# nv-tlabs/3dgrut

Measured on AMD Instinct MI355X. Metric: train rays/sec (3DGUT forward+backward, primary rays), higher is better.
Workload: dtype f32; 1 GPU; 3DGUT fwd+bwd, 1000000 Gaussians (cloud B trained-like, seed 42), 1920x1080, one view per GPU, SH degree 3, k_buffer 0; parallelism=view-dp1

## Files before the change

3dgrut_amd/csrc/common.hpp:

```cpp
#pragma once

#include <hip/hip_runtime.h>

#include <cstdarg>
#include <cstdint>
#include <cstdio>
#include <cstring>

#include "../../include/grut_amd.h"

#define GRUT_ABI_VERSION 5
#define GRUT_WAVE 64

namespace grut {

void set_last_error(const char* fmt, ...);

#define GRUT_HIP(expr)                                                                          \
    do {                                                                                        \
        hipError_t _e = (expr);                                                                 \
        if (_e != hipSuccess) {                                                                 \
            grut::set_last_error("%s:%d %s -> %s", __FILE__, __LINE__, #expr, hipGetErrorString(_e)); \
            return GRUT_ERR_RUNTIME;                                                            \
        }                                                                                       \
    } while (0)

#define GRUT_CHECK(expr)                       \
    do {                                       \
        int _s = (expr);                       \
        if (_s != GRUT_OK) return _s;          \
    } while (0)

#define GRUT_REQUIRE(cond, ...)                \
    do {                                       \
        if (!(cond)) {                         \
            grut::set_last_error(__VA_ARGS__); \
            return GRUT_ERR_BAD_INPUT;         \
        }                                      \
    } while (0)

#ifdef __HIPCC__
__device__ __forceinline__ uint32_t xcd_contiguous(uint32_t b, uint32_t n) {
    const uint32_t xcd = b & 7u, idx = b >> 3, q = n >> 3, rem = n & 7u;
    return xcd * q + (xcd < rem ? xcd : rem) + idx;
}
#endif

struct ScratchAllocator {
    void* (*alloc)(void* user, uint64_t bytes) = nullptr;
    void (*release)(void* user, void* ptr) = nullptr;
    void* user = nullptr;
};
ScratchAllocator& scratch_allocator();
inline hipStream_t& scratch_stream() {
    static thread_local hipStream_t s = nullptr;
    return s;
}
struct ScratchStreamScope {
    hipStream_t prev;
    explicit ScratchStreamScope(hipStream_t s) : prev(scratch_stream()) { scratch_stream() = s; }
    ~ScratchStreamScope() { scratch_stream() = prev; }
    ScratchStreamScope(const ScratchStreamScope&) = delete;
    ScratchStreamScope& operator=(const ScratchStreamScope&) = delete;
};
struct DeviceBuffer {
    void* ptr = nullptr;
    size_t bytes = 0;
    bool external = false;
    int ensure(size_t need, float growth = 1.0f) {
        if (need <= bytes) return GRUT_OK;
        size_t n = (size_t)((double)need * growth);
        n = (n + 255) & ~(size_t)255;
        release();
        const ScratchAllocator& a = scratch_allocator();
        if (a.alloc) {
            ptr = a.alloc(a.user, n);
            if (!ptr) {
                set_last_error("scratch allocation of %zu bytes failed in the caller's allocator", n);
                return GRUT_ERR_RUNTIME;
            }
            external = true;
            {
                static int count = 0;
                const char* pz = getenv("GRUT_POISON_SCRATCH");
                const char* pi = getenv("GRUT_POISON_INDEX");
                const bool poison = pz && (!pi || atoi(pi) == count);
                if (pz && pi && atoi(pi) == count) fprintf(stderr, "[grut] poisoned allocation %d: %zu bytes\n", count, n);
                ++count;
                GRUT_HIP(hipMemsetAsync(ptr, poison ? atoi(pz) : 0, n, scratch_stream()));
            }
        } else {
            GRUT_HIP(hipMalloc(&ptr, n));
            external = false;
        }
        bytes = n;
        return GRUT_OK;
    }
    void release() {
        if (ptr) {
            const ScratchAllocator& a = scratch_allocator();
            if (external && a.release) a.release(a.user, ptr);
            else if (!external) (void)hipFree(ptr);
        }
        ptr = nullptr;
        bytes = 0;
    }
    template <typename T> T* as() const { return reinterpret_cast<T*>(ptr); }
};

inline uint32_t div_up(uint32_t a, uint32_t b) { return (a + b - 1) / b; }

struct EventTimer {
    static constexpr int kRing = 256;
    hipEvent_t start[kRing], stop[kRing];
    int count = 0, created = 0;
    int begin(hipStream_t s) {
        int i = count % kRing;
        if (i >= created) {
            GRUT_HIP(hipEventCreate(&start[i]));
            GRUT_HIP(hipEventCreate(&stop[i]));
            created = i + 1;
        }
        GRUT_HIP(hipEventRecord(start[i], s));
        return GRUT_OK;
    }
    int end(hipStream_t s) {
        int i = count % kRing;
        GRUT_HIP(hipEventRecord(stop[i], s));
        count++;
        return GRUT_OK;
    }
    float collect() {
        int n = count < kRing ? count : kRing;
        if (n == 0) return -1.f;
        double sum = 0;
        for (int i = 0; i < n; ++i) {
            float ms = 0;
            (void)hipEventSynchronize(stop[i]);
            (void)hipEventElapsedTime(&ms, start[i], stop[i]);
            sum += ms;
        }
        count = 0;
        return (float)(sum / n);
    }
    void destroy() {
        for (int i = 0; i < created; ++i) {
            (void)hipEventDestroy(start[i]);
            (void)hipEventDestroy(stop[i]);
        }
        created = 0;
    }
};

size_t scan_scratch_bytes(uint32_t n);
int inclusive_scan_u32(hipStream_t s, uint32_t n, const uint32_t* in, const uint32_t* gather, uint32_t* out,
                       void* scratch, size_t scratch_bytes);
size_t sort_scratch_bytes(uint32_t n);
int sort_pairs_u32(hipStream_t s, uint32_t n, const uint32_t* n_dev, int begin_bit, int end_bit,
                   uint32_t* keys, uint32_t* vals, uint32_t* keys_tmp, uint32_t* vals_tmp,
                   void* scratch, size_t scratch_bytes, uint32_t** out_keys, uint32_t** out_vals, bool vals_iota = false);

}

#ifdef __HIPCC__
namespace grut {

struct f3 {
    float x, y, z;
};
__device__ __forceinline__ f3 mk3(float x, float y, float z) { return f3{x, y, z}; }
__device__ __forceinline__ f3 operator+(f3 a, f3 b) { return f3{a.x + b.x, a.y + b.y, a.z + b.z}; }
__device__ __forceinline__ f3 operator-(f3 a, f3 b) { return f3{a.x - b.x, a.y - b.y, a.z - b.z}; }
__device__ __forceinline__ f3 operator*(f3 a, f3 b) { return f3{a.x * b.x, a.y * b.y, a.z * b.z}; }
__device__ __forceinline__ f3 operator*(f3 a, float s) { return f3{a.x * s, a.y * s, a.z * s}; }
__device__ __forceinline__ f3 operator*(float s, f3 a) { return f3{a.x * s, a.y * s, a.z * s}; }
__device__ __forceinline__ float dot(f3 a, f3 b) { return fmaf(a.x, b.x, fmaf(a.y, b.y, a.z * b.z)); }
__device__ __forceinline__ float mul_rn(float a, float b) { float r; asm("v_mul_f32 %0, %1, %2" : "=v"(r) : "v"(a), "v"(b)); return r; }
__device__ __forceinline__ float add_rn(float a, float b) { float r; asm("v_add_f32 %0, %1, %2" : "=v"(r) : "v"(a), "v"(b)); return r; }
__device__ __forceinline__ float mul_rn_u(float uniform, float b) { float r; asm("v_mul_f32 %0, %1, %2" : "=v"(r) : "s"(uniform), "v"(b)); return r; }
__device__ __forceinline__ float add_rn_u(float uniform, float b) { float r; asm("v_add_f32 %0, %1, %2" : "=v"(r) : "s"(uniform), "v"(b)); return r; }
__device__ __forceinline__ f3 cross(f3 a, f3 b) {
    return f3{a.y * b.z - a.z * b.y, a.z * b.x - a.x * b.z, a.x * b.y - a.y * b.x};
}
struct m3 {
    f3 r0, r1, r2;
};
__device__ __forceinline__ f3 mul_rows(const m3& m, f3 p) { return f3{dot(m.r0, p), dot(m.r1, p), dot(m.r2, p)}; }
__device__ __forceinline__ f3 mul_cols(const m3& m, f3 g) {
    return f3{g.x * m.r0.x + g.y * m.r1.x + g.z * m.r2.x, g.x * m.r0.y + g.y * m.r1.y + g.z * m.r2.y,
              g.x * m.r0.z + g.y * m.r1.z + g.z * m.r2.z};
}
__device__ __forceinline__ m3 quat_wxyz_to_rotT(float r, float x, float y, float z) {
    const float xx = x * x, yy = y * y, zz = z * z, xy = x * y, xz = x * z, yz = y * z;
    const float rx = r * x, ry = r * y, rz = r * z;
    m3 m;
    m.r0 = f3{1.f - 2.f * (yy + zz), 2.f * (xy + rz), 2.f * (xz - ry)};
    m.r1 = f3{2.f * (xy - rz), 1.f - 2.f * (xx + zz), 2.f * (yz + rx)};
    m.r2 = f3{2.f * (xz + ry), 2.f * (yz - rx), 1.f - 2.f * (xx + yy)};
    return m;
}

template <int DEG>
__device__ __forceinline__ float particle_response(float g) {
    if constexpr (DEG == 8) { const float g2 = g * g; return __expf(-0.000685871056241f * g2 * g2); }
    else if constexpr (DEG == 5) return __expf(-0.0185185185185f * g * g * sqrtf(g));
    else if constexpr (DEG == 4) return __expf(-0.0555555555556f * g * g);
    else if constexpr (DEG == 3) return __expf(-0.166666666667f * g * sqrtf(g));
    else if constexpr (DEG == 1) return __expf(-1.5f * sqrtf(g));
    else if constexpr (DEG == 0) return fmaxf(1.f - 0.329630334487f * sqrtf(g), 0.f);
    else return __expf(-0.5f * g);
}
template <int DEG>
__device__ __forceinline__ float particle_response_grd(float g, float gres, float gresGrd) {
    if constexpr (DEG == 8) return (-0.000685871056241f * 4.f) * g * g * g * gres * gresGrd;
    else if constexpr (DEG == 5) return (-0.0185185185185f * 2.5f) * g * sqrtf(g) * gres * gresGrd;
    else if constexpr (DEG == 4) return (-0.0555555555556f * 2.f) * g * gres * gresGrd;
    else if constexpr (DEG == 3) return (-0.166666666667f * 1.5f) * sqrtf(g) * gres * gresGrd;
    else if constexpr (DEG == 1) return (-1.5f * 0.5f) * sqrtf(g) * gres * gresGrd;
    else if constexpr (DEG == 0) return gres > 0.f ? (0.5f * -0.329630334487f * rsqrtf(g)) * gresGrd : 0.f;
    else return -0.5f * gres * gresGrd;
}

__device__ __forceinline__ int lane_id() { return (int)__builtin_amdgcn_mbcnt_hi(~0u, __builtin_amdgcn_mbcnt_lo(~0u, 0u)); }

template <int CTRL, int ROW_MASK = 0xf>
__device__ __forceinline__ float dpp_add(float v) {
    const int moved = __builtin_amdgcn_update_dpp(0, __float_as_int(v), CTRL, ROW_MASK, 0xf, true);
    return v + __int_as_float(moved);
}
__device__ __forceinline__ float wave_sum_to_lane63(float v) {
    v = dpp_add<0x111>(v);
    v = dpp_add<0x112>(v);
    v = dpp_add<0x114>(v);
    v = dpp_add<0x118>(v);
    v = dpp_add<0x142, 0xa>(v);
    v = dpp_add<0x143, 0xc>(v);
    return v;
}
template <int CTRL>
__device__ __forceinline__ float dpp_perm(float v) {
    return __int_as_float(__builtin_amdgcn_update_dpp(0, __float_as_int(v), CTRL, 0xf, 0xf, true));
}
__device__ __forceinline__ float wave_reduce_scatter16_rows(const float (&v)[16], int lane) {
    const bool b3 = lane & 8, b2 = lane & 4, b1 = lane & 2, b0 = lane & 1;
    float w[8], x[4], y[2];
#pragma unroll
    for (int i = 0; i < 8; ++i) {
        const float keep = b3 ? v[8 + i] : v[i], send = b3 ? v[i] : v[8 + i];
        w[i] = keep + dpp_perm<0x140>(send);
    }
#pragma unroll
    for (int i = 0; i < 4; ++i) {
        const float keep = b2 ? w[4 + i] : w[i], send = b2 ? w[i] : w[4 + i];
        x[i] = keep + dpp_perm<0x141>(send);
    }
#pragma unroll
    for (int i = 0; i < 2; ++i) {
        const float keep = b1 ? x[2 + i] : x[i], send = b1 ? x[i] : x[2 + i];
        y[i] = keep + dpp_perm<0x4E>(send);
    }
    float z = (b0 ? y[1] : y[0]) + dpp_perm<0xB1>(b0 ? y[0] : y[1]);
    return z;
}
__device__ __forceinline__ float wave_reduce_scatter16(const float (&v)[16], int lane) {
    float z = wave_reduce_scatter16_rows(v, lane);
    z += __shfl_xor(z, 16, 64);
    z += __shfl_xor(z, 32, 64);
    return z;
}

__device__ __forceinline__ float wave_reduce_scatter16_all(const float (&v)[16], int lane) {
    typedef unsigned v2u __attribute__((ext_vector_type(2)));
    const float z = wave_reduce_scatter16_rows(v, lane);
    const v2u a = __builtin_amdgcn_permlane32_swap(__float_as_uint(z), __float_as_uint(z), false, false);
    const float s = __uint_as_float(a.x) + __uint_as_float(a.y);
    const v2u b = __builtin_amdgcn_permlane16_swap(__float_as_uint(s), __float_as_uint(s), false, false);
    return __uint_as_float(b.x) + __uint_as_float(b.y);
}

typedef float v2f __attribute__((ext_vector_type(2)));
struct p3 {
    v2f x, y, z;
};
__device__ __forceinline__ v2f splat(float s) { v2f r = {s, s}; return r; }
__device__ __forceinline__ v2f pfma(v2f a, v2f b, v2f c) { return __builtin_elementwise_fma(a, b, c); }
__device__ __forceinline__ v2f pfma(float a, v2f b, v2f c) { return __builtin_elementwise_fma(splat(a), b, c); }
__device__ __forceinline__ v2f pdot(p3 a, p3 b) { return pfma(a.x, b.x, pfma(a.y, b.y, a.z * b.z)); }
__device__ __forceinline__ v2f pdot(f3 a, p3 b) { return pfma(a.x, b.x, pfma(a.y, b.y, a.z * b.z)); }
__device__ __forceinline__ p3 pcross(p3 a, p3 b) {
    return p3{pfma(a.y, b.z, -(a.z * b.y)), pfma(a.z, b.x, -(a.x * b.z)), pfma(a.x, b.y, -(a.y * b.x))};
}
__device__ __forceinline__ v2f psel(bool c0, bool c1, v2f t, v2f f) { v2f r = {c0 ? t.x : f.x, c1 ? t.y : f.y}; return r; }
__device__ __forceinline__ v2f pmax0(v2f a) { v2f r = {fmaxf(a.x, 0.f), fmaxf(a.y, 0.f)}; return r; }
__device__ __forceinline__ v2f prcp(v2f a) { v2f r = {__builtin_amdgcn_rcpf(a.x), __builtin_amdgcn_rcpf(a.y)}; return r; }

template <int DEG>
__device__ __forceinline__ float response_gray_limit(float x) {
    if (!(x < 1.f) || !(x > 0.f)) return x > 0.f ? 0.f : 3.0e38f;
    const float L = -logf(x);
    if constexpr (DEG == 8) return sqrtf(sqrtf(L / 0.000685871056241f));
    else if constexpr (DEG == 5) return powf(L / 0.0185185185185f, 0.4f);
    else if constexpr (DEG == 4) return sqrtf(L / 0.0555555555556f);
    else if constexpr (DEG == 3) return powf(L / 0.166666666667f, 2.f / 3.f);
    else if constexpr (DEG == 1) { const float t = L / 1.5f; return t * t; }
    else if constexpr (DEG == 0) { const float t = (1.f - x) / 0.329630334487f; return t * t; }
    else return 2.f * L;
}

__device__ __forceinline__ float wave_sum(float v) {
    v = wave_sum_to_lane63(v);
    return __int_as_float(__builtin_amdgcn_readlane(__float_as_int(v), 63));
}

// ... 3 lines not shown
```

3dgrut_amd/csrc/grt_api.hip:

```cpp
#include <cstdlib>
#include <vector>

#include "grt_internal.hpp"

using namespace grut;

struct GrtHandle {
    GrtConfig cfg;
    int device = -1;
    uint32_t N = 0;
    bool built = false;
    hipStream_t build_stream = nullptr;
    DeviceBuffer refit_todo;
    DeviceBuffer box8;
    uint32_t NP = 0;
    DeviceBuffer inst, aabb, slack, scene_enc, scene, codes, ids, codes_tmp, ids_tmp, sort_scratch, nodes,
        counters, dbg_ids, dbg_count;
    uint32_t* sorted_ids = nullptr;
    uint32_t* sorted_codes = nullptr;
    float scene_host[6] = {0, 0, 0, 0, 0, 0};
    bool scene_host_valid = false;
    EventTimer fwd_timer, bwd_timer, build_timer;
    DeviceBuffer log_pool, log_table, log_nbwd, log_state;
    GrtHitLog log = {nullptr, nullptr, nullptr, nullptr, 0, 0};
// ... 73 lines not shown
}

static GrtTraceParams trace_params(const GrtHandle* h, const GrtFrame& f) {
    GrtTraceParams P;
    memset(&P, 0, sizeof(P));
    P.degree = h->cfg.particle_kernel_degree;
    P.prim = h->cfg.primitive_type;
    P.bary = h->cfg.pipeline_type == GRUT_PIPELINE_BARYCENTRIC_SURFELS;
    P.clamping = h->cfg.particle_kernel_density_clamping;
    P.box8 = h->cfg.primitive_type == GRUT_PRIM_CUSTOM ? h->box8.as<float>() : nullptr;
    P.ncoef = (h->cfg.particle_radiance_sph_degree + 1) * (h->cfg.particle_radiance_sph_degree + 1);
    P.sph_degree = f.sph_degree < h->cfg.particle_radiance_sph_degree ? f.sph_degree : h->cfg.particle_radiance_sph_degree;
    if (P.sph_degree < 0) P.sph_degree = 0;
    P.normals = h->cfg.enable_normals;
    P.hitcounts = h->cfg.enable_hitcounts;
    P.min_response = h->cfg.particle_kernel_min_response;
    P.min_alpha = h->cfg.particle_kernel_min_alpha;
    P.max_alpha = h->cfg.particle_kernel_max_alpha;
    P.min_transmittance = f.min_transmittance;
    P.W = f.width;
    P.H = f.height;
    for (int k = 0; k < 12; ++k) P.ray_to_world[k] = f.ray_to_world[k];
    P.ray_to_world_dev = f.device_ray_to_world;
    P.sph_half = h->cfg.particle_feature_half;
    P.nht = h->cfg.feature_transform_type;
    if (P.nht) {
        const GrtConfig& c = h->cfg;
        P.nht_k = c.particle_feature_dim; P.nht_ipd = c.interp_point_feature_dim; P.nht_support = c.feature_interpolation_support;
        P.nht_act = c.feature_activation_type; P.nht_nf = c.feature_activation_num_frequencies;
        P.nht_ray_dim = P.nht_ipd * (P.nht_act == 2 ? 2 * P.nht_nf : (P.nht_act == 1 ? P.nht_nf : 1));
    }
    static const int sphere_lists = getenv("GRUT_GRT_SPHERE_LISTS") ? 1 : 0;
    P.sphere_lists = sphere_lists;
    static const float list_mark = getenv("GRUT_GRT_LIST_MARK") ? (float)atof(getenv("GRUT_GRT_LIST_MARK")) : 1.0f;
    P.list_mark = list_mark;
    static const uint32_t lane_area = getenv("GRUT_GRT_LANE_AREA") ? (uint32_t)atoi(getenv("GRUT_GRT_LANE_AREA")) : 32u;
    P.bin_lane_area = lane_area < 1u ? 1u : (lane_area > 64u ? 64u : lane_area);
    P.out_half = h->cfg.feature_output_half;
    return P;
}

static GrtBvh bvh_view(const GrtHandle* h) {
    GrtBvh b;
    b.nodes = h->nodes.as<GrtNode>();
    b.inst = h->inst.as<float>();
    b.scene = h->scene.as<float>();
    b.N = h->NP;
    return b;
}

extern "C" {

int grt_create(const GrtConfig* config, GrtHandle** handle) {
    GRUT_REQUIRE(config && handle, "grt_create: null argument");
    GRUT_CHECK(grt_validate(*config));
    GrtHandle* h = new GrtHandle();
    h->cfg = *config;
    if (hipGetDevice(&h->device) != hipSuccess) {
        set_last_error("grt_create: no HIP device");
        delete h;
        return GRUT_ERR_RUNTIME;
    }
    if (hipHostMalloc(reinterpret_cast<void**>(&h->log_state_host), 64, hipHostMallocDefault) != hipSuccess ||
        hipEventCreateWithFlags(&h->log_event, hipEventDisableTiming) != hipSuccess) {
        set_last_error("grt_create: pinned buffer / event allocation failed");
        delete h;
        return GRUT_ERR_RUNTIME;
    }
    *handle = h;
    return GRUT_OK;
}

static void release_scratch(GrtHandle* h) {
    DeviceBuffer* bufs[] = {&h->refit_todo, &h->box8, &h->inst, &h->aabb, &h->slack, &h->scene_enc, &h->scene, &h->codes, &h->ids, &h->codes_tmp, &h->ids_tmp,
                            &h->sort_scratch, &h->nodes, &h->counters, &h->dbg_ids, &h->dbg_count,
                            &h->work_counters, &h->l_flags, &h->l_starts, &h->l_bounds, &h->l_pair_cache, &h->l_block_cones, &h->l_super_cones, &h->l_inst_rel, &h->l_key_bits,
                            &h->l_counts, &h->l_pidx, &h->l_key_tmp, &h->l_pidx_tmp, &h->l_offsets, &h->l_scan_scratch, &h->l_sort_scratch,
                            &h->l_block_keys, &h->l_vals, &h->l_block_keys_tmp, &h->l_vals_tmp, &h->l_ranges,
                            &h->log_pool, &h->log_table, &h->log_nbwd, &h->log_state, &h->m_aabb, &h->m_slack, &h->m_scene_enc,
                            &h->m_scene, &h->m_codes, &h->m_ids, &h->m_codes_tmp, &h->m_ids_tmp, &h->m_sort_scratch, &h->m_nodes, &h->m_done, &h->m_materials};
    for (DeviceBuffer* b : bufs) b->release();
}

int grt_trim(GrtHandle* h) {
    GRUT_REQUIRE(h, "grt_trim: null handle");
    GRUT_HIP(hipDeviceSynchronize());
    release_scratch(h);
    h->built = false;
    h->tree_async = false;
    h->mesh_built = false;
    h->N = 0;
    h->NP = 0;
    h->log_valid = false;
    h->log_event_pending = false;
    h->scene_host_valid = false;
    h->list_entries = 0;
    h->log = GrtHitLog{nullptr, nullptr, nullptr, nullptr, 0, 0};
    h->log_lists = GrtLists{nullptr, nullptr, nullptr, nullptr, nullptr};
    h->sorted_codes = nullptr;
    h->sorted_ids = nullptr;
    return GRUT_OK;
}

void grt_destroy(GrtHandle* h) {
    if (!h) return;
    if (h->tree_stream) (void)hipStreamSynchronize(h->tree_stream);
    release_scratch(h);
    if (h->log_state_host) (void)hipHostFree(h->log_state_host);
    if (h->l_host) (void)hipHostFree(h->l_host);
    if (h->log_event) (void)hipEventDestroy(h->log_event);
    if (h->list_event) (void)hipEventDestroy(h->list_event);
    if (h->side_fork) (void)hipEventDestroy(h->side_fork);
    if (h->side_join) (void)hipEventDestroy(h->side_join);
    if (h->side_stream) (void)hipStreamDestroy(h->side_stream);
    if (h->tree_fork) (void)hipEventDestroy(h->tree_fork);
    if (h->tree_done) (void)hipEventDestroy(h->tree_done);
    if (h->tree_stream) (void)hipStreamDestroy(h->tree_stream);
    h->fwd_timer.destroy();
    h->bwd_timer.destroy();
    h->build_timer.destroy();
    delete h;
}

int grt_build_bvh(GrtHandle* h, void* stream_, uint32_t N, const float* positions, const float* rotations, const float* scales,
                  const float* densities, int rebuild, int allow_update) {
    (void)allow_update;
    GRUT_REQUIRE(h, "grt_build_bvh: null handle");
    hipStream_t s = reinterpret_cast<hipStream_t>(stream_);
    ScratchStreamScope scratch_scope(s);
    if (N == 0) {
        h->N = 0;
        h->NP = 0;
        h->built = true;
        return GRUT_OK;
    }
    GRUT_REQUIRE(positions && rotations && scales && densities, "grt_build_bvh: null buffer");
    const uint32_t per = h->cfg.primitive_type == GRUT_PRIM_TRIHEXA ? 3u : (h->cfg.primitive_type == GRUT_PRIM_SPHERE ? 2u : 1u);
    GRUT_REQUIRE((uint64_t)N * per <= 0x1FFFFFFEu, "grt_build_bvh: %u particles (the hit buffers keep 29 bits of proxy index)", N);
    if (!rebuild && (!h->built || h->N != N)) rebuild = 1;
    GRUT_CHECK(h->wait_tree(s));
    if (h->cfg.enable_kernel_timings) GRUT_CHECK(h->build_timer.begin(s));
    const uint32_t NP = N * per;
    const size_t n = NP;
    GRUT_CHECK(h->inst.ensure(n * 48, 1.25f));
    GRUT_CHECK(h->aabb.ensure(n * 24, 1.25f));
    GRUT_CHECK(h->slack.ensure(n * 4, 1.25f));
    if (h->cfg.primitive_type == GRUT_PRIM_CUSTOM) GRUT_CHECK(h->box8.ensure(n * 32, 1.25f));
    GRUT_CHECK(h->scene_enc.ensure(grt_scene_enc_bytes()));
    GRUT_CHECK(h->scene.ensure(64));
    GRUT_CHECK(h->codes.ensure(n * 4, 1.25f));
    GRUT_CHECK(h->ids.ensure(n * 4, 1.25f));
    GRUT_CHECK(h->codes_tmp.ensure(n * 4, 1.25f));
    GRUT_CHECK(h->ids_tmp.ensure(n * 4, 1.25f));
    GRUT_CHECK(h->sort_scratch.ensure(sort_scratch_bytes((uint32_t)(n * 1.25f) + 4096)));
    GRUT_CHECK(h->nodes.ensure(n * sizeof(GrtNode), 1.25f));
    GRUT_CHECK(h->counters.ensure(n * 4, 1.25f));

    GrtBuildParams P;
    P.N = NP;
    P.degree = h->cfg.particle_kernel_degree;
    P.prim = h->cfg.primitive_type;
    P.clamping = h->cfg.particle_kernel_density_clamping;
    P.min_response = h->cfg.particle_kernel_min_response;
    uint32_t* scene_enc = h->scene_enc.as<uint32_t>();
    grt_launch_proxies(s, P, positions, rotations, scales, densities, h->inst.as<float>(), h->aabb.as<float>(), h->slack.as<float>(), scene_enc,
                       h->cfg.primitive_type == GRUT_PRIM_CUSTOM ? h->box8.as<float>() : nullptr);
    grt_launch_morton(s, NP, h->aabb.as<float>(), scene_enc, h->scene.as<float>(), rebuild ? h->codes.as<uint32_t>() : nullptr,
                      rebuild ? h->ids.as<uint32_t>() : nullptr);
    GRUT_CHECK(h->refit_todo.ensure((n + 1) * 4, 1.25f));
    static const bool sync_build = getenv("GRUT_GRT_SYNC_BUILD") != nullptr;
    hipStream_t ts = s;
    h->tree_async = false;
    if (!sync_build) {
        if (!h->tree_stream) {
            GRUT_HIP(hipStreamCreateWithFlags(&h->tree_stream, hipStreamNonBlocking));
            GRUT_HIP(hipEventCreateWithFlags(&h->tree_fork, hipEventDisableTiming));
            GRUT_HIP(hipEventCreateWithFlags(&h->tree_done, hipEventDisableTiming));
        }
        GRUT_HIP(hipEventRecord(h->tree_fork, s));
        GRUT_HIP(hipStreamWaitEvent(h->tree_stream, h->tree_fork, 0));
        ts = h->tree_stream;
    }
    if (rebuild) {
        uint32_t *sc = nullptr, *si = nullptr;
        GRUT_CHECK(sort_pairs_u32(ts, NP, nullptr, 0, 30, h->codes.as<uint32_t>(), h->ids.as<uint32_t>(), h->codes_tmp.as<uint32_t>(),
                                  h->ids_tmp.as<uint32_t>(), h->sort_scratch.ptr, h->sort_scratch.bytes, &sc, &si));
        h->sorted_codes = sc;
        h->sorted_ids = si;
        grt_launch_hierarchy(ts, NP, sc, si, h->nodes.as<GrtNode>());
    }
    GRUT_HIP(hipMemsetAsync(h->counters.ptr, 0, n, ts));
    grt_launch_refit(ts, NP, h->aabb.as<float>(), h->slack.as<float>(), h->nodes.as<GrtNode>(), h->counters.as<uint8_t>(), h->refit_todo.as<uint32_t>());
    GRUT_HIP(hipGetLastError());
    if (h->cfg.enable_kernel_timings) GRUT_CHECK(h->build_timer.end(ts));
    if (ts != s) {
        GRUT_HIP(hipEventRecord(h->tree_done, ts));
        h->tree_async = true;
    }
    h->N = N;
    h->NP = NP;
    h->built = true;
    h->build_stream = s;
    h->scene_host_valid = false;
    return GRUT_OK;
}

static int build_lists(GrtHandle* h, hipStream_t s, const GrtTraceParams& P, const GrtBvh& bvh, const float* ray_origin, const float* ray_direction,
                       GrtLists* out) {
    GrtLists lists = {nullptr, nullptr, nullptr, nullptr, nullptr, nullptr};
    h->list_entries = 0;
    h->log_lists = lists;
    if (!getenv("GRUT_GRT_NO_LISTS") && h->N > 0 && !(h->cfg.primitive_type == GRUT_PRIM_CUSTOM && getenv("GRUT_GRT_CUSTOM_WALK")) && !(h->cfg.primitive_type == GRUT_PRIM_TRIHEXA && getenv("GRUT_GRT_TRIHEXA_WALK")) && !(h->cfg.primitive_type == GRUT_PRIM_TRISURFEL && getenv("GRUT_GRT_TRISURFEL_WALK")) &&
        (h->cfg.primitive_type == GRUT_PRIM_INSTANCES || !getenv("GRUT_GRT_NO_MESH_LISTS"))) {
        const uint32_t N = h->NP, nb = grt_num_blocks(P.W, P.H), ns = grt_num_super(P.W, P.H);
        if (!h->l_host) GRUT_HIP(hipHostMalloc(reinterpret_cast<void**>(&h->l_host), 64));
        GRUT_CHECK(h->l_flags.ensure(64));
        GRUT_CHECK(h->l_block_cones.ensure(grt_cone_table_bytes(P.W, P.H), 1.25f));
        GRUT_CHECK(h->l_super_cones.ensure((size_t)ns * sizeof(GrtCone), 1.25f));
        GRUT_CHECK(h->l_inst_rel.ensure((size_t)N * 64, 1.25f));
        GRUT_CHECK(h->l_pair_cache.ensure(grt_pair_cache_bytes(N), 1.25f));
        for (DeviceBuffer* b4 : {&h->l_key_bits, &h->l_counts, &h->l_pidx, &h->l_key_tmp, &h->l_pidx_tmp, &h->l_offsets, &h->l_starts})
            GRUT_CHECK(b4->ensure((size_t)N * 4, 1.25f));
        GRUT_CHECK(h->l_scan_scratch.ensure(scan_scratch_bytes((uint32_t)(N * 1.25f) + 4096)));
        uint32_t* flag = h->l_flags.as<uint32_t>();
        uint32_t* dir_len = flag + 2;
        grt_launch_list_cones(s, P, ray_origin, ray_direction, flag, dir_len, h->l_block_cones.as<GrtCone>(), h->l_super_cones.as<GrtCone>());
        grt_launch_list_count(s, P, bvh, ray_origin, flag, dir_len, h->l_block_cones.as<GrtCone>(), h->l_super_cones.as<GrtCone>(),
                              h->l_inst_rel.as<float>(), h->l_key_bits.as<uint32_t>(), h->l_counts.as<uint32_t>(), h->l_pidx.as<uint32_t>(), h->l_pair_cache.ptr);
        GRUT_CHECK(h->l_sort_scratch.ensure(sort_scratch_bytes((uint32_t)(N * 1.25f) + 4096)));
        uint32_t *sorted_key = nullptr, *rank_to_particle = nullptr;
        GRUT_CHECK(sort_pairs_u32(s, N, nullptr, 16, 32, h->l_key_bits.as<uint32_t>(), h->l_pidx.as<uint32_t>(), h->l_key_tmp.as<uint32_t>(),
                                  h->l_pidx_tmp.as<uint32_t>(), h->l_sort_scratch.ptr, h->l_sort_scratch.bytes, &sorted_key, &rank_to_particle, true));
        GRUT_CHECK(inclusive_scan_u32(s, N, h->l_counts.as<uint32_t>(), rank_to_particle, h->l_offsets.as<uint32_t>(), h->l_scan_scratch.ptr,
                                      h->l_scan_scratch.bytes));
        grt_launch_list_check(s, N, h->l_offsets.as<uint32_t>(), flag);
        GRUT_HIP(hipMemcpyAsync(&h->l_host[0], h->l_offsets.as<uint32_t>() + (N - 1), 4, hipMemcpyDeviceToHost, s));
        GRUT_HIP(hipMemcpyAsync(&h->l_host[1], flag, 8, hipMemcpyDeviceToHost, s));
        if (!h->list_event) GRUT_HIP(hipEventCreateWithFlags(&h->list_event, hipEventDisableTiming));
        GRUT_HIP(hipEventRecord(h->list_event, s));
        int bits = 1;
        while ((1ull << bits) <= nb) ++bits;
        uint32_t *sorted_blocks = nullptr, *sorted_ids = nullptr;
        auto enqueue_tail = [&](uint32_t n, const uint32_t* n_dev) -> int {
            grt_launch_list_expand(s, P, bvh, ray_origin, flag, dir_len, h->l_block_cones.as<GrtCone>(), h->l_super_cones.as<GrtCone>(),
                                   rank_to_particle, h->l_offsets.as<uint32_t>(), h->l_counts.as<uint32_t>(), h->l_starts.as<uint32_t>(), n,
                                   h->l_block_keys.as<uint32_t>(), h->l_vals.as<uint32_t>(), h->l_pair_cache.ptr);
            GRUT_CHECK(sort_pairs_u32(s, n, n_dev, 0, bits, h->l_block_keys.as<uint32_t>(), h->l_vals.as<uint32_t>(), h->l_block_keys_tmp.as<uint32_t>(),
                                      h->l_vals_tmp.as<uint32_t>(), h->l_sort_scratch.ptr, h->l_sort_scratch.bytes, &sorted_blocks, &sorted_ids));
            GRUT_HIP(hipMemsetAsync(h->l_ranges.ptr, 0, (size_t)nb * 8, s));
            grt_launch_list_ranges(s, n, n_dev, nb, sorted_blocks, h->l_ranges.as<uint32_t>());
            return GRUT_OK;
        };
        auto ensure_entries = [&](uint32_t n) -> bool {
            bool ok = true;
            for (DeviceBuffer* b4 : {&h->l_block_keys, &h->l_vals, &h->l_block_keys_tmp, &h->l_vals_tmp}) ok = ok && b4->ensure((size_t)n * 4, 1.3f) == GRUT_OK;
            ok = ok && h->l_ranges.ensure((size_t)nb * 8, 1.25f) == GRUT_OK;
            ok = ok && h->l_bounds.ensure((size_t)n * 8, 1.3f) == GRUT_OK;
            ok = ok && h->l_sort_scratch.ensure(sort_scratch_bytes((uint32_t)(n * 1.3f) + 4096)) == GRUT_OK;
            if (!ok) (void)hipGetLastError();
            return ok;
        };
        auto entry_capacity = [&]() -> uint32_t {
            size_t cap = h->l_bounds.bytes / 8;
            for (const DeviceBuffer* b4 : {&h->l_block_keys, &h->l_vals, &h->l_block_keys_tmp, &h->l_vals_tmp}) cap = cap < b4->bytes / 4 ? cap : b4->bytes / 4;
            if (h->l_ranges.bytes < (size_t)nb * 8) return 0u;
            while (cap > 0 && h->l_sort_scratch.bytes < sort_scratch_bytes((uint32_t)cap)) cap = cap * 3 / 4;
            return (uint32_t)(cap < 0xFFFF0000ull ? cap : 0xFFFF0000ull);
        };
        const bool speculate = getenv("GRUT_GRT_SPECULATE") != nullptr;
        const uint32_t spec_cap = speculate ? entry_capacity() : 0u;
        if (spec_cap > 0) GRUT_CHECK(enqueue_tail(spec_cap, h->l_offsets.as<uint32_t>() + (N - 1)));
        GRUT_HIP(hipEventSynchronize(h->list_event));
        const uint64_t I = h->l_host[0];
        bool usable = h->l_host[1] != 0u && h->l_host[2] == 0u && I > 0 && I < 0xFFFF0000ull;
        if (usable && !(spec_cap > 0 && I <= spec_cap)) {
            usable = ensure_entries((uint32_t)I);
            if (usable) GRUT_CHECK(enqueue_tail((uint32_t)I, nullptr));
        }
        if (usable) {
            lists.ranges = h->l_ranges.as<uint32_t>();
            lists.entries = sorted_ids;
            lists.inst_rel = h->l_inst_rel.as<float>();
            lists.block_cones = h->l_block_cones.as<GrtCone>();
            lists.dir_len_enc = dir_len;
            lists.bounds = h->l_bounds.as<float2>();
            h->list_entries = I;
        }
    }
    *out = lists;
    return GRUT_OK;
}

static int grt_forward_impl(GrtHandle* h, hipStream_t s, const GrtFrame* frame, const float* particle_density, const float* particle_sph,
                            const float* ray_origin, const float* ray_direction, float* out_features, float* out_density,
                            float* out_hit_distance, float* out_normals, float* out_hits_count, int32_t* out_visibility,
                            uint32_t* dbg_ids, uint32_t* dbg_count, uint32_t dbg_cap) {
    ScratchStreamScope scratch_scope(s);
    GRUT_REQUIRE(h && frame, "grt_forward: null handle/frame");
    if (!h->built) {
        set_last_error("grt_forward: build_bvh has not been called");
        return GRUT_ERR_NOT_READY;
    }
    GRUT_REQUIRE(frame->width > 0 && frame->height > 0, "grt_forward: empty image");
    GRUT_REQUIRE(frame->num_particles == h->N, "grt_forward: %u particles but the BVH holds %u", frame->num_particles, h->N);
    GRUT_REQUIRE(ray_origin && ray_direction && out_features && out_density && out_hit_distance && out_hits_count, "grt_forward: null buffer");
    if (h->N == 0) return GRUT_OK;
    GRUT_REQUIRE(particle_density && particle_sph && out_visibility, "grt_forward: null particle buffer");
    GRUT_REQUIRE(!h->cfg.enable_normals || out_normals, "grt_forward: normals enabled but no buffer");
    GrtTraceParams P = trace_params(h, *frame);
    P.dbg_cap = dbg_cap;
    if (h->cfg.enable_kernel_timings) GRUT_CHECK(h->fwd_timer.begin(s));
    GrtHitLog log = {nullptr, nullptr, nullptr, nullptr, 0, 0};
    h->log_valid = false;
    GRUT_REQUIRE(!(P.nht && dbg_ids), "grt_debug_forward_hits: not provided with neural harmonic features");
    if ((frame->keep_hits_for_backward || P.nht) && !dbg_ids && !P.bary) {
        const uint32_t blocks = div_up((uint32_t)P.W, 8) * div_up((uint32_t)P.H, 8);
        uint32_t want = blocks * 10u;
        if (h->log_event_pending && hipEventQuery(h->log_event) == hipSuccess) {
            h->log_event_pending = false;
            const uint32_t used = h->log_state_host[0];
            if (used + used / 2 > want) want = used + used / 2;
            if (h->log_state_host[7] && h->log_rounds < 4096u) h->log_rounds *= 2u;
        }
        const uint32_t kMaxRounds = h->log_rounds;
        if (h->log.capacity_chunks > want) want = h->log.capacity_chunks;
        if (const char* e = getenv("GRUT_GRT_LOG_CHUNKS")) want = (uint32_t)atoi(e) > 0 ? (uint32_t)atoi(e) : 1u;
        GRUT_CHECK(h->log_pool.ensure((size_t)want * kGrtLogSlots * 64 * 4));
        GRUT_CHECK(h->log_table.ensure((size_t)blocks * kMaxRounds * 4, 1.25f));
        GRUT_CHECK(h->log_nbwd.ensure((size_t)P.W * P.H * 4, 1.25f));
        GRUT_CHECK(h->log_state.ensure(64));
        h->log.pool = h->log_pool.as<uint32_t>();
        h->log.table = h->log_table.as<uint32_t>();
        h->log.ray_flags = h->log_nbwd.as<uint32_t>();
        h->log.state = h->log_state.as<uint32_t>();
        h->log.capacity_chunks = want;
        h->log.max_rounds = kMaxRounds;
        GRUT_HIP(hipMemsetAsync(h->log.table, 0xFF, (size_t)blocks * kMaxRounds * 4, s));
        GRUT_HIP(hipMemsetAsync(h->log.state, 0, 64, s));
        log = h->log;
        h->log_valid = true;
        h->log_W = P.W;
        h->log_H = P.H;
        h->log_density = particle_density;
        h->log_ray_o = ray_origin;
        h->log_ray_d = ray_direction;
        h->log_frame = *frame;
    }
    unsigned long long* counters = nullptr;
    if (getenv("GRUT_GRT_COUNT")) {
        const size_t wbytes = 128 + 24 * ((size_t)div_up((uint32_t)P.W, 64) * div_up((uint32_t)P.H, 64) * 64 + 512);
        GRUT_CHECK(h->work_counters.ensure(wbytes));
        counters = h->work_counters.as<unsigned long long>();
        GRUT_HIP(hipMemsetAsync(counters, 0, wbytes, s));
    }
    GrtBvh bvh = bvh_view(h);
    GrtLists lists;
    GRUT_CHECK(build_lists(h, s, P, bvh, ray_origin, ray_direction, &lists));
    if (h->log_valid || (P.bary && frame->keep_hits_for_backward)) h->log_lists = lists;
    if (!lists.ranges) GRUT_CHECK(h->wait_tree(s));
    grt_launch_trace_fwd(s, P, bvh, particle_density, particle_sph, ray_origin, ray_direction, out_features, out_density,
                         out_hit_distance, out_normals, out_hits_count, out_visibility, dbg_ids, dbg_count, counters, log, lists);
    if (P.nht) {
        for (int attempt = 0; attempt < 8; ++attempt) {
            uint32_t st[8] = {0, 0, 0, 0, 0, 0, 0, 0};
            GRUT_HIP(hipMemcpyAsync(st, log.state, 32, hipMemcpyDeviceToHost, s));
            GRUT_HIP(hipStreamSynchronize(s));
            if (st[1] == 0u && st[7] == 0u) break;
            GRUT_REQUIRE(attempt < 7, "grt_forward: the hit log does not fit (neural harmonic features)");
            const uint32_t blocks = div_up((uint32_t)P.W, 8) * div_up((uint32_t)P.H, 8);
            if (st[7]) {
                h->log_rounds = h->log_rounds < 4096u ? h->log_rounds * 2u : h->log_rounds;
                GRUT_CHECK(h->log_table.ensure((size_t)blocks * h->log_rounds * 4, 1.25f));
                h->log.table = h->log_table.as<uint32_t>();
                h->log.max_rounds = h->log_rounds;
            }
            const uint32_t want = st[7] && st[0] < h->log.capacity_chunks ? h->log.capacity_chunks : h->log.capacity_chunks * 2u;
            GRUT_CHECK(h->log_pool.ensure((size_t)want * kGrtLogSlots * 64 * 4));
            h->log.pool = h->log_pool.as<uint32_t>();
            h->log.capacity_chunks = want;
            GRUT_HIP(hipMemsetAsync(h->log.table, 0xFF, (size_t)blocks * h->log.max_rounds * 4, s));
            GRUT_HIP(hipMemsetAsync(h->log.state, 0, 64, s));
            log = h->log;
            grt_launch_trace_fwd(s, P, bvh, particle_density, particle_sph, ray_origin, ray_direction, out_features, out_density,
                                 out_hit_distance, out_normals, out_hits_count, out_visibility, dbg_ids, dbg_count, counters, log, lists);
        }
        grt_launch_nht_fwd(s, P, particle_density, particle_sph, ray_origin, ray_direction, out_features, log);
    }
    if (log.pool && !h->log_event_pending) {
        GRUT_HIP(hipMemcpyAsync(h->log_state_host, log.state, 32, hipMemcpyDeviceToHost, s));
        GRUT_HIP(hipEventRecord(h->log_event, s));
        h->log_event_pending = true;
    }
    if (counters) {
        GRUT_HIP(hipMemcpyAsync(h->work_host, counters, 128, hipMemcpyDeviceToHost, s));
        GRUT_HIP(hipStreamSynchronize(s));
        fprintf(stderr, "[grut] grt fwd: nodes %llu, leaf tests %llu, processed %llu, rounds %llu, inserts %llu (rays %d)\n", h->work_host[0],
                h->work_host[1], h->work_host[2], h->work_host[3], h->work_host[4], frame->width * frame->height);
        fprintf(stderr, "[grut] grt fwd list batches fetched (64 entries each) %llu\n", h->work_host[12]);
        fprintf(stderr, "[grut] grt fwd leaf tests: passed %llu, distance out of range %llu, box missed %llu, beyond 3 sigma %llu; wave-level leaf visits %llu, of which ran the box test %llu, the insert chain %llu\n",
                h->work_host[5], h->work_host[6], h->work_host[7], h->work_host[8], h->work_host[9], h->work_host[10], h->work_host[11]);
        fprintf(stderr, "[grut] grt fwd phases, summed over the packets' waves (ms): scans %.1f (candidate work loops %.1f with packet lists), hit log %.1f, per-hit evaluation %.1f\n", h->work_host[13] * 1e-5,
                lists.ranges ? h->work_host[0] * 1e-5 : 0.0, h->work_host[14] * 1e-5, h->work_host[15] * 1e-5);
        if (lists.ranges) h->work_host[0] = 0;
    }
    GRUT_HIP(hipGetLastError());
    if (h->cfg.enable_kernel_timings) GRUT_CHECK(h->fwd_timer.end(s));
    return GRUT_OK;
}

int grt_forward(GrtHandle* h, void* stream_, const GrtFrame* frame, const float* particle_density, const void* particle_sph,
                const float* ray_origin, const float* ray_direction, void* out_features, float* out_density, float* out_hit_distance,
                float* out_normals, float* out_hits_count, int32_t* out_visibility) {
    return grt_forward_impl(h, reinterpret_cast<hipStream_t>(stream_), frame, particle_density, reinterpret_cast<const float*>(particle_sph), ray_origin, ray_direction,
                            reinterpret_cast<float*>(out_features), out_density, out_hit_distance, out_normals, out_hits_count, out_visibility, nullptr, nullptr, 0);
}

int grt_debug_forward_hits(GrtHandle* h, void* stream_, const GrtFrame* frame, const float* particle_density, const void* particle_sph,
                           const float* ray_origin, const float* ray_direction, void* out_features, float* out_density,
                           float* out_hit_distance, float* out_normals, float* out_hits_count, int32_t* out_visibility,
                           uint32_t* hit_ids, uint32_t* hit_counts, uint32_t capacity) {
    GRUT_REQUIRE(hit_ids && hit_counts && capacity > 0, "grt_debug_forward_hits: null hit buffers");
    return grt_forward_impl(h, reinterpret_cast<hipStream_t>(stream_), frame, particle_density, reinterpret_cast<const float*>(particle_sph), ray_origin, ray_direction,
                            reinterpret_cast<float*>(out_features), out_density, out_hit_distance, out_normals, out_hits_count, out_visibility, hit_ids, hit_counts,
                            capacity);
}

int grt_backward(GrtHandle* h, void* stream_, const GrtFrame* frame, const float* particle_density, const void* particle_sph_,
                 const float* ray_origin, const float* ray_direction, const void* features_, const float* density, const float* hit_distance,
                 const float* normals, const float* grad_features, const float* grad_density, const float* grad_hit_distance,
                 const float* grad_normals, float* grad_particle_density, float* grad_particle_sph) {
    const float* particle_sph = reinterpret_cast<const float*>(particle_sph_);
    const float* features = reinterpret_cast<const float*>(features_);
    (void)normals;
    (void)grad_normals;
    GRUT_REQUIRE(h && frame, "grt_backward: null handle/frame");
    if (h->cfg.pipeline_type == GRUT_PIPELINE_BARYCENTRIC_SURFELS) {
        set_last_error("grt_backward: pipeline_type barycentricSurfels is forward only (the reference ships no backward program for it)");
        return GRUT_ERR_UNSUPPORTED;
    }
    hipStream_t s = reinterpret_cast<hipStream_t>(stream_);
    ScratchStreamScope scratch_scope(s);
    if (!h->built) {
        set_last_error("grt_backward: build_bvh has not been called");
        return GRUT_ERR_NOT_READY;
    }
    GRUT_REQUIRE(frame->num_particles == h->N, "grt_backward: %u particles but the BVH holds %u", frame->num_particles, h->N);
    if (h->N == 0) return GRUT_OK;
    GRUT_REQUIRE(particle_density && particle_sph && ray_origin && ray_direction && features && density && hit_distance && grad_features &&
                     grad_density && grad_particle_density && grad_particle_sph, "grt_backward: null buffer");
    GrtTraceParams P = trace_params(h, *frame);
    P.bwd_sig = h->dbg_bwd_sig;
    P.bwd_cnt = h->dbg_bwd_cnt;
    if (h->cfg.enable_kernel_timings) GRUT_CHECK(h->bwd_timer.begin(s));
    GrtHitLog log = {nullptr, nullptr, nullptr, nullptr, 0, 0};
    GrtLists lists = {nullptr, nullptr, nullptr, nullptr, nullptr, nullptr};
    if (h->log_matches(*frame, particle_density, ray_origin, ray_direction)) {
        log = h->log;
        lists = h->log_lists;
    }
    if (log.pool && getenv("GRUT_GRT_COUNT")) {
        std::vector<uint32_t> nb((size_t)P.W * P.H);
        uint32_t st[2] = {0, 0};
        GRUT_HIP(hipMemcpyAsync(nb.data(), log.ray_flags, nb.size() * 4, hipMemcpyDeviceToHost, s));
        GRUT_HIP(hipMemcpyAsync(st, log.state, 8, hipMemcpyDeviceToHost, s));
        GRUT_HIP(hipStreamSynchronize(s));
        size_t flagged = 0;
        for (uint32_t v : nb) flagged += (v >> 31);
        fprintf(stderr, "[grut] grt bwd: %zu of %zu rays re-derive their rounds (log chunks %u, overflow %u, lists %s)\n", flagged, nb.size(), st[0], st[1],
                lists.ranges ? "yes" : "no");
    }
    if (!lists.ranges) GRUT_CHECK(h->wait_tree(s));
    hipStream_t rederive = s;
    struct SideJoin {
        GrtHandle* h;
        hipStream_t s;
        bool armed;
        int join() {
            armed = false;
            GRUT_HIP(hipEventRecord(h->side_join, h->side_stream));
            GRUT_HIP(hipStreamWaitEvent(s, h->side_join, 0));
            return GRUT_OK;
        }
        ~SideJoin() { if (armed) (void)join(); }
    } side{h, s, false};
    if (log.pool) {
        if (!h->side_stream) {
            GRUT_HIP(hipStreamCreateWithFlags(&h->side_stream, hipStreamNonBlocking));
            GRUT_HIP(hipEventCreateWithFlags(&h->side_fork, hipEventDisableTiming));
            GRUT_HIP(hipEventCreateWithFlags(&h->side_join, hipEventDisableTiming));
        }
        GRUT_HIP(hipEventRecord(h->side_fork, s));
        side.armed = true;
        GRUT_HIP(hipStreamWaitEvent(h->side_stream, h->side_fork, 0));
        rederive = h->side_stream;
    }
    grt_launch_trace_bwd(s, rederive, P, bvh_view(h), particle_density, particle_sph, ray_origin, ray_direction, features, density, hit_distance,
                         grad_features, grad_density, grad_hit_distance, grad_particle_density, grad_particle_sph, log, lists);
    if (log.pool) GRUT_CHECK(side.join());
    GRUT_HIP(hipGetLastError());
    if (h->cfg.enable_kernel_timings) GRUT_CHECK(h->bwd_timer.end(s));
    return GRUT_OK;
}

int grt_build_mesh_bvh(GrtHandle* h, void* stream_, uint32_t num_vertices, const float* vertices, uint32_t num_faces, const int32_t* triangles,
                       int rebuild, int allow_update) {
    GRUT_REQUIRE(h, "grt_build_mesh_bvh: null handle");
    hipStream_t s = reinterpret_cast<hipStream_t>(stream_);
    ScratchStreamScope scratch_scope(s);
    const bool refit_only = !rebuild && allow_update && h->mesh_built && h->mesh_faces == num_faces && num_faces > 0;
    h->mesh_built = false;
    if (num_faces == 0) {
        h->mesh_faces = 0;
        h->mesh_built = true;
        return GRUT_OK;
    }
    GRUT_REQUIRE(vertices && triangles && num_vertices > 0, "grt_build_mesh_bvh: null buffer");
    const size_t n = num_faces;
    GRUT_CHECK(h->m_aabb.ensure(n * 24, 1.25f));
    GRUT_CHECK(h->m_slack.ensure(n * 4, 1.25f));
    GRUT_CHECK(h->m_scene_enc.ensure(grt_scene_enc_bytes()));
    GRUT_CHECK(h->m_scene.ensure(64));
    GRUT_CHECK(h->m_codes.ensure(n * 4, 1.25f));
    GRUT_CHECK(h->m_ids.ensure(n * 4, 1.25f));
    GRUT_CHECK(h->m_codes_tmp.ensure(n * 4, 1.25f));
    GRUT_CHECK(h->m_ids_tmp.ensure(n * 4, 1.25f));
    GRUT_CHECK(h->m_sort_scratch.ensure(sort_scratch_bytes((uint32_t)(n * 1.25f) + 4096)));
    GRUT_CHECK(h->m_nodes.ensure(n * sizeof(GrtNode), 1.25f));
    GRUT_CHECK(h->m_done.ensure(n * 4, 1.25f));
    grt_launch_mesh_aabb(s, num_faces, vertices, triangles, h->m_aabb.as<float>(), h->m_slack.as<float>(), h->m_scene_enc.as<uint32_t>());
    grt_launch_morton(s, num_faces, h->m_aabb.as<float>(), h->m_scene_enc.as<uint32_t>(), h->m_scene.as<float>(),
                      refit_only ? nullptr : h->m_codes.as<uint32_t>(), refit_only ? nullptr : h->m_ids.as<uint32_t>());
    if (!refit_only) {
        uint32_t *sc = nullptr, *si = nullptr;
        GRUT_CHECK(sort_pairs_u32(s, num_faces, nullptr, 0, 30, h->m_codes.as<uint32_t>(), h->m_ids.as<uint32_t>(), h->m_codes_tmp.as<uint32_t>(),
                                  h->m_ids_tmp.as<uint32_t>(), h->m_sort_scratch.ptr, h->m_sort_scratch.bytes, &sc, &si));
        grt_launch_hierarchy(s, num_faces, sc, si, h->m_nodes.as<GrtNode>());
    }
    GRUT_HIP(hipMemsetAsync(h->m_done.ptr, 0, n, s));
    grt_launch_refit(s, num_faces, h->m_aabb.as<float>(), h->m_slack.as<float>(), h->m_nodes.as<GrtNode>(), h->m_done.as<uint8_t>());
    GRUT_HIP(hipGetLastError());
    h->mesh_faces = num_faces;
    h->mesh_built = true;
    return GRUT_OK;
}

int grt_trace_hybrid(GrtHandle* h, void* stream_, const GrtFrame* frame, const float* particle_density, const void* particle_sph_,
                     const float* ray_origin, const float* ray_direction, const float* ray_max_t, const GrtMesh* mesh, const GrtHybridOptions* options,
                     float* out_radiance, float* out_opacity, float* out_last_ray, uint32_t* out_bounces) {
    GRUT_REQUIRE(h && frame && mesh && options, "grt_trace_hybrid: null argument");
    const float* particle_sph = reinterpret_cast<const float*>(particle_sph_);
    hipStream_t s = reinterpret_cast<hipStream_t>(stream_);
    ScratchStreamScope scratch_scope(s);
    if (!h->built || !h->mesh_built) {
        set_last_error("grt_trace_hybrid: build_bvh / build_mesh_bvh have not been called");
        return GRUT_ERR_NOT_READY;
    }
    GRUT_REQUIRE(frame->width > 0 && frame->height > 0 && ray_origin && ray_direction && out_radiance && out_opacity, "grt_trace_hybrid: null buffer");
    GRUT_REQUIRE(frame->num_particles == h->N, "grt_trace_hybrid: %u particles but the BVH holds %u", frame->num_particles, h->N);
    GRUT_REQUIRE(mesh->num_faces == h->mesh_faces, "grt_trace_hybrid: %u faces but the mesh BVH holds %u", mesh->num_faces, h->mesh_faces);
    GRUT_REQUIRE(h->N == 0 || (particle_density && particle_sph), "grt_trace_hybrid: null particle buffer");
    GRUT_REQUIRE(mesh->num_faces == 0 || (mesh->vertices && mesh->triangles && mesh->prim_type && mesh->refractive_index), "grt_trace_hybrid: null mesh buffer");
    GRUT_REQUIRE(!(options->playground_opts & 1u) || mesh->num_faces == 0 || mesh->vertex_normals, "grt_trace_hybrid: smooth normals need vertex_normals");
    GRUT_REQUIRE((mesh->vertex_tangents != nullptr) == (mesh->vertex_has_tangents != nullptr), "grt_trace_hybrid: vertex_tangents and vertex_has_tangents go together");
    GRUT_REQUIRE(mesh->num_materials == 0 || mesh->materials, "grt_trace_hybrid: null material table");
    const GrtTraceParams P = trace_params(h, *frame);
    GRUT_CHECK(h->wait_tree(s));
    GrtBvh bvh = bvh_view(h);
    GrtMaterial fallback;
    memset(&fallback, 0, sizeof(fallback));
    fallback.diffuse_factor[0] = fallback.diffuse_factor[1] = fallback.diffuse_factor[2] = fallback.diffuse_factor[3] = 1.f;
    fallback.alpha_cutoff = 0.5f;
    const uint32_t nm = mesh->num_materials ? mesh->num_materials : 1u;
    GRUT_CHECK(h->m_materials.ensure((size_t)nm * sizeof(GrtMaterial), 2.f));
    GRUT_HIP(hipMemcpyAsync(h->m_materials.ptr, mesh->num_materials ? mesh->materials : &fallback, (size_t)nm * sizeof(GrtMaterial), hipMemcpyHostToDevice, s));
    GRUT_HIP(hipStreamSynchronize(s));
    GrtMeshView mv;
    mv.nodes = h->m_nodes.as<GrtNode>();
    mv.vertices = mesh->vertices; mv.triangles = mesh->triangles; mv.vnormals = mesh->vertex_normals; mv.vtangents = mesh->vertex_tangents;
    mv.vhas_tangents = mesh->vertex_has_tangents; mv.prim_type = mesh->prim_type; mv.mat_uv = mesh->mat_uv; mv.mat_id = mesh->mat_id;
    mv.refr = mesh->refractive_index; mv.materials = h->m_materials.as<GrtMaterial>(); mv.num_materials = nm; mv.envmap = mesh->envmap;
    mv.envmap_offset[0] = mesh->envmap_offset[0]; mv.envmap_offset[1] = mesh->envmap_offset[1];
    mv.F = mesh->num_faces;
    GrtHybridParams hp;
    hp.opts = options->playground_opts;
    hp.max_pbr_bounces = options->max_pbr_bounces;
    hp.frame_number = options->frame_number;
    if (h->cfg.enable_kernel_timings) GRUT_CHECK(h->fwd_timer.begin(s));
    GrtLists lists;
    GRUT_CHECK(build_lists(h, s, P, bvh, ray_origin, ray_direction, &lists));
    grt_launch_hybrid(s, P, bvh, mv, hp, particle_density, particle_sph, ray_origin, ray_direction, ray_max_t, out_radiance, out_opacity, out_last_ray,
                      out_bounces, lists);
    GRUT_HIP(hipGetLastError());
    if (h->cfg.enable_kernel_timings) GRUT_CHECK(h->fwd_timer.end(s));
    return GRUT_OK;
}

int grt_debug_backward_signature(GrtHandle* h, unsigned long long* ray_signature, uint32_t* ray_hit_count) {
    GRUT_REQUIRE(h && ((ray_signature != nullptr) == (ray_hit_count != nullptr)), "grt_debug_backward_signature: both buffers or none");
    h->dbg_bwd_sig = ray_signature;
    h->dbg_bwd_cnt = ray_hit_count;
    return GRUT_OK;
}

int grt_timings(GrtHandle* h, float* forward_ms, float* backward_ms, float* build_ms) {
    GRUT_REQUIRE(h, "grt_timings: null handle");
    if (forward_ms) *forward_ms = h->fwd_timer.collect();
    if (backward_ms) *backward_ms = h->bwd_timer.collect();
    if (build_ms) *build_ms = h->build_timer.collect();
    return GRUT_OK;
}

int grt_debug_fetch_work(GrtHandle* h, void* stream_, unsigned long long* out, uint64_t count) {
    GRUT_REQUIRE(h && out, "grt_debug_fetch_work: null argument");
    GRUT_REQUIRE(h->work_counters.ptr && count * 8 <= h->work_counters.bytes, "grt_debug_fetch_work: no instrumented frame / count too large");
    GRUT_HIP(hipMemcpyAsync(out, h->work_counters.ptr, count * 8, hipMemcpyDeviceToDevice, reinterpret_cast<hipStream_t>(stream_)));
    return GRUT_OK;
}

int grt_stats(GrtHandle* h, GrtStats* stats) {
    GRUT_REQUIRE(h && stats, "grt_stats: null argument");
    memset(stats, 0, sizeof(*stats));
    stats->num_particles = h->N;
    stats->num_nodes = h->NP > 1 ? h->NP - 1 : (h->NP ? 1 : 0);
    stats->nodes_visited = h->work_host[0];
    stats->candidates = h->work_host[1];
    stats->processed_hits = h->work_host[2];
    stats->list_entries = h->list_entries;
    stats->packet_tests = h->work_host[9];
    stats->list_batches = h->work_host[12];
    if (h->log_valid && h->log.pool) {
        uint32_t st[8] = {0, 0, 0, 0, 0, 0, 0, 0};
        GRUT_HIP(hipDeviceSynchronize());
        GRUT_HIP(hipMemcpy(st, h->log.state, 32, hipMemcpyDeviceToHost));
        stats->bwd_premise_rays = st[2];
        stats->bwd_rederived_rays = st[3];
        stats->bwd_atomic_instructions = st[4];
        stats->bwd_atomic_words = (uint64_t)st[5] * 16u;
    }
    if (h->built && h->N > 0) {
        if (!h->scene_host_valid) {
            GRUT_HIP(hipMemcpyAsync(h->scene_host, h->scene.ptr, 24, hipMemcpyDeviceToHost, h->build_stream));
            GRUT_HIP(hipStreamSynchronize(h->build_stream));
            h->scene_host_valid = true;
        }
        for (int k = 0; k < 6; ++k) stats->scene_aabb[k] = h->scene_host[k];
    }
    return GRUT_OK;
}

int grt_debug_fetch_instances(GrtHandle* h, void* stream_, float* instances) {
    GRUT_REQUIRE(h && h->built && instances, "grt_debug_fetch_instances: no BVH / null buffer");
    const size_t per = h->N ? h->NP / h->N : 1;
    if (h->N) GRUT_HIP(hipMemcpy2DAsync(instances, 48, h->inst.ptr, 48 * per, 48, h->N, hipMemcpyDeviceToDevice, reinterpret_cast<hipStream_t>(stream_)));
    return GRUT_OK;
}

int grt_debug_fetch_custom_boxes(GrtHandle* h, void* stream_, float* box8) {
    GRUT_REQUIRE(h && h->built && box8, "grt_debug_fetch_custom_boxes: no BVH / null buffer");
    if (h->cfg.primitive_type != GRUT_PRIM_CUSTOM) { set_last_error("grt_debug_fetch_custom_boxes: primitive_type is not custom"); return GRUT_ERR_NOT_READY; }
    if (h->N) GRUT_HIP(hipMemcpyAsync(box8, h->box8.ptr, (size_t)h->N * 32, hipMemcpyDeviceToDevice, reinterpret_cast<hipStream_t>(stream_)));
    return GRUT_OK;
}

int grt_debug_fetch_lists(GrtHandle* h, void* stream_, uint32_t* ranges, uint32_t* entries, uint64_t entry_capacity) {
    GRUT_REQUIRE(h && ranges && entries, "grt_debug_fetch_lists: null argument");
    if (!h->log_lists.ranges || h->list_entries == 0 || h->list_entries > entry_capacity) {
        set_last_error("grt_debug_fetch_lists: no packet lists kept (a training forward of a one-origin frame keeps them) or capacity %llu < %llu entries",
                       (unsigned long long)entry_capacity, (unsigned long long)h->list_entries);
        return GRUT_ERR_NOT_READY;
    }
    hipStream_t s = reinterpret_cast<hipStream_t>(stream_);
    const uint32_t blocks = div_up((uint32_t)h->log_W, 8) * div_up((uint32_t)h->log_H, 8);
    GRUT_HIP(hipMemcpyAsync(ranges, h->log_lists.ranges, (size_t)blocks * 8, hipMemcpyDeviceToDevice, s));
    GRUT_HIP(hipMemcpyAsync(entries, h->log_lists.entries, (size_t)h->list_entries * 4, hipMemcpyDeviceToDevice, s));
    return GRUT_OK;
}

}
```

3dgrut_amd/csrc/gut_api.hip:

```cpp
#include <vector>

#include "gut_internal.hpp"

namespace grut {

static thread_local char g_last_error[512] = "";
ScratchAllocator& scratch_allocator() {
    static ScratchAllocator a;
    return a;
}
void set_last_error(const char* fmt, ...) {
    va_list ap;
    va_start(ap, fmt);
    vsnprintf(g_last_error, sizeof(g_last_error), fmt, ap);
    va_end(ap);
}

static uint32_t bits_for(uint32_t n) {
    uint32_t b = 1;
    while ((1ull << b) <= n) ++b;
    return b;
}

}

using namespace grut;

struct GutHandle {
    GutConfig cfg;
    int device = -1;
    DeviceBuffer tiles_count, proj_pos, conic_opacity, extent, depth, rgb, depth_key, particle_idx;
    DeviceBuffer depth_key_tmp, particle_idx_tmp, offsets, sort_scratch, scan_scratch, counters;
    DeviceBuffer rec64;
    DeviceBuffer part_offset, pos_particle, grad_partial, grad_flag, g_rgb, poses_dev, walk8;
    DeviceBuffer tile_keys, tile_vals, tile_keys_tmp, tile_vals_tmp, tile_sort_scratch, ranges;
    DeviceBuffer ck_tc, ck_d, ck_reached, ck_boundary_tile, ck_nht;
    GutCheckpoints checkpoints;
    uint32_t* host_counters = nullptr;
    hipEvent_t count_event = nullptr;
    bool have_forward = false;
    hipStream_t fwd_stream = nullptr;
    const void* fwd_density = nullptr;
    const void* fwd_ray_o = nullptr;
    const void* fwd_ray_d = nullptr;
    uint32_t fwd_frame_id = 0;
    GutParams params;
    uint32_t num_intersections = 0;
    uint32_t tile_capacity = 0;
    uint32_t ck_boundaries_capacity = 0;
    uint32_t* sorted_pos = nullptr;
    uint32_t* sorted_tile_keys = nullptr;
    uint32_t* rank_to_particle = nullptr;
    GutStats stats;
    EventTimer fwd_timer, bwd_timer;
    bool profile = false;
    bool count_work = false;
    DeviceBuffer work_counters;
    unsigned long long work_host[4] = {0, 0, 0, 0};
    bool work_pending = false;
    static constexpr int kProfRing = 64;
    hipEvent_t prof_ev[kProfRing][GUT_NUM_STAGES][2];
    bool prof_used[kProfRing][GUT_NUM_STAGES];
    int prof_slot = 0, prof_created = 0;
    int prof_fwd_slot = 0;

    uint32_t profile_mask = 0xFFFFFFFFu;
    int stage_begin(int stage, hipStream_t s, int slot) {
        if (!profile || !((profile_mask >> stage) & 1u)) return GRUT_OK;
        GRUT_HIP(hipEventRecord(prof_ev[slot][stage][0], s));
        return GRUT_OK;
    }
    int stage_end(int stage, hipStream_t s, int slot) {
        if (!profile || !((profile_mask >> stage) & 1u)) return GRUT_OK;
        GRUT_HIP(hipEventRecord(prof_ev[slot][stage][1], s));
        prof_used[slot][stage] = true;
        return GRUT_OK;
    }
};

static int validate_config(const GutConfig& c) {
    GRUT_REQUIRE(c.ut_require_all_sigma_points_valid == 0, "ut_require_all_sigma_points_valid must be false (threedgut.cuh:78)");
    GRUT_REQUIRE(c.particle_radiance_sph_degree >= 0 && c.particle_radiance_sph_degree <= 3, "sph degree must be in [0,3]");
    if (c.k_buffer_size != 0 && c.k_buffer_size != 4 && c.k_buffer_size != 8 && c.k_buffer_size != 16) {
        set_last_error("k_buffer_size=%d: the hit buffer is instantiated for 0 (unsorted), 4, 8 and 16 entries", c.k_buffer_size);
        return GRUT_ERR_UNSUPPORTED;
    }
    if (c.feature_transform_type != 0) {
        GRUT_REQUIRE(c.feature_transform_type == 1, "feature_transform_type %d: 0 (SH) or 1 (neural harmonic features)", c.feature_transform_type);
        GRUT_REQUIRE(c.feature_interpolation_support == 0 || c.feature_interpolation_support == 1, "feature_interpolation_support must be 0 (centre) or 1 (tetrahedra)");
        GRUT_REQUIRE(c.feature_activation_type >= 0 && c.feature_activation_type <= 3, "feature_activation_type must be 0..3");
        const int points = c.feature_interpolation_support == 1 ? 4 : 1;
        GRUT_REQUIRE(c.interp_point_feature_dim >= 1 && c.interp_point_feature_dim <= 16 && c.particle_feature_dim == points * c.interp_point_feature_dim,
                     "particle_feature_dim %d must be %d x interp_point_feature_dim (1..16)", c.particle_feature_dim, points);
        const int nf = c.feature_activation_num_frequencies;
        const int nr = c.interp_point_feature_dim * (c.feature_activation_type == 2 ? 2 * nf : (c.feature_activation_type == 1 ? nf : 1));
        GRUT_REQUIRE(nf >= 1 && nr >= 1 && nr <= 32, "ray feature dim %d: 1..32 supported", nr);
    }
    const int d = c.particle_kernel_degree;
    GRUT_REQUIRE(d == 0 || d == 1 || d == 2 || d == 3 || d == 4 || d == 5 || d == 8, "unsupported particle_kernel_degree %d", d);
    return GRUT_OK;
}

static GutParams make_params(const GutConfig& c, const GutFrame& f) {
    GutParams P;
    memset(&P, 0, sizeof(P));
    P.degree = c.particle_kernel_degree;
    P.min_response = c.particle_kernel_min_response;
    P.min_alpha = c.particle_kernel_min_alpha;
    P.max_alpha = c.particle_kernel_max_alpha;
    P.min_transmittance = c.min_transmittance;
    P.n_active = f.n_active_features < c.particle_radiance_sph_degree ? f.n_active_features : c.particle_radiance_sph_degree;
    if (P.n_active < 0) P.n_active = 0;
    P.ncoef = (c.particle_radiance_sph_degree + 1) * (c.particle_radiance_sph_degree + 1);
    P.hitcounts = c.enable_hitcounts;
    const float D = 3.f;
    const float lambda = c.ut_alpha * c.ut_alpha * (D + c.ut_kappa) - D;
    P.ut_w0m = lambda / (D + lambda);
    P.ut_wi = 1.f / (2.f * (D + lambda));
    P.ut_w0c = lambda / (D + lambda) + (1.f - c.ut_alpha * c.ut_alpha + c.ut_beta);
    P.ut_delta = sqrtf(c.ut_alpha * c.ut_alpha * (D + c.ut_kappa));
    P.ut_margin = c.ut_in_image_margin_factor;
    P.ut_require_all = c.ut_require_all_sigma_points_valid;
    P.n_rs_iter = c.n_rolling_shutter_iterations;
    P.k_buffer = c.k_buffer_size;
    P.global_z = c.global_z_order;
    P.rect_bounding = c.rect_bounding;
    P.tight_opacity = c.tight_opacity_bounding;
    P.tile_culling = c.tile_based_culling;
    P.W = f.width;
    P.H = f.height;
    P.gx = (f.width + 15) / 16;
    P.gy = (f.height + 15) / 16;
    P.N = f.num_particles;
    P.cam = f.camera;
    P.poses = make_frame_poses(f.pose_start, f.pose_end);
    P.poses_dev = nullptr;
    P.work = nullptr;
    P.out_features = f.out_features;
    P.out_opacity = f.out_opacity;
    P.sph_half = c.particle_feature_half;
    P.out_half = c.feature_output_half;
    P.nht = c.feature_transform_type;
    if (P.nht) {
        P.nht_k = c.particle_feature_dim; P.nht_ipd = c.interp_point_feature_dim; P.nht_support = c.feature_interpolation_support;
        P.nht_act = c.feature_activation_type; P.nht_nf = c.feature_activation_num_frequencies;
        P.nht_ray_dim = P.nht_ipd * (P.nht_act == 2 ? 2 * P.nht_nf : (P.nht_act == 1 ? P.nht_nf : 1));
    }
    return P;
}

static int ensure_particle_scratch(GutHandle* h, uint32_t N) {
    const size_t n = N ? N : 1;
    GRUT_CHECK(h->tiles_count.ensure(n * 4, 1.25f));
    GRUT_CHECK(h->proj_pos.ensure(n * 8, 1.25f));
    GRUT_CHECK(h->conic_opacity.ensure(n * 16, 1.25f));
    GRUT_CHECK(h->extent.ensure(n * 8, 1.25f));
    GRUT_CHECK(h->depth.ensure(n * 4, 1.25f));
    GRUT_CHECK(h->rgb.ensure(n * 12, 1.25f));
    GRUT_CHECK(h->depth_key.ensure(n * 4, 1.25f));
    GRUT_CHECK(h->particle_idx.ensure(n * 4, 1.25f));
    GRUT_CHECK(h->depth_key_tmp.ensure(n * 4, 1.25f));
    GRUT_CHECK(h->particle_idx_tmp.ensure(n * 4, 1.25f));
    GRUT_CHECK(h->offsets.ensure(n * 4, 1.25f));
    GRUT_CHECK(h->part_offset.ensure(n * 4, 1.25f));
    GRUT_CHECK(h->rec64.ensure(n * 64, 1.25f));
    GRUT_CHECK(h->walk8.ensure(n * 8, 1.25f));
    GRUT_CHECK(h->sort_scratch.ensure(sort_scratch_bytes((uint32_t)(n * 1.25f) + 4096)));
    GRUT_CHECK(h->scan_scratch.ensure(scan_scratch_bytes((uint32_t)(n * 1.25f) + 4096)));
    if (!h->counters.ptr) {
        GRUT_CHECK(h->counters.ensure(kGutCounterWords * 4));
        GRUT_HIP(hipMemset(h->counters.ptr, 0, kGutCounterWords * 4));
    }
    return GRUT_OK;
}

static int ensure_intersection_scratch(GutHandle* h, uint32_t I, uint32_t tiles) {
    const size_t n = I ? I : 1;
    if (n > h->tile_capacity) h->tile_capacity = (uint32_t)n;
    GRUT_CHECK(h->tile_keys.ensure(n * 4, 1.3f));
    GRUT_CHECK(h->tile_vals.ensure(n * 4, 1.3f));
    GRUT_CHECK(h->tile_keys_tmp.ensure(n * 4, 1.3f));
    GRUT_CHECK(h->tile_vals_tmp.ensure(n * 4, 1.3f));
    GRUT_CHECK(h->pos_particle.ensure(n * 4, 1.3f));
    GRUT_CHECK(h->tile_sort_scratch.ensure(sort_scratch_bytes((uint32_t)n), 1.3f));
    GRUT_CHECK(h->ranges.ensure((size_t)tiles * 8 + 8));
    const size_t nb = (size_t)I / kGutSegment + 1;
    if (!h->params.nht && h->params.k_buffer == 0) {
        GRUT_CHECK(h->ck_tc.ensure(nb * 4 * 64 * 16, 1.3f));
        GRUT_CHECK(h->ck_d.ensure(nb * 4 * 64 * 4, 1.3f));
    }
    GRUT_CHECK(h->ck_reached.ensure(nb * 4, 1.3f));
    GRUT_CHECK(h->ck_boundary_tile.ensure(nb * 4, 1.3f));
    h->checkpoints.tc = h->ck_tc.as<float4>();
    h->checkpoints.d = h->ck_d.as<float>();
    h->checkpoints.reached = h->ck_reached.as<uint8_t>();
    h->checkpoints.boundary_tile = h->ck_boundary_tile.as<uint32_t>();
    h->checkpoints.num_boundaries = (uint32_t)nb;
    h->ck_boundaries_capacity = (uint32_t)nb;
    if (nht_fast_path(h->params)) GRUT_CHECK(h->ck_nht.ensure(nht_checkpoint_bytes((uint32_t)nb), 1.3f));
    return GRUT_OK;
}

static GutProjected projected_view(GutHandle* h) {
    GutProjected p;
    p.tiles_count = h->tiles_count.as<uint32_t>();
    p.proj_pos = h->proj_pos.as<float2>();
    p.conic_opacity = h->conic_opacity.as<float4>();
    p.extent = h->extent.as<float2>();
    p.depth = h->depth.as<float>();
    p.rgb = h->rgb.as<float>();
    p.depth_key = h->depth_key.as<uint32_t>();
    p.particle_idx = h->particle_idx.as<uint32_t>();
    p.part_offset = h->part_offset.as<uint32_t>();
    p.rec64 = h->rec64.as<float4>();
    static const bool no_walk_cache = getenv("GRUT_GUT_NO_WALK_CACHE") != nullptr;
    p.walk8 = (no_walk_cache || h->params.gx >= 4096 || h->params.gy >= 4096) ? nullptr : h->walk8.as<uint2>();
    return p;
}

extern "C" {

int grut_abi_version(void) { return GRUT_ABI_VERSION; }
int grut_set_allocator(GrutAllocFn alloc_fn, GrutFreeFn free_fn, void* user) {
    GRUT_REQUIRE((alloc_fn == nullptr) == (free_fn == nullptr), "grut_set_allocator: give both functions or neither");
    grut::ScratchAllocator& a = grut::scratch_allocator();
    a.alloc = alloc_fn;
    a.release = free_fn;
    a.user = user;
    return GRUT_OK;
}
const char* grut_last_error(void) { return grut::g_last_error; }

int gut_create(const GutConfig* config, GutHandle** handle) {
    GRUT_REQUIRE(config && handle, "gut_create: null argument");
    GRUT_CHECK(validate_config(*config));
    GutHandle* h = new GutHandle();
    h->cfg = *config;
    memset(&h->stats, 0, sizeof(h->stats));
    if (hipGetDevice(&h->device) != hipSuccess) {
        set_last_error("gut_create: no HIP device");
        delete h;
        return GRUT_ERR_RUNTIME;
    }
    if (hipHostMalloc(reinterpret_cast<void**>(&h->host_counters), 64, hipHostMallocDefault) != hipSuccess ||
        hipEventCreateWithFlags(&h->count_event, hipEventDisableTiming) != hipSuccess) {
        set_last_error("gut_create: pinned counter / event allocation failed");
        delete h;
        return GRUT_ERR_RUNTIME;
    }
    *handle = h;
    return GRUT_OK;
}

static void release_scratch(GutHandle* h) {
    DeviceBuffer* bufs[] = {&h->tiles_count, &h->proj_pos, &h->conic_opacity, &h->extent, &h->depth, &h->rgb, &h->depth_key,
                            &h->particle_idx, &h->depth_key_tmp, &h->particle_idx_tmp, &h->offsets, &h->sort_scratch,
                            &h->scan_scratch, &h->counters, &h->rec64, &h->walk8, &h->part_offset, &h->pos_particle, &h->grad_partial, &h->grad_flag,
                            &h->g_rgb, &h->poses_dev, &h->work_counters, &h->tile_keys, &h->tile_vals, &h->tile_keys_tmp,
                            &h->tile_vals_tmp, &h->tile_sort_scratch, &h->ranges, &h->ck_tc, &h->ck_d, &h->ck_nht, &h->ck_reached,
                            &h->ck_boundary_tile};
    for (DeviceBuffer* b : bufs) b->release();
}

int gut_trim(GutHandle* h) {
    GRUT_REQUIRE(h, "gut_trim: null handle");
    if (h->fwd_stream) GRUT_HIP(hipStreamSynchronize(h->fwd_stream));
    else GRUT_HIP(hipDeviceSynchronize());
    release_scratch(h);
    h->tile_capacity = 0;
    h->have_forward = false;
    h->num_intersections = 0;
    h->sorted_pos = nullptr;
    h->sorted_tile_keys = nullptr;
    h->work_pending = false;
    h->ck_boundaries_capacity = 0;
    memset(&h->checkpoints, 0, sizeof(h->checkpoints));
    return GRUT_OK;
}

void gut_destroy(GutHandle* h) {
    if (!h) return;
    release_scratch(h);
    if (h->host_counters) (void)hipHostFree(h->host_counters);
    if (h->count_event) (void)hipEventDestroy(h->count_event);
    h->fwd_timer.destroy();
    h->bwd_timer.destroy();
    if (h->prof_created)
        for (int r = 0; r < GutHandle::kProfRing; ++r)
            for (int st = 0; st < GUT_NUM_STAGES; ++st) {
                (void)hipEventDestroy(h->prof_ev[r][st][0]);
                (void)hipEventDestroy(h->prof_ev[r][st][1]);
            }
    delete h;
}

int gut_forward(GutHandle* h, void* stream_, const GutFrame* frame, const float* particle_density, const void* particle_sph_,
                const float* ray_origin, const float* ray_direction, void* out_feat_density_, float* out_hit_distance,
                float* out_hit_count, int32_t* out_visibility) {
    const float* particle_sph = reinterpret_cast<const float*>(particle_sph_);
    float* out_feat_density = reinterpret_cast<float*>(out_feat_density_);
    GRUT_REQUIRE(h && frame, "gut_forward: null handle/frame");
    GRUT_REQUIRE(frame->width > 0 && frame->height > 0, "gut_forward: empty image");
    GRUT_REQUIRE(ray_origin && ray_direction && out_feat_density && out_hit_distance && out_hit_count, "gut_forward: null ray/output buffer");
    hipStream_t s = reinterpret_cast<hipStream_t>(stream_);
    ScratchStreamScope scratch_scope(s);
    h->have_forward = false;
    const uint32_t N = frame->num_particles;
    h->params = make_params(h->cfg, *frame);
    const GutParams& P = h->params;
    const uint32_t tiles = (uint32_t)(P.gx * P.gy);
    h->stats.num_particles = N;
    h->stats.num_tiles = tiles;
    h->stats.num_visible = 0;
    h->stats.num_intersections = 0;
    h->stats.key_bits = bits_for(tiles);
    h->num_intersections = 0;
    h->fwd_stream = s;
    h->fwd_density = particle_density;
    h->fwd_ray_o = ray_origin;
    h->fwd_ray_d = ray_direction;
    h->fwd_frame_id = frame->frame_id;
    if (N == 0) {
        h->have_forward = true;
        return GRUT_OK;
    }
    GRUT_REQUIRE(particle_density && particle_sph && out_visibility, "gut_forward: null particle buffer");
    GRUT_REQUIRE(!h->cfg.feature_output_half || (!frame->out_features && !frame->out_opacity), "gut_forward: feature_output_half excludes out_features / out_opacity");
    GRUT_REQUIRE(!h->cfg.feature_transform_type || (!frame->out_features && !frame->out_opacity), "gut_forward: neural harmonic features exclude out_features / out_opacity");
    if (h->cfg.enable_kernel_timings) GRUT_CHECK(h->fwd_timer.begin(s));

    GRUT_CHECK(ensure_particle_scratch(h, N));
    static const bool legacy_lists = getenv("GRUT_GUT_LEGACY_LISTS") != nullptr;
    const bool direct = h->stats.key_bits <= 16 && !legacy_lists;
    h->params.rec64 = direct ? h->rec64.as<float4>() : nullptr;
    h->params.ord_shift = h->stats.key_bits;
    h->params.sorted_keys = nullptr;
    if (frame->device_T_to_world) {
// ... 8 lines not shown
        h->params.work = h->work_counters.as<unsigned long long>();
        h->params.work_task_capacity = (uint32_t)((h->work_counters.bytes / 8 - fwd_words) / 2);
        h->work_pending = true;
    }
    const GutProjected proj = projected_view(h);
    uint32_t* d_counters = h->counters.as<uint32_t>();

    const int slot = h->prof_slot % GutHandle::kProfRing;
    if (h->profile) {
        for (int st = 0; st < GUT_NUM_STAGES; ++st) h->prof_used[slot][st] = false;
        h->prof_fwd_slot = slot;
        h->prof_slot++;
    }
    GRUT_CHECK(h->stage_begin(GUT_STAGE_PROJECT, s, slot));
    launch_project(s, P, particle_density, particle_sph, proj, out_visibility, d_counters + 1);
    GRUT_CHECK(h->stage_end(GUT_STAGE_PROJECT, s, slot));
    GRUT_CHECK(h->stage_begin(GUT_STAGE_DEPTH_SORT, s, slot));
    uint32_t *sorted_depth = nullptr, *rank_to_particle = nullptr;
    GRUT_CHECK(sort_pairs_u32(s, N, nullptr, 0, 32, proj.depth_key, proj.particle_idx, h->depth_key_tmp.as<uint32_t>(),
                              h->particle_idx_tmp.as<uint32_t>(), h->sort_scratch.ptr, h->sort_scratch.bytes, &sorted_depth,
                              &rank_to_particle, true));
    h->rank_to_particle = rank_to_particle;
    GRUT_CHECK(h->stage_end(GUT_STAGE_DEPTH_SORT, s, slot));
    GRUT_CHECK(h->stage_begin(GUT_STAGE_SCAN, s, slot));
    GRUT_CHECK(inclusive_scan_u32(s, N, proj.tiles_count, rank_to_particle, h->offsets.as<uint32_t>(), h->scan_scratch.ptr,
                                  h->scan_scratch.bytes));
    GRUT_CHECK(h->stage_end(GUT_STAGE_SCAN, s, slot));
    GRUT_CHECK(h->ranges.ensure((size_t)tiles * 8 + 8));
    launch_prepare_tail(s, h->offsets.as<uint32_t>() + (N - 1), d_counters + 1, h->host_counters, h->ranges.as<uint32_t>(), tiles * 2u,
                        h->ck_reached.as<uint32_t>(), h->ck_reached.ptr ? h->ck_boundaries_capacity : 0u);
    GRUT_HIP(hipEventRecord(h->count_event, s));
    const uint32_t tile_mask = (h->stats.key_bits >= 32) ? 0xFFFFFFFFu : ((1u << h->stats.key_bits) - 1u);
    bool first_tail = true;
    auto enqueue_tail = [&](uint32_t n, const uint32_t* n_dev) -> int {
        GRUT_CHECK(h->stage_begin(GUT_STAGE_EXPAND, s, slot));
        launch_expand(s, P, proj, rank_to_particle, h->offsets.as<uint32_t>(), n, h->tile_keys.as<uint32_t>(),
                      direct ? h->tile_vals.as<uint32_t>() : nullptr , h->pos_particle.as<uint32_t>());
        GRUT_CHECK(h->stage_end(GUT_STAGE_EXPAND, s, slot));
        GRUT_CHECK(h->stage_begin(GUT_STAGE_TILE_SORT, s, slot));
        uint32_t *sorted_tiles = nullptr, *sorted_idx = nullptr;
        GRUT_CHECK(sort_pairs_u32(s, n, n_dev, 0, (int)h->stats.key_bits, h->tile_keys.as<uint32_t>(), h->tile_vals.as<uint32_t>(),
                                  h->tile_keys_tmp.as<uint32_t>(), h->tile_vals_tmp.as<uint32_t>(), h->tile_sort_scratch.ptr,
                                  h->tile_sort_scratch.bytes, &sorted_tiles, &sorted_idx, !direct));
        h->sorted_tile_keys = sorted_tiles;
        h->params.sorted_keys = sorted_tiles;
        h->sorted_pos = sorted_idx;
        GRUT_CHECK(h->stage_end(GUT_STAGE_TILE_SORT, s, slot));
        GRUT_CHECK(h->stage_begin(GUT_STAGE_TILE_RANGES, s, slot));
        if (!first_tail) {
            GRUT_HIP(hipMemsetAsync(h->ranges.ptr, 0, (size_t)tiles * 8, s));
            GRUT_HIP(hipMemsetAsync(h->ck_reached.ptr, 0, (size_t)h->ck_boundaries_capacity * 4, s));
        }
        first_tail = false;
        launch_tile_ranges(s, n, n_dev, tile_mask, tiles, sorted_tiles, h->ranges.as<uint32_t>(), h->checkpoints.boundary_tile);
        GRUT_CHECK(h->stage_end(GUT_STAGE_TILE_RANGES, s, slot));
        GRUT_CHECK(h->stage_begin(GUT_STAGE_RENDER_FWD, s, slot));
        if (nht_fast_path(P))
            launch_render_nhtp_fwd(s, P, h->ranges.as<uint32_t>(), sorted_idx, h->pos_particle.as<uint32_t>(), particle_density, particle_sph, ray_origin,
                                   ray_direction, out_feat_density, out_hit_distance, out_hit_count, h->ck_nht.ptr, h->checkpoints, true);
        else if (P.nht)
            launch_render_nht_fwd(s, P, h->ranges.as<uint32_t>(), sorted_idx, h->pos_particle.as<uint32_t>(), particle_density, particle_sph, ray_origin,
                                  ray_direction, out_feat_density, out_hit_distance, out_hit_count);
        else if (P.k_buffer > 0)
            launch_render_k_fwd(s, P, h->ranges.as<uint32_t>(), sorted_idx, h->pos_particle.as<uint32_t>(), particle_density, proj.rgb, ray_origin,
                                ray_direction, out_feat_density, out_hit_distance, out_hit_count);
        else
            launch_render_fwd(s, P, h->ranges.as<uint32_t>(), sorted_idx, h->pos_particle.as<uint32_t>(), particle_density, proj.rgb, ray_origin,
                              ray_direction, out_feat_density, out_hit_distance, out_hit_count, h->checkpoints, true);
        GRUT_CHECK(h->stage_end(GUT_STAGE_RENDER_FWD, s, slot));
        return GRUT_OK;
    };
    const bool speculative = h->tile_capacity > 0;
    if (speculative) GRUT_CHECK(enqueue_tail(h->tile_capacity, h->offsets.as<uint32_t>() + (N - 1)));
    GRUT_HIP(hipEventSynchronize(h->count_event));
    const uint32_t I = h->host_counters[0];
    h->stats.num_visible = h->host_counters[1];
    h->stats.num_intersections = I;
    h->num_intersections = I;
    if (I == 0) {
        const float far = 1e6f;
        uint32_t bits;
        memcpy(&bits, &far, 4);
        GRUT_HIP(hipMemsetAsync(out_feat_density, 0, (size_t)P.W * P.H * (P.nht ? P.nht_ray_dim + 1 : 4) * (P.out_half ? 2 : 4), s));
        GRUT_HIP(hipMemsetD32Async(reinterpret_cast<hipDeviceptr_t>(out_hit_distance), (int)bits, (size_t)P.W * P.H, s));
        GRUT_HIP(hipMemsetAsync(out_hit_count, 0, (size_t)P.W * P.H * 4, s));
        if (P.out_features) GRUT_HIP(hipMemsetAsync(P.out_features, 0, (size_t)P.W * P.H * 12, s));
        if (P.out_opacity) GRUT_HIP(hipMemsetAsync(P.out_opacity, 0, (size_t)P.W * P.H * 4, s));
        if (h->cfg.enable_kernel_timings) GRUT_CHECK(h->fwd_timer.end(s));
        h->have_forward = true;
        return GRUT_OK;
    }
    if (!speculative || I > h->tile_capacity) {
        GRUT_CHECK(ensure_intersection_scratch(h, I + I / 2, tiles));
        first_tail = false;
        GRUT_CHECK(enqueue_tail(I, nullptr));
    }
    h->checkpoints.num_boundaries = I / kGutSegment + 1;
    GRUT_HIP(hipGetLastError());
    if (h->cfg.enable_kernel_timings) GRUT_CHECK(h->fwd_timer.end(s));
    h->have_forward = true;
    return GRUT_OK;
}

static int backward_impl(GutHandle* h, void* stream_, const GutFrame* frame, const float* particle_density, const void* particle_sph_,
                         const float* ray_origin, const float* ray_direction, const void* feat_density_, const float* grad_feat_density,
                         const float* hit_distance, const float* grad_hit_distance, float* grad_particle_density, float* grad_particle_sph,
                         float* grad_radiance, const GutGradIO* io = nullptr, uint32_t num_chunks = 1, GrutChunkFn on_chunk = nullptr,
                         void* chunk_user = nullptr) {
    const float* particle_sph = reinterpret_cast<const float*>(particle_sph_);
    const float* feat_density = reinterpret_cast<const float*>(feat_density_);
    GRUT_REQUIRE(h && frame, "gut_backward: null handle/frame");
    hipStream_t s = reinterpret_cast<hipStream_t>(stream_);
    ScratchStreamScope scratch_scope(s);
    if (!h->have_forward || h->fwd_stream != s) {
        set_last_error("gut_backward: no forward context on this stream");
        return GRUT_ERR_NOT_READY;
    }
    const GutParams& P = h->params;
    GRUT_REQUIRE(frame->num_particles == P.N && frame->width == P.W && frame->height == P.H, "gut_backward: frame differs from the forward frame");
    if (frame->frame_id != h->fwd_frame_id || (P.N > 0 && (particle_density != h->fwd_density || ray_origin != h->fwd_ray_o || ray_direction != h->fwd_ray_d))) {
        set_last_error("gut_backward: the forward context belongs to another forward (a later gut_forward ran on this handle before this "
                       "backward); run each backward before the next forward, or use one handle per in-flight frame");
        return GRUT_ERR_NOT_READY;
    }
    if (P.N == 0) return GRUT_OK;
    if (P.nht) {
        if (grad_radiance) {
            set_last_error("gut_backward_factored: neural harmonic features have no per-view factorisation; reduce the dense gradients");
            return GRUT_ERR_UNSUPPORTED;
        }
        const bool fast = nht_fast_path(P);
        if (io && !fast) {
            set_last_error("gut_backward_unpacked: this feature shape runs on the generic kernels, which write packed gradients only");
            return GRUT_ERR_UNSUPPORTED;
        }
        GRUT_REQUIRE(particle_density && particle_sph && feat_density && (io || grad_feat_density) && hit_distance && (io || grad_particle_density) &&
                         grad_particle_sph, "gut_backward: null buffer");
        if (h->cfg.enable_kernel_timings) GRUT_CHECK(h->bwd_timer.begin(s));
        GRUT_HIP(hipMemsetAsync(grad_particle_sph, 0, (size_t)P.N * P.nht_k * 4, s));
        const size_t I = h->num_intersections;
        if (fast) {
            const int slot = h->prof_fwd_slot;
            const GutProjected proj = projected_view(h);
            const GutGradOut g_out = io ? GutGradOut{nullptr, io->grad_positions, io->grad_density, io->grad_rotation, io->grad_scale}
                                        : GutGradOut{grad_particle_density, nullptr, nullptr, nullptr, nullptr};
            if (io) {
                GRUT_REQUIRE(io->grad_positions && io->grad_density && io->grad_rotation && io->grad_scale, "gut_backward_unpacked: null gradient output");
                GRUT_REQUIRE((reinterpret_cast<uintptr_t>(io->grad_rotation) & 15u) == 0, "gut_backward_unpacked: grad_rotation must be 16-byte aligned");
            }
            GutGradSlots slots;
            slots.stride = 16;
            slots.partial = nullptr;
            slots.flag = nullptr;
            slots.pos_particle = h->pos_particle.as<uint32_t>();
            if (I > 0) {
                GRUT_CHECK(h->grad_partial.ensure(2 * I * (size_t)slots.stride * 4, 1.3f));
                GRUT_CHECK(h->grad_flag.ensure(2 * I + 96, 1.3f));
                slots.partial = h->grad_partial.as<float>();
                slots.flag = h->grad_flag.as<uint8_t>();
                GRUT_HIP(hipMemsetAsync(slots.flag, 0, 2 * I, s));
                GRUT_CHECK(h->stage_begin(GUT_STAGE_RENDER_BWD, s, slot));
                launch_render_nhtp_bwd(s, P, h->ranges.as<uint32_t>(), h->sorted_pos, particle_density, particle_sph, ray_origin, ray_direction, feat_density,
                                       io ? nullptr : grad_feat_density, io ? io->grad_features : nullptr, io ? io->grad_opacity : nullptr, hit_distance,
                                       grad_hit_distance, slots, grad_particle_sph, h->ck_nht.ptr, h->checkpoints);
                GRUT_CHECK(h->stage_end(GUT_STAGE_RENDER_BWD, s, slot));
            }
            GRUT_CHECK(h->stage_begin(GUT_STAGE_PROJECT_BWD, s, slot));
            launch_grad_finalize_nht(s, P, proj, particle_density, slots, I > 0, g_out);
            GRUT_CHECK(h->stage_end(GUT_STAGE_PROJECT_BWD, s, slot));
        } else {
            GRUT_HIP(hipMemsetAsync(grad_particle_density, 0, (size_t)P.N * 48, s));
            if (I > 0)
                launch_render_nht_bwd(s, P, h->ranges.as<uint32_t>(), h->sorted_pos, h->pos_particle.as<uint32_t>(), particle_density, particle_sph, ray_origin,
                                      ray_direction, feat_density, grad_feat_density, hit_distance, grad_hit_distance, grad_particle_density, grad_particle_sph);
        }
        GRUT_HIP(hipGetLastError());
        if (h->cfg.enable_kernel_timings) GRUT_CHECK(h->bwd_timer.end(s));
        return GRUT_OK;
    }
    const GutGradIn g_in = io ? GutGradIn{nullptr, io->grad_features, io->grad_opacity} : GutGradIn{grad_feat_density, nullptr, nullptr};
    const GutGradOut g_out = io ? GutGradOut{nullptr, io->grad_positions, io->grad_density, io->grad_rotation, io->grad_scale}
                                : GutGradOut{grad_particle_density, nullptr, nullptr, nullptr, nullptr};
    if (io) {
        GRUT_REQUIRE(io->grad_positions && io->grad_density && io->grad_rotation && io->grad_scale, "gut_backward_unpacked: null gradient output");
        GRUT_REQUIRE((reinterpret_cast<uintptr_t>(io->grad_rotation) & 15u) == 0, "gut_backward_unpacked: grad_rotation must be 16-byte aligned");
        if (P.k_buffer > 0) {
            set_last_error("gut_backward_unpacked: the sorted (k_buffer_size > 0) backward accumulates into packed rows; use gut_backward");
            return GRUT_ERR_UNSUPPORTED;
        }
    }
    GRUT_REQUIRE(particle_density && particle_sph && feat_density && (io || grad_feat_density) && hit_distance && (io || grad_particle_density) &&
                     (grad_particle_sph || grad_radiance), "gut_backward: null buffer");
    if (h->cfg.enable_kernel_timings) GRUT_CHECK(h->bwd_timer.begin(s));
    const GutProjected proj = projected_view(h);
    const int slot = h->prof_fwd_slot;
    const bool has_gdist = grad_hit_distance != nullptr;
    GutGradSlots slots;
    slots.stride = has_gdist ? 20 : 16;
    slots.partial = nullptr;
    slots.flag = nullptr;
    slots.pos_particle = h->pos_particle.as<uint32_t>();
    const size_t I = h->num_intersections;
    if (P.k_buffer > 0) {
        GRUT_CHECK(h->g_rgb.ensure((size_t)P.N * 12, 1.25f));
        GRUT_HIP(hipMemsetAsync(h->g_rgb.ptr, 0, (size_t)P.N * 12, s));
        GRUT_HIP(hipMemsetAsync(grad_particle_density, 0, (size_t)P.N * 48, s));
        if (I > 0) {
            GRUT_CHECK(h->stage_begin(GUT_STAGE_RENDER_BWD, s, slot));
            launch_render_k_bwd(s, P, h->ranges.as<uint32_t>(), h->sorted_pos, h->pos_particle.as<uint32_t>(), particle_density, proj.rgb, ray_origin,
                                ray_direction, feat_density, grad_feat_density, hit_distance, grad_hit_distance, grad_particle_density,
                                h->g_rgb.as<float>());
            GRUT_CHECK(h->stage_end(GUT_STAGE_RENDER_BWD, s, slot));
        }
        GRUT_CHECK(h->stage_begin(GUT_STAGE_PROJECT_BWD, s, slot));
        launch_project_bwd(s, P, proj, particle_density, particle_sph, h->g_rgb.as<float>(), g_out, grad_particle_sph, grad_radiance);
        GRUT_CHECK(h->stage_end(GUT_STAGE_PROJECT_BWD, s, slot));
        GRUT_HIP(hipGetLastError());
        if (h->cfg.enable_kernel_timings) GRUT_CHECK(h->bwd_timer.end(s));
        return GRUT_OK;
    }
    if (I > 0) {
        GRUT_CHECK(h->grad_partial.ensure(2 * I * (size_t)slots.stride * 4, 1.3f));
        GRUT_CHECK(h->grad_flag.ensure(2 * I + 96, 1.3f));
        slots.partial = h->grad_partial.as<float>();
        slots.flag = h->grad_flag.as<uint8_t>();
        GRUT_HIP(hipMemsetAsync(slots.flag, 0, 2 * I, s));
        GRUT_CHECK(h->stage_begin(GUT_STAGE_RENDER_BWD, s, slot));
        launch_render_bwd(s, P, h->ranges.as<uint32_t>(), h->sorted_pos, particle_density, proj.rgb, ray_origin, ray_direction, feat_density,
                          g_in, hit_distance, grad_hit_distance, slots, h->checkpoints);
        GRUT_CHECK(h->stage_end(GUT_STAGE_RENDER_BWD, s, slot));
    }
    GRUT_CHECK(h->stage_begin(GUT_STAGE_PROJECT_BWD, s, slot));
    GRUT_CHECK(h->g_rgb.ensure((size_t)P.N * 12, 1.25f));
    if (num_chunks <= 1 || !on_chunk) {
        launch_grad_finalize(s, P, proj, particle_density, particle_sph, slots, has_gdist, I > 0, h->g_rgb.as<float>(), g_out,
                             grad_particle_sph, grad_radiance);
    } else {
        const uint32_t per = ((P.N + num_chunks - 1) / num_chunks + 127u) & ~127u;
        uint32_t c = 0;
        for (uint32_t first = 0; first < P.N; first += per, ++c) {
            const uint32_t end = first + per < P.N ? first + per : P.N;
            launch_grad_finalize(s, P, proj, particle_density, particle_sph, slots, has_gdist, I > 0, h->g_rgb.as<float>(), g_out,
                                 grad_particle_sph, grad_radiance, first, end);
            on_chunk(chunk_user, c, first, end - first);
        }
    }
    GRUT_CHECK(h->stage_end(GUT_STAGE_PROJECT_BWD, s, slot));
    GRUT_HIP(hipGetLastError());
    if (h->cfg.enable_kernel_timings) GRUT_CHECK(h->bwd_timer.end(s));
    return GRUT_OK;
}

int gut_backward(GutHandle* h, void* stream, const GutFrame* frame, const float* particle_density, const void* particle_sph,
                 const float* ray_origin, const float* ray_direction, const void* feat_density, const float* grad_feat_density,
                 const float* hit_distance, const float* grad_hit_distance, float* grad_particle_density, float* grad_particle_sph) {
    return backward_impl(h, stream, frame, particle_density, particle_sph, ray_origin, ray_direction, feat_density, grad_feat_density, hit_distance,
                         grad_hit_distance, grad_particle_density, grad_particle_sph, nullptr);
}

int gut_backward_unpacked(GutHandle* h, void* stream, const GutFrame* frame, const float* particle_density, const void* particle_sph,
                          const float* ray_origin, const float* ray_direction, const void* feat_density, const float* hit_distance,
                          const float* grad_hit_distance, const GutGradIO* io, float* grad_particle_sph) {
    GRUT_REQUIRE(io, "gut_backward_unpacked: null GutGradIO");
    return backward_impl(h, stream, frame, particle_density, particle_sph, ray_origin, ray_direction, feat_density, nullptr, hit_distance,
                         grad_hit_distance, nullptr, grad_particle_sph, nullptr, io);
}

int gut_backward_factored(GutHandle* h, void* stream, const GutFrame* frame, const float* particle_density, const void* particle_sph,
                          const float* ray_origin, const float* ray_direction, const void* feat_density, const float* grad_feat_density,
                          const float* hit_distance, const float* grad_hit_distance, float* grad_particle_density, float* grad_radiance) {
    GRUT_REQUIRE(grad_radiance, "gut_backward_factored: null buffer");
    return backward_impl(h, stream, frame, particle_density, particle_sph, ray_origin, ray_direction, feat_density, grad_feat_density, hit_distance,
                         grad_hit_distance, grad_particle_density, nullptr, grad_radiance);
}

int gut_backward_factored_chunked(GutHandle* h, void* stream, const GutFrame* frame, const float* particle_density, const void* particle_sph,
                                  const float* ray_origin, const float* ray_direction, const void* feat_density, const float* grad_feat_density,
                                  const float* hit_distance, const float* grad_hit_distance, float* grad_particle_density, float* grad_radiance,
                                  uint32_t num_chunks, GrutChunkFn on_chunk, void* user) {
    GRUT_REQUIRE(grad_radiance && on_chunk && num_chunks >= 1, "gut_backward_factored_chunked: null buffer / callback");
    GRUT_REQUIRE(!h || h->cfg.k_buffer_size == 0, "gut_backward_factored_chunked: the sorted mode finalises in one piece");
    return backward_impl(h, stream, frame, particle_density, particle_sph, ray_origin, ray_direction, feat_density, grad_feat_density, hit_distance,
                         grad_hit_distance, grad_particle_density, nullptr, grad_radiance, nullptr, num_chunks < 2 ? 2 : num_chunks, on_chunk, user);
}

int grut_sph_grad_from_views(void* stream, uint32_t num_particles, uint32_t num_views, const float* view_factors, const float* positions,
                             uint32_t position_stride, int32_t n_active_features, int32_t sph_degree, float scale, float* grad_particle_sph) {
    GRUT_REQUIRE(num_views > 0 && sph_degree >= 0 && sph_degree <= 3 && position_stride >= 3, "grut_sph_grad_from_views: bad arguments");
    if (num_particles == 0) return GRUT_OK;
    GRUT_REQUIRE(view_factors && positions && grad_particle_sph, "grut_sph_grad_from_views: null buffer");
    launch_sph_grad_from_views(reinterpret_cast<hipStream_t>(stream), num_particles, num_views, view_factors, positions, position_stride,
                               n_active_features, (sph_degree + 1) * (sph_degree + 1), scale, grad_particle_sph);
    GRUT_HIP(hipGetLastError());
    return GRUT_OK;
}

int gut_timings(GutHandle* h, float* forward_ms, float* backward_ms) {
    GRUT_REQUIRE(h, "gut_timings: null handle");
    if (forward_ms) *forward_ms = h->fwd_timer.collect();
    if (backward_ms) *backward_ms = h->bwd_timer.collect();
    return GRUT_OK;
}

int gut_profile_enable(GutHandle* h, int enable) {
    GRUT_REQUIRE(h, "gut_profile_enable: null handle");
    if (enable && h->prof_created == 0) {
        for (int r = 0; r < GutHandle::kProfRing; ++r)
            for (int st = 0; st < GUT_NUM_STAGES; ++st) {
                GRUT_HIP(hipEventCreate(&h->prof_ev[r][st][0]));
                GRUT_HIP(hipEventCreate(&h->prof_ev[r][st][1]));
                h->prof_used[r][st] = false;
            }
        h->prof_created = 1;
    }
    h->profile = enable != 0;
    h->count_work = enable >= 2;
    return GRUT_OK;
}

int gut_profile_select(GutHandle* h, uint32_t stage_mask) {
    GRUT_REQUIRE(h, "gut_profile_select: null handle");
    h->profile_mask = stage_mask;
    return GRUT_OK;
}

int gut_profile_read(GutHandle* h, float* stage_ms) {
    GRUT_REQUIRE(h && stage_ms, "gut_profile_read: null argument");
    GRUT_REQUIRE(h->prof_created, "gut_profile_read: profiling was never enabled");
    for (int st = 0; st < GUT_NUM_STAGES; ++st) {
        double sum = 0;
        int n = 0;
        for (int r = 0; r < GutHandle::kProfRing; ++r) {
            if (!h->prof_used[r][st]) continue;
            float ms = 0.f;
            GRUT_HIP(hipEventSynchronize(h->prof_ev[r][st][1]));
            GRUT_HIP(hipEventElapsedTime(&ms, h->prof_ev[r][st][0], h->prof_ev[r][st][1]));
            sum += ms;
            n++;
            h->prof_used[r][st] = false;
        }
        stage_ms[st] = n ? (float)(sum / n) : -1.f;
    }
    h->prof_slot = 0;
    return GRUT_OK;
}

int gut_stats(GutHandle* h, GutStats* stats) {
    GRUT_REQUIRE(h && stats, "gut_stats: null argument");
    if (h->work_pending && h->work_counters.ptr) {
        std::vector<unsigned long long> all(h->work_counters.bytes / 8);
        GRUT_HIP(hipMemcpyAsync(all.data(), h->work_counters.ptr, all.size() * 8, hipMemcpyDeviceToHost, h->fwd_stream));
        GRUT_HIP(hipStreamSynchronize(h->fwd_stream));
        for (int k = 0; k < 4; ++k) h->work_host[k] = all[k];
        const size_t n_fwd = (((size_t)h->params.gx * h->params.gy + 7) & ~(size_t)7) * 2;
        for (size_t b = 0; b < n_fwd && 16 + 4 * b + 3 < all.size(); ++b) {
            h->work_host[0] += all[16 + 4 * b + 2] & 0xFFFFFFFFull;
            h->work_host[1] += all[16 + 4 * b + 2] >> 32;
        }
        h->work_pending = false;
    }
    *stats = h->stats;
    stats->fwd_entries_evaluated = h->count_work ? h->work_host[0] : 0;
    stats->fwd_entries_accepted = h->count_work ? h->work_host[1] : 0;
    stats->bwd_entries_evaluated = h->count_work ? h->work_host[2] : 0;
    stats->bwd_entries_accepted = h->count_work ? h->work_host[3] : 0;
    return GRUT_OK;
}

int gut_debug_fetch_work(GutHandle* h, void* stream_, unsigned long long* out, uint64_t count) {
    GRUT_REQUIRE(h && out, "gut_debug_fetch_work: null argument");
    GRUT_REQUIRE(h->work_counters.ptr && count * 8 <= h->work_counters.bytes, "gut_debug_fetch_work: no instrumented frame / count too large");
    GRUT_HIP(hipMemcpyAsync(out, h->work_counters.ptr, count * 8, hipMemcpyDeviceToDevice, reinterpret_cast<hipStream_t>(stream_)));
    return GRUT_OK;
}

int gut_debug_fetch(GutHandle* h, void* stream_, uint32_t* tiles_count, float* proj_pos, float* conic_opacity, float* extent,
                    float* depth, float* rgb, uint32_t* sorted_particle_idx, uint32_t* tile_ranges) {
    GRUT_REQUIRE(h && h->have_forward, "gut_debug_fetch: no forward context");
    hipStream_t s = reinterpret_cast<hipStream_t>(stream_);
// ... 22 lines not shown
```

3dgrut_amd/csrc/gut_internal.hpp:

```cpp
#pragma once

#include "camera.hpp"
#include "common.hpp"

namespace grut {

struct GutParams {
    int degree;
    float min_response, min_alpha, max_alpha, min_transmittance;
    int n_active, ncoef, hitcounts;
    float ut_w0m, ut_wi, ut_w0c, ut_delta, ut_margin;
    int ut_require_all, n_rs_iter, k_buffer, global_z, rect_bounding, tight_opacity, tile_culling;
    int W, H, gx, gy;
    uint32_t N;
    GrutCamera cam;
    FramePoses poses;
    unsigned long long* work;
    const float4* rec64;
    const uint32_t* sorted_keys;
    uint32_t ord_shift;
    int nht, nht_k, nht_ipd, nht_support, nht_act, nht_nf, nht_ray_dim;
    int sph_half, out_half;
    uint32_t work_task_capacity;
    float* out_features;
    float* out_opacity;
    const FramePoses* poses_dev;
};
#ifdef __HIPCC__
__device__ __forceinline__ const FramePoses& frame_poses(const GutParams& P) { return P.poses_dev ? *P.poses_dev : P.poses; }
#endif
void launch_frame_poses(hipStream_t s, const float* T_start, const float* T_end, FramePoses* out);
void launch_prepare_tail(hipStream_t s, const uint32_t* last_offset, uint32_t* num_visible, uint32_t* host_counters, uint32_t* ranges_words,
                         uint32_t n_ranges_words, uint32_t* reached_words, uint32_t n_reached_words);

struct GutProjected {
    uint32_t* tiles_count;
    float2* proj_pos;
    float4* conic_opacity;
    float2* extent;
    float* depth;
    float* rgb;
    uint32_t* depth_key;
    uint32_t* particle_idx;
    uint32_t* part_offset;
    float4* rec64;
    uint2* walk8;
};

struct GutGradSlots {
    float* partial;
    uint8_t* flag;
    const uint32_t* pos_particle;
    int stride;
};

struct GutGradOut {
    float* packed;
    float* pos;
    float* dns;
    float* rot;
    float* scl;
};
struct GutGradIn {
    const float* fd;
    const float* rgb;
    const float* opa;
};
#ifdef __HIPCC__
__device__ __forceinline__ float4 load_grad_in(const GutGradIn& g, size_t pix) {
    if (g.fd) return reinterpret_cast<const float4*>(g.fd)[pix];
    float4 r = make_float4(0.f, 0.f, 0.f, 0.f);
    if (g.rgb) { r.x = g.rgb[3 * pix]; r.y = g.rgb[3 * pix + 1]; r.z = g.rgb[3 * pix + 2]; }
    if (g.opa) r.w = g.opa[pix];
    return r;
}
#endif

#ifndef GRUT_GUT_SEGMENT
#define GRUT_GUT_SEGMENT 64
#endif
constexpr uint32_t kGutSegment = GRUT_GUT_SEGMENT;

struct GutCheckpoints {
    float4* tc;
    float* d;
    uint8_t* reached;
    uint32_t* boundary_tile;
    uint32_t num_boundaries;
};

constexpr uint32_t kGutCounterReplicas = 64, kGutCounterStride = 32, kGutCounterWords = kGutCounterReplicas * kGutCounterStride + 32;
void launch_project(hipStream_t s, const GutParams& P, const float* density12, const float* sph, const GutProjected& out,
                    int32_t* visibility, uint32_t* num_visible);
void launch_expand(hipStream_t s, const GutParams& P, const GutProjected& proj, const uint32_t* rank_to_particle,
                   const uint32_t* offsets, uint32_t capacity, uint32_t* tile_keys, uint32_t* tile_vals, uint32_t* pos_particle);
void launch_gather_particle_idx(hipStream_t s, uint32_t n, const uint32_t* sorted_pos, const uint32_t* pos_particle, uint32_t* out);
void launch_tile_ranges(hipStream_t s, uint32_t n, const uint32_t* n_dev, uint32_t tile_mask, uint32_t num_tiles,
                        const uint32_t* sorted_tile_keys, uint32_t* ranges, uint32_t* boundary_tile);
void launch_render_fwd(hipStream_t s, const GutParams& P, const uint32_t* ranges, const uint32_t* sorted_pos, const uint32_t* pos_particle,
                       const float* density12,
                       const float* rgb, const float* ray_o, const float* ray_d, float* out_fd, float* out_dist, float* out_cnt,
                       const GutCheckpoints& ck, bool write_checkpoints);
void launch_render_bwd(hipStream_t s, const GutParams& P, const uint32_t* ranges, const uint32_t* sorted_pos, const float* density12,
                       const float* rgb, const float* ray_o, const float* ray_d, const float* fd, const GutGradIn& g_fd, const float* dist,
                       const float* g_dist, const GutGradSlots& slots, const GutCheckpoints& ck);
void launch_render_nht_fwd(hipStream_t s, const GutParams& P, const uint32_t* ranges, const uint32_t* sorted_pos, const uint32_t* pos_particle,
                           const float* density12, const float* features, const float* ray_o, const float* ray_d, float* out_fd, float* out_dist,
                           float* out_cnt);
void launch_render_nht_bwd(hipStream_t s, const GutParams& P, const uint32_t* ranges, const uint32_t* sorted_pos, const uint32_t* pos_particle,
                           const float* density12, const float* features, const float* ray_o, const float* ray_d, const float* fd, const float* g_fd,
                           const float* dist, const float* g_dist, float* g_density12, float* g_features);
bool nht_fast_path(const GutParams& P);
uint64_t nht_checkpoint_bytes(uint32_t num_boundaries);
void launch_render_nhtp_fwd(hipStream_t s, const GutParams& P, const uint32_t* ranges, const uint32_t* sorted_pos, const uint32_t* pos_particle,
                            const float* density12, const float* features, const float* ray_o, const float* ray_d, float* out_fd, float* out_dist,
                            float* out_cnt, void* ck_nht, const GutCheckpoints& ck, bool write_checkpoints);
void launch_render_nhtp_bwd(hipStream_t s, const GutParams& P, const uint32_t* ranges, const uint32_t* sorted_pos, const float* density12,
                            const float* features, const float* ray_o, const float* ray_d, const float* fd, const float* g_fd, const float* g_feat,
                            const float* g_opa, const float* dist, const float* g_dist, const GutGradSlots& slots, float* g_features,
                            const void* ck_nht, const GutCheckpoints& ck);
void launch_grad_finalize_nht(hipStream_t s, const GutParams& P, const GutProjected& proj, const float* density12, const GutGradSlots& slots,
                              bool have_partials, const GutGradOut& g_out);
void launch_render_k_fwd(hipStream_t s, const GutParams& P, const uint32_t* ranges, const uint32_t* sorted_pos, const uint32_t* pos_particle,
                         const float* density12, const float* rgb, const float* ray_o, const float* ray_d, float* out_fd, float* out_dist,
                         float* out_cnt);
void launch_render_k_bwd(hipStream_t s, const GutParams& P, const uint32_t* ranges, const uint32_t* sorted_pos, const uint32_t* pos_particle,
                         const float* density12, const float* rgb, const float* ray_o, const float* ray_d, const float* fd, const float* g_fd,
                         const float* dist, const float* g_dist, float* g_density12, float* g_rgb);
void launch_project_bwd(hipStream_t s, const GutParams& P, const GutProjected& proj, const float* density12, const float* sph,
                        const float* g_rgb, const GutGradOut& g_out, float* g_sph, float* g_radiance, uint32_t first = 0u, uint32_t end = 0xFFFFFFFFu);
void launch_grad_finalize(hipStream_t s, const GutParams& P, const GutProjected& proj, const float* density12, const float* sph,
                          const GutGradSlots& slots, bool has_gdist, bool have_partials, float* g_rgb, const GutGradOut& g_out, float* g_sph,
                          float* g_radiance, uint32_t first = 0u, uint32_t end = 0xFFFFFFFFu);
void launch_sph_grad_from_views(hipStream_t s, uint32_t N, uint32_t n_views, const float* factors, const float* positions, uint32_t pos_stride,
                                int n_active, int ncoef, float scale, float* g_sph);

}
```

3dgrut_amd/csrc/gut_kernels.hip:

```cpp
#include <cstdlib>

#include <hip/hip_fp16.h>

#include "gut_internal.hpp"

namespace grut {

namespace {

#define GRUT_SH_CONSTANTS                                                                                                   \
    constexpr float kC0 = 0.28209479177387814f, kC1 = 0.4886025119029199f;                                                  \
    constexpr float kC2[5] = {1.0925484305920792f, -1.0925484305920792f, 0.31539156525252005f, -1.0925484305920792f,        \
                              0.5462742152960396f};                                                                         \
    constexpr float kC3[7] = {-0.5900435899266435f, 2.890611442640554f, -0.4570457994644658f, 0.3731763325901154f,          \
                              -0.4570457994644658f, 1.445305721320277f, -0.5900435899266435f};                               \
    (void)kC0; (void)kC1; (void)kC2; (void)kC3

__device__ __forceinline__ void sh_basis(int deg, f3 d, float b[16]) {
    GRUT_SH_CONSTANTS;
    const float x = d.x, y = d.y, z = d.z;
#pragma unroll
    for (int i = 0; i < 16; ++i) b[i] = 0.f;
    b[0] = kC0;
    if (deg > 0) {
// ... 560 lines not shown
        const TileConic sco = {bcast_f(tc.cx, src), bcast_f(tc.cy, src), bcast_f(tc.cz, src), bcast_f(tc.rcpx, src), bcast_f(tc.rcpy, src)};
        const uint32_t sp = (uint32_t)bcast_i((int)p, src), send = (uint32_t)bcast_i((int)max_off, src);
        uint32_t o = (uint32_t)bcast_i((int)off, src);
        const uint32_t o0 = o;
        coop_tile_walk(lane, P.gx, culling, sb, sco, bcast_f(cx, src), bcast_f(cy, src), bcast_f(pmax, src),
                       [&](bool keep, uint32_t tile) {
                           const unsigned long long m = __ballot(keep);
                           const uint32_t slot = o + (uint32_t)__popcll(m & lt_mask);
                           if (keep && slot < send) emit_entry(direct, osh, tile_keys, tile_vals, pos_particle, slot, slot - o0, tile, sp);
                           o += (uint32_t)__popcll(m);
                       });
        for (uint32_t q = o + lane; q < send; q += 64) emit_padding(direct, tile_keys, tile_vals, pos_particle, q);
    }
}

__global__ __launch_bounds__(256) void gut_gather_particle_idx_kernel(uint32_t n, const uint32_t* __restrict__ sorted_pos,
                                                                      const uint32_t* __restrict__ pos_particle, uint32_t* __restrict__ out) {
    const uint32_t k = blockIdx.x * blockDim.x + threadIdx.x;
    if (k < n) out[k] = pos_particle ? pos_particle[sorted_pos[k]] : sorted_pos[k];
}

__global__ __launch_bounds__(256) void gut_tile_ranges_kernel(uint32_t n_cap, const uint32_t* __restrict__ n_dev, uint32_t tile_mask,
                                                              uint32_t num_tiles, const uint32_t* __restrict__ sorted_tile_keys,
                                                              uint2* __restrict__ ranges, uint32_t* __restrict__ boundary_tile) {
    const uint32_t k0 = (blockIdx.x * blockDim.x + threadIdx.x) * 4u;
    const uint32_t n = n_dev ? min(n_cap, *n_dev) : n_cap;
    if (k0 >= n) return;
    uint32_t key[4];
    if (k0 + 4u <= n) {
        const uint4 v = *reinterpret_cast<const uint4*>(sorted_tile_keys + k0);
        key[0] = v.x; key[1] = v.y; key[2] = v.z; key[3] = v.w;
    } else {
#pragma unroll
        for (int j = 0; j < 4; ++j) key[j] = (k0 + j < n) ? sorted_tile_keys[k0 + j] : 0u;
    }
    uint32_t pt = k0 ? (sorted_tile_keys[k0 - 1] & tile_mask) : 0xFFFFFFFFu;
#pragma unroll
    for (int j = 0; j < 4; ++j) {
        const uint32_t k = k0 + j;
        if (k >= n) break;
        const uint32_t t = key[j] & tile_mask;
        const bool valid = t < num_tiles;
        if ((k % kGutSegment) == 0) boundary_tile[k / kGutSegment] = valid ? t : 0xFFFFFFFFu;
        if (k == 0) {
            if (valid) ranges[t].x = 0;
        } else if (pt != t) {
            if (pt < num_tiles) ranges[pt].y = k;
            if (valid) ranges[t].x = k;
        }
        if (valid && k == n - 1) ranges[t].y = n;
        pt = t;
    }
}

constexpr uint32_t kGatherSmall = 32;
struct __attribute__((packed, aligned(2))) FlagChunk {
    unsigned long long lo, hi;
};

__device__ __forceinline__ float4 quat_contract(const float m[9], float4 q2) {
    const float r = q2.x, x = q2.y, y = q2.z, z = q2.w;
    const float m00 = m[0], m01 = m[1], m02 = m[2], m10 = m[3], m11 = m[4], m12 = m[5], m20 = m[6], m21 = m[7], m22 = m[8];
    const float s01 = m01 + m10, s02 = m02 + m20, s12 = m12 + m21;
    const float a01 = m01 - m10, a02 = m20 - m02, a12 = m12 - m21;
    float4 d;
    d.x = z * a01 + y * a02 + x * a12;
    d.y = y * s01 + z * s02 + r * a12 - 2.f * x * (m11 + m22);
    d.z = x * s01 + z * s12 + r * a02 - 2.f * y * (m00 + m22);
    d.w = x * s02 + y * s12 + r * a01 - 2.f * z * (m00 + m11);
    return d;
}

template <int STRIDE>
struct QuadAcc {
    float4 a;
    float4 x;
    __device__ __forceinline__ void clear() { a = make_float4(0.f, 0.f, 0.f, 0.f); x = a; }
    __device__ __forceinline__ void add_rows4(const float* __restrict__ partial, size_t sb, int b0, int b1, int b2, int b3, int c) {
        const float4 z = make_float4(0.f, 0.f, 0.f, 0.f);
        const float4* r0 = reinterpret_cast<const float4*>(partial + (sb + (size_t)b0) * STRIDE);
        const float4* r1 = reinterpret_cast<const float4*>(partial + (sb + (size_t)(b1 < 0 ? b0 : b1)) * STRIDE);
        const float4* r2 = reinterpret_cast<const float4*>(partial + (sb + (size_t)(b2 < 0 ? b0 : b2)) * STRIDE);
        const float4* r3 = reinterpret_cast<const float4*>(partial + (sb + (size_t)(b3 < 0 ? b0 : b3)) * STRIDE);
        const float4 v0 = r0[c], v1 = r1[c], v2 = r2[c], v3 = r3[c];
        float4 w0 = z, w1 = z, w2 = z, w3 = z;
        if (STRIDE > 16 && c == 0) { w0 = r0[4]; w1 = r1[4]; w2 = r2[4]; w3 = r3[4]; }
        a.x += v0.x; a.y += v0.y; a.z += v0.z; a.w += v0.w;
        if (b1 >= 0) { a.x += v1.x; a.y += v1.y; a.z += v1.z; a.w += v1.w; }
        if (b2 >= 0) { a.x += v2.x; a.y += v2.y; a.z += v2.z; a.w += v2.w; }
        if (b3 >= 0) { a.x += v3.x; a.y += v3.y; a.z += v3.z; a.w += v3.w; }
        if (STRIDE > 16 && c == 0) {
            x.x += w0.x; x.y += w0.y; x.z += w0.z; x.w += w0.w;
            if (b1 >= 0) { x.x += w1.x; x.y += w1.y; x.z += w1.z; x.w += w1.w; }
            if (b2 >= 0) { x.x += w2.x; x.y += w2.y; x.z += w2.z; x.w += w2.w; }
            if (b3 >= 0) { x.x += w3.x; x.y += w3.y; x.z += w3.z; x.w += w3.w; }
        }
    }
    __device__ __forceinline__ void add_row(const float* __restrict__ partial, size_t slot, int c) {
        const float4* row = reinterpret_cast<const float4*>(partial + slot * STRIDE);
        const float4 v = row[c];
        a.x += v.x; a.y += v.y; a.z += v.z; a.w += v.w;
        if (STRIDE > 16 && c == 0) {
            const float4 w = row[4];
            x.x += w.x; x.y += w.y; x.z += w.z; x.w += w.w;
        }
    }
};
template <int J>
__device__ __forceinline__ float quad_bcast(float v) {
    return __int_as_float(__builtin_amdgcn_update_dpp(0, __float_as_int(v), J | (J << 2) | (J << 4) | (J << 6), 0xf, 0xf, false));
}
template <int X>
__device__ __forceinline__ float quad_bcast_xor(float v) {
    constexpr int perm = X == 1 ? (1 | (0 << 2) | (3 << 4) | (2 << 6)) : (2 | (3 << 2) | (0 << 4) | (1 << 6));
    return __int_as_float(__builtin_amdgcn_update_dpp(0, __float_as_int(v), perm, 0xf, 0xf, false));
}
__device__ __forceinline__ float xor_sum_quads(float v) {
    v += __shfl_xor(v, 4, 64);
    v += __shfl_xor(v, 8, 64);
    v += __shfl_xor(v, 16, 64);
    v += __shfl_xor(v, 32, 64);
    return v;
}

template <int STRIDE, bool NHT = false, bool FUSE_SH = false>
__global__ __launch_bounds__(256) void gut_grad_gather_kernel(GutParams P, GutProjected proj, const float4* __restrict__ density12,
                                                              GutGradSlots slots, int have_partials, GutGradOut g_out,
                                                              float* __restrict__ g_rgb, uint32_t first, uint32_t end,
                                                              const float* __restrict__ sph = nullptr, float* __restrict__ g_sph = nullptr) {
    const int lane = threadIdx.x & 63, c = threadIdx.x & 3;
    const uint32_t i = first + blockIdx.x * 64u + (threadIdx.x >> 2);
    const uint32_t count = (i < end) ? proj.tiles_count[i] : 0u;
    const bool has = count != 0;
    QuadAcc<STRIDE> acc;
    acc.clear();
    const uint32_t off = has ? proj.part_offset[i] : 0u;
    float4 q = make_float4(1.f, 0.f, 0.f, 0.f), sc = make_float4(1.f, 1.f, 1.f, 0.f);
    if (has) { q = density12[3 * (size_t)i + 1]; sc = density12[3 * (size_t)i + 2]; }
    float4 sh0 = make_float4(0.f, 0.f, 0.f, 0.f), sh1 = sh0, sh2 = sh0, pa = sh0;
    f3 rad = mk3(0.f, 0.f, 0.f);
    if (FUSE_SH && has) {
        const float4* row = reinterpret_cast<const float4*>(sph + 48 * (size_t)i) + 3 * c;
        sh0 = row[0]; sh1 = row[1]; sh2 = row[2];
        pa = density12[3 * (size_t)i];
        rad = mk3(proj.rgb[3 * (size_t)i], proj.rgb[3 * (size_t)i + 1], proj.rgb[3 * (size_t)i + 2]);
    }
    if (have_partials) {
        if (has && count <= kGatherSmall) {
            const size_t s0 = 2 * (size_t)off;
            const uint32_t nb = 2 * count;
            for (uint32_t base = 0; base < nb; base += 64) {
                const FlagChunk* fc = reinterpret_cast<const FlagChunk*>(slots.flag + s0 + base);
                const FlagChunk w0 = fc[0], w1 = fc[1], w2 = fc[2], w3 = fc[3];
                constexpr unsigned long long kPack = 0x0102040810204080ull, kLsb = 0x0101010101010101ull;
                auto pack8 = [](unsigned long long w) { return ((w & kLsb) * kPack) >> 56; };
                unsigned long long m = pack8(w0.lo) | (pack8(w0.hi) << 8) | (pack8(w1.lo) << 16) | (pack8(w1.hi) << 24) |
                                       (pack8(w2.lo) << 32) | (pack8(w2.hi) << 40) | (pack8(w3.lo) << 48) | (pack8(w3.hi) << 56);
                const uint32_t rem = nb - base;
                if (rem < 64) m &= (1ull << rem) - 1ull;
                const size_t sb = s0 + base;
                while (m) {
                    const int b0 = __ffsll((long long)m) - 1;
                    m &= m - 1;
                    const int b1 = m ? __ffsll((long long)m) - 1 : -1;
                    m &= m - 1;
                    const int b2 = m ? __ffsll((long long)m) - 1 : -1;
                    m &= m - 1;
                    const int b3 = m ? __ffsll((long long)m) - 1 : -1;
                    m &= m - 1;
                    acc.add_rows4(slots.partial, sb, b0, b1, b2, b3, c);
                }
            }
        }
        unsigned long long big = __ballot(has && count > kGatherSmall && c == 0);
        while (big) {
            const int src = __ffsll((long long)big) - 1;
            big &= big - 1;
            const size_t s0 = 2 * (size_t)(uint32_t)__builtin_amdgcn_readlane((int)off, src);
            const uint32_t n2 = 2u * (uint32_t)__builtin_amdgcn_readlane((int)count, src);
            QuadAcc<STRIDE> part;
            part.clear();
            const int g = lane >> 2;
            for (uint32_t base = 0; base < n2; base += 64) {
                const bool set = (base + (uint32_t)lane < n2) && slots.flag[s0 + base + lane] != 0;
                const unsigned long long m = __ballot(set);
                if (m == 0) continue;
                int b[4], nb = 0;
#pragma unroll
                for (int j = 0; j < 4; ++j)
                    if ((m >> (g + 16 * j)) & 1ull) b[nb++] = g + 16 * j;
                if (nb > 0)
                    part.add_rows4(slots.partial, s0 + base, b[0], nb > 1 ? b[1] : -1, nb > 2 ? b[2] : -1, nb > 3 ? b[3] : -1, c);
            }
            part.a.x = xor_sum_quads(part.a.x); part.a.y = xor_sum_quads(part.a.y);
            part.a.z = xor_sum_quads(part.a.z); part.a.w = xor_sum_quads(part.a.w);
            if (STRIDE > 16) {
                part.x.x = xor_sum_quads(part.x.x); part.x.y = xor_sum_quads(part.x.y);
                part.x.z = xor_sum_quads(part.x.z); part.x.w = xor_sum_quads(part.x.w);
            }
            if ((lane >> 2) == (src >> 2)) acc = part;
        }
    }
    float r[20];
    r[0] = quad_bcast<0>(acc.a.x); r[1] = quad_bcast<0>(acc.a.y); r[2] = quad_bcast<0>(acc.a.z); r[3] = quad_bcast<0>(acc.a.w);
    r[4] = quad_bcast<1>(acc.a.x); r[5] = quad_bcast<1>(acc.a.y); r[6] = quad_bcast<1>(acc.a.z); r[7] = quad_bcast<1>(acc.a.w);
    r[8] = quad_bcast<2>(acc.a.x); r[9] = quad_bcast<2>(acc.a.y); r[10] = quad_bcast<2>(acc.a.z); r[11] = quad_bcast<2>(acc.a.w);
    r[12] = quad_bcast<3>(acc.a.x); r[13] = quad_bcast<3>(acc.a.y); r[14] = quad_bcast<3>(acc.a.z); r[15] = quad_bcast<3>(acc.a.w);
    r[16] = quad_bcast<0>(acc.x.x); r[17] = quad_bcast<0>(acc.x.y); r[18] = quad_bcast<0>(acc.x.z); r[19] = 0.f;
    if (i >= end) return;
    float4* gd = reinterpret_cast<float4*>(g_out.packed + 12 * (size_t)i);
    if (FUSE_SH && !has) {
        float4* out = reinterpret_cast<float4*>(g_sph + 48 * (size_t)i) + 3 * c;
        out[0] = out[1] = out[2] = make_float4(0.f, 0.f, 0.f, 0.f);
    }
    if (!has) {
        if (g_out.packed) {
            if (c < 3) gd[c] = make_float4(0.f, 0.f, 0.f, 0.f);
        } else if (c == 0) {
            g_out.pos[3 * (size_t)i] = 0.f; g_out.pos[3 * (size_t)i + 1] = 0.f; g_out.pos[3 * (size_t)i + 2] = 0.f;
            g_out.dns[i] = 0.f;
        } else if (c == 1) {
            reinterpret_cast<float4*>(g_out.rot)[i] = make_float4(0.f, 0.f, 0.f, 0.f);
        } else if (c == 2) {
            g_out.scl[3 * (size_t)i] = 0.f; g_out.scl[3 * (size_t)i + 1] = 0.f; g_out.scl[3 * (size_t)i + 2] = 0.f;
        }
        return;
    }
    const m3 rt = quat_wxyz_to_rotT(q.x, q.y, q.z, q.w);
    const f3 B = mk3(r[0], r[1], r[2]);
    const float* m = &r[4];
    const f3 gpos = mk3(-(B.x * rt.r0.x + B.y * rt.r1.x + B.z * rt.r2.x), -(B.x * rt.r0.y + B.y * rt.r1.y + B.z * rt.r2.y),
                        -(B.x * rt.r0.z + B.y * rt.r1.z + B.z * rt.r2.z));
    float gsx = -(rt.r0.x * m[0] + rt.r0.y * m[1] + rt.r0.z * m[2]) / sc.x;
    float gsy = -(rt.r1.x * m[3] + rt.r1.y * m[4] + rt.r1.z * m[5]) / sc.y;
    float gsz = -(rt.r2.x * m[6] + rt.r2.y * m[7] + rt.r2.z * m[8]) / sc.z;
    if (STRIDE > 16) { gsx += r[16]; gsy += r[17]; gsz += r[18]; }
    if (NHT) { gsx += r[13]; gsy += r[14]; gsz += r[15]; }
    const float4 dq = quat_contract(m, make_float4(2.f * q.x, 2.f * q.y, 2.f * q.z, 2.f * q.w));
    f3 gpos_out = gpos;
    if (FUSE_SH) {
        const FramePoses& FP = frame_poses(P);
        const int nact = min((P.n_active + 1) * (P.n_active + 1), P.ncoef);
        float ilen;
        const f3 dir = sh_view_direction(mk3(pa.x, pa.y, pa.z), mk3(FP.s2w_t[0], FP.s2w_t[1], FP.s2w_t[2]), ilen);
        f3 g = mk3(r[13], r[14], r[15]);
        if (!(rad.x > 0.f)) g.x = 0.f;
        if (!(rad.y > 0.f)) g.y = 0.f;
        if (!(rad.z > 0.f)) g.z = 0.f;
        const float rowv[12] = {sh0.x, sh0.y, sh0.z, sh0.w, sh1.x, sh1.y, sh1.z, sh1.w, sh2.x, sh2.y, sh2.z, sh2.w};
        float o[12];
        f3 gdir = mk3(0.f, 0.f, 0.f);
        auto part = [&](auto group) {
            constexpr int G = decltype(group)::value;
            float basis[16];
            f3 dbasis[16];
            sh_basis_pinned(P.n_active, dir, basis);
            sh_basis_grad_pinned(P.n_active, dir, dbasis);
#pragma unroll
            for (int j = 0; j < 4; ++j) {
                const bool on = 4 * G + j < nact;
                o[3 * j] = o[3 * j + 1] = o[3 * j + 2] = 0.f;
                if (on) {
                    const float s = sh_row_dot(g, rowv[3 * j], rowv[3 * j + 1], rowv[3 * j + 2]);
                    gdir = sh_axpy(gdir, dbasis[4 * G + j], s);
                    o[3 * j] = mul_rn(basis[4 * G + j], g.x); o[3 * j + 1] = mul_rn(basis[4 * G + j], g.y); o[3 * j + 2] = mul_rn(basis[4 * G + j], g.z);
                }
            }
        };
        switch (c) {
        case 0: part(std::integral_constant<int, 0>{}); break;
        case 1: part(std::integral_constant<int, 1>{}); break;
        case 2: part(std::integral_constant<int, 2>{}); break;
        default: part(std::integral_constant<int, 3>{}); break;
        }
        gdir = sh_sum(gdir, mk3(quad_bcast_xor<1>(gdir.x), quad_bcast_xor<1>(gdir.y), quad_bcast_xor<1>(gdir.z)));
        gdir = sh_sum(gdir, mk3(quad_bcast_xor<2>(gdir.x), quad_bcast_xor<2>(gdir.y), quad_bcast_xor<2>(gdir.z)));
        const f3 gsh = sh_position_gradient(dir, ilen, gdir);
        gpos_out = mk3(add_rn(gpos.x, gsh.x), add_rn(gpos.y, gsh.y), add_rn(gpos.z, gsh.z));
        float4* out = reinterpret_cast<float4*>(g_sph + 48 * (size_t)i) + 3 * c;
        out[0] = make_float4(o[0], o[1], o[2], o[3]);
        out[1] = make_float4(o[4], o[5], o[6], o[7]);
        out[2] = make_float4(o[8], o[9], o[10], o[11]);
    }
    if (FUSE_SH) {
        if (c == 0) {
            if (g_out.packed) gd[0] = make_float4(gpos_out.x, gpos_out.y, gpos_out.z, r[3]);
            else {
                g_out.pos[3 * (size_t)i] = gpos_out.x; g_out.pos[3 * (size_t)i + 1] = gpos_out.y; g_out.pos[3 * (size_t)i + 2] = gpos_out.z;
                g_out.dns[i] = r[3];
            }
        } else if (c == 1) {
            if (g_out.packed) gd[1] = dq;
            else reinterpret_cast<float4*>(g_out.rot)[i] = dq;
        } else if (c == 2) {
            if (g_out.packed) gd[2] = make_float4(gsx, gsy, gsz, 0.f);
            else { g_out.scl[3 * (size_t)i] = gsx; g_out.scl[3 * (size_t)i + 1] = gsy; g_out.scl[3 * (size_t)i + 2] = gsz; }
        }
        return;
    }
    if (c == 0) {
        if (g_out.packed) gd[0] = make_float4(gpos.x, gpos.y, gpos.z, r[3]);
        else {
            g_out.pos[3 * (size_t)i] = gpos.x; g_out.pos[3 * (size_t)i + 1] = gpos.y; g_out.pos[3 * (size_t)i + 2] = gpos.z;
            g_out.dns[i] = r[3];
        }
    } else if (c == 1) {
        if (g_out.packed) gd[1] = dq;
        else reinterpret_cast<float4*>(g_out.rot)[i] = dq;
    } else if (c == 2) {
        if (g_out.packed) gd[2] = make_float4(gsx, gsy, gsz, 0.f);
        else { g_out.scl[3 * (size_t)i] = gsx; g_out.scl[3 * (size_t)i + 1] = gsy; g_out.scl[3 * (size_t)i + 2] = gsz; }
    } else if (!NHT) {
        g_rgb[3 * (size_t)i] = r[13];
        g_rgb[3 * (size_t)i + 1] = r[14];
        g_rgb[3 * (size_t)i + 2] = r[15];
    }
}

constexpr int kShStride = 49;
template <bool FACTORED>
__global__ __launch_bounds__(128) void gut_project_bwd_kernel(GutParams P, const uint32_t* __restrict__ tiles_count,
                                                              const float4* __restrict__ density12, const float* __restrict__ sph,
                                                              const float* __restrict__ rgb, const float* __restrict__ g_rgb,
                                                              GutGradOut g_out, float* __restrict__ g_sph,
                                                              float* __restrict__ g_radiance, uint32_t first, uint32_t end) {
    __shared__ float s_rows[2][64 * kShStride];
    const int wave = threadIdx.x >> 6, lane = threadIdx.x & 63;
    const uint32_t wave_base = first + blockIdx.x * 128u + (uint32_t)wave * 64u;
    const uint32_t i = wave_base + lane;
    const int rowlen = 3 * P.ncoef;
    const int nact = min((P.n_active + 1) * (P.n_active + 1), P.ncoef);
    float* rows = s_rows[wave];
    const FramePoses& FP = frame_poses(P);
    const bool has = (i < end) && (tiles_count[i] != 0);
    const unsigned long long has_mask = __ballot(has);
    const int nrows = (int)min(64u, end > wave_base ? end - wave_base : 0u);
    if (P.sph_half) {
// ... 247 lines not shown
```

3dgrut_amd/csrc/gut_render.hip:

```cpp
#include <hip/hip_fp16.h>

#include "gut_internal.hpp"
#ifndef GRUT_RENDER_PART
#define GRUT_RENDER_PART 2
#endif

#ifndef GRUT_BWD_FULL_REDUCE
#define GRUT_BWD_FULL_REDUCE 2
#endif
#ifndef GRUT_BWD_WAVES
#define GRUT_BWD_WAVES 4
#endif

namespace grut {

namespace {

struct Ray {
    f3 o, d;
    float tmin, tmax;
    bool valid;
    bool inside;
};
__device__ __forceinline__ void swapf(float& a, float& b) { const float t = a; a = b; b = t; }
// ... 727 lines not shown
            const v2f ioma = prcp(oma);
            const v2f inextT_raw = iT * ioma;
            const v2f inextT = psel(nextT.x <= P.min_transmittance, nextT.y <= P.min_transmittance, splat(0.f), inextT_raw);
            const v2f resTrm = psel(alpha.x < 0.999999f, alpha.y < 0.999999f, T_fin * ioma, T);
            v2f dalpha = -(resTrm * gT);
            const p3 dc = p3{gC.x * weight, gC.y * weight, gC.z * weight};
            Cr = pfma(r4.x, weight, Cr); Cg = pfma(r4.y, weight, Cg); Cb = pfma(r4.z, weight, Cb);
            const v2f rr = pmax0((C_fin.x - Cr) * inextT), rg = pmax0((C_fin.y - Cg) * inextT), rb = pmax0((C_fin.z - Cb) * inextT);
            dalpha = pfma(T, pfma(r4.x - rr, gC.x, pfma(r4.y - rg, gC.y, (r4.z - rb) * gC.z)), dalpha);

            const v2f vu = pdot(g.v, g.u);
            const v2f t = vu * il2;
            const p3 a = p3{pfma(-t, g.v.x, g.u.x), pfma(-t, g.v.y, g.u.y), pfma(-t, g.v.z, g.u.z)};
            p3 dl;
            if (UNI) dl = p3{splat(rp.origin.x - r0.w), splat(rp.origin.y - r1.w), splat(rp.origin.z - r2.w)};
            else dl = p3{rp.o.x - r0.w, rp.o.y - r1.w, rp.o.z - r2.w};

            p3 uX = p3{splat(0.f), splat(0.f), splat(0.f)}, vX = uX, sX = uX;
            if (HAS_GDIST) {
                const v2f il = v2f{__builtin_amdgcn_rsqf(g.l2.x), __builtin_amdgcn_rsqf(g.l2.y)};
                const p3 nrm = p3{g.v.x * il, g.v.y * il, g.v.z * il};
                const v2f nu = vu * il;
                const v2f pdt = -nu;
                const p3 gscl = p3{prcp(splat(r3.x)), prcp(splat(r3.y)), prcp(splat(r3.z))};
                const p3 grdd = p3{nrm.x * pdt, nrm.y * pdt, nrm.z * pdt};
                const p3 grds = p3{gscl.x * grdd.x, gscl.y * grdd.y, gscl.z * grdd.z};
                const v2f gsq = pdot(grds, grds);
                const v2f gdist = v2f{__builtin_amdgcn_sqrtf(gsq.x), __builtin_amdgcn_sqrtf(gsq.y)};
                D = pfma(weight, gdist, D);
                const v2f resHitT = pmax0((D_fin - D) * inextT);
                dalpha = pfma((gdist - resHitT) * T, gD, dalpha);
                const v2f k = psel(gsq.x > 0.f, gsq.y > 0.f, weight * prcp(gdist) * gD, splat(0.f));
                const p3 grdsGrd = p3{grds.x * k, grds.y * k, grds.z * k};
                sX = p3{grdd.x * grdsGrd.x, grdd.y * grdsGrd.y, grdd.z * grdsGrd.z};
                const p3 sg = p3{gscl.x * grdsGrd.x, gscl.y * grdsGrd.y, gscl.z * grdsGrd.z};
                const v2f sd = pdot(sg, nrm);
                const p3 nGrd = p3{pfma(sg.x, pdt, -(g.u.x * sd)), pfma(sg.y, pdt, -(g.u.y * sd)), pfma(sg.z, pdt, -(g.u.z * sd))};
                uX = p3{-(nrm.x * sd), -(nrm.y * sd), -(nrm.z * sd)};
                const v2f ng = pdot(nrm, nGrd);
                vX = p3{(nGrd.x - nrm.x * ng) * il, (nGrd.y - nrm.y * ng) * il, (nGrd.z - nrm.z * ng) * il};
            }

            dalpha = psel(h0, h1, dalpha, splat(0.f));
            const v2f dn = resp * dalpha;
            const v2f dresp = r3.w * dalpha;
            const v2f wg2 = psel(h0, h1, 2.f * v2f{particle_response_grd<DEG>(gray.x, resp.x, dresp.x),
                                                    particle_response_grd<DEG>(gray.y, resp.y, dresp.y)}, splat(0.f));
            p3 uGrd = p3{a.x * wg2, a.y * wg2, a.z * wg2};
            float terms[16], extra[16];
            if (!HAS_GDIST) {
                const p3 B = p3{r3.x * uGrd.x, r3.y * uGrd.y, r3.z * uGrd.z};
                p3 e;
                v2f s;
                if (UNI) { e = rp.d; s = -t; }
                else { e = p3{pfma(-t, rp.d.x, dl.x), pfma(-t, rp.d.y, dl.y), pfma(-t, rp.d.z, dl.z)}; s = splat(1.f); }
                const p3 Bs = p3{B.x * s, B.y * s, B.z * s};
                const v2f m[9] = {Bs.x * e.x, Bs.x * e.y, Bs.x * e.z, Bs.y * e.x, Bs.y * e.y, Bs.y * e.z, Bs.z * e.x, Bs.z * e.y, Bs.z * e.z};
                terms[0] = B.x.x + B.x.y; terms[1] = B.y.x + B.y.y; terms[2] = B.z.x + B.z.y; terms[3] = dn.x + dn.y;
#pragma unroll
                for (int k = 0; k < 9; ++k) terms[4 + k] = m[k].x + m[k].y;
                terms[13] = dc.x.x + dc.x.y; terms[14] = dc.y.x + dc.y.y; terms[15] = dc.z.x + dc.z.y;
            } else {
                const v2f mt = psel(h0, h1, splat(1.f), splat(0.f));
                uGrd = p3{pfma(uX.x, mt, uGrd.x), pfma(uX.y, mt, uGrd.y), pfma(uX.z, mt, uGrd.z)};
                const p3 vGrd = p3{pfma(vX.x, mt, -(t * a.x * wg2)), pfma(vX.y, mt, -(t * a.y * wg2)), pfma(vX.z, mt, -(t * a.z * wg2))};
                const p3 B = p3{r3.x * uGrd.x, r3.y * uGrd.y, r3.z * uGrd.z};
                const p3 Bv = p3{r3.x * vGrd.x, r3.y * vGrd.y, r3.z * vGrd.z};
                const v2f m[9] = {pfma(B.x, dl.x, Bv.x * rp.d.x), pfma(B.x, dl.y, Bv.x * rp.d.y), pfma(B.x, dl.z, Bv.x * rp.d.z),
                                  pfma(B.y, dl.x, Bv.y * rp.d.x), pfma(B.y, dl.y, Bv.y * rp.d.y), pfma(B.y, dl.z, Bv.y * rp.d.z),
                                  pfma(B.z, dl.x, Bv.z * rp.d.x), pfma(B.z, dl.y, Bv.z * rp.d.y), pfma(B.z, dl.z, Bv.z * rp.d.z)};
                terms[0] = B.x.x + B.x.y; terms[1] = B.y.x + B.y.y; terms[2] = B.z.x + B.z.y; terms[3] = dn.x + dn.y;
#pragma unroll
                for (int k = 0; k < 9; ++k) terms[4 + k] = m[k].x + m[k].y;
                terms[13] = dc.x.x + dc.x.y; terms[14] = dc.y.x + dc.y.y; terms[15] = dc.z.x + dc.z.y;
                const p3 sXm = p3{sX.x * mt, sX.y * mt, sX.z * mt};
#pragma unroll
                for (int k = 0; k < 16; ++k) extra[k] = 0.f;
                extra[0] = sXm.x.x + sXm.x.y; extra[1] = sXm.y.x + sXm.y.y; extra[2] = sXm.z.x + sXm.z.y;
            }
#if GRUT_BWD_FULL_REDUCE == 2
            {
#pragma unroll
                for (int k = 0; k < 16; ++k) s_tr[k * 65 + lane] = terms[k];
                __builtin_amdgcn_fence(__ATOMIC_RELEASE, "workgroup");
                __builtin_amdgcn_wave_barrier();
                const float* col = &s_tr[(lane & 15) * 65 + (lane >> 4) * 16];
                float part = col[0];
#pragma unroll
                for (int k = 1; k < 16; ++k) part += col[k];
                typedef unsigned v2u __attribute__((ext_vector_type(2)));
                const v2u sa = __builtin_amdgcn_permlane32_swap(__float_as_uint(part), __float_as_uint(part), false, false);
                const float s2 = __uint_as_float(sa.x) + __uint_as_float(sa.y);
                const v2u sb = __builtin_amdgcn_permlane16_swap(__float_as_uint(s2), __float_as_uint(s2), false, false);
                const float tot = __uint_as_float(sb.x) + __uint_as_float(sb.y);
                if (lane < 16) s_acc[j * 16 + lane] = tot;
                __builtin_amdgcn_wave_barrier();
            }
            if (HAS_GDIST) {
                const float tot2 = wave_reduce_scatter16_all(extra, lane);
                if (lane < 16) s_acc2[j * 16 + lane] = tot2;
            }
#elif GRUT_BWD_FULL_REDUCE
            const float tot = wave_reduce_scatter16_all(terms, lane);
            if (lane < 16) s_acc[j * 16 + lane] = tot;
            if (HAS_GDIST) {
                const float tot2 = wave_reduce_scatter16_all(extra, lane);
                if (lane < 16) s_acc2[j * 16 + lane] = tot2;
            }
#else
            s_acc[j * 64 + lane] = wave_reduce_scatter16_rows(terms, lane);
            if (HAS_GDIST) s_acc2[j * 64 + lane] = wave_reduce_scatter16_rows(extra, lane);
#endif
            T = nextT;
            iT = inextT_raw;
            alive0 = alive0 && !(T.x < P.min_transmittance);
            alive1 = alive1 && !(T.y < P.min_transmittance);
        }
        __syncthreads();
        if (lane < (int)kBatch && ((hit_entries >> lane) & 1u)) {
            const float4* rec = &s_rec[lane * kRecQuads];
            const uint32_t pos = __float_as_uint(rec[5].w);
#if GRUT_BWD_FULL_REDUCE
            const float4* acc = reinterpret_cast<const float4*>(&s_acc[lane * 16]);
            float4 a0 = acc[0], a1 = acc[1], a2 = acc[2], a3 = acc[3];
#else
            const float4* acc = reinterpret_cast<const float4*>(&s_acc[lane * 64]);
            float4 a0 = acc[0], a1 = acc[1], a2 = acc[2], a3 = acc[3];
#pragma unroll
            for (int r = 1; r < 4; ++r) {
                const float4 b0 = acc[4 * r], b1 = acc[4 * r + 1], b2 = acc[4 * r + 2], b3 = acc[4 * r + 3];
                a0.x += b0.x; a0.y += b0.y; a0.z += b0.z; a0.w += b0.w; a1.x += b1.x; a1.y += b1.y; a1.z += b1.z; a1.w += b1.w;
                a2.x += b2.x; a2.y += b2.y; a2.z += b2.z; a2.w += b2.w; a3.x += b3.x; a3.y += b3.y; a3.z += b3.z; a3.w += b3.w;
            }
#endif
            if (!HAS_GDIST && UNI) {
                const float4 r0 = rec[0], r1 = rec[1], r2 = rec[2];
                const f3 dl = rp.origin - mk3(r0.w, r1.w, r2.w);
                a1.x += a0.x * dl.x; a1.y += a0.x * dl.y; a1.z += a0.x * dl.z;
                a1.w += a0.y * dl.x; a2.x += a0.y * dl.y; a2.y += a0.y * dl.z;
                a2.z += a0.z * dl.x; a2.w += a0.z * dl.y; a3.x += a0.z * dl.z;
            }
            const size_t slot = 2 * (size_t)pos + half;
            float4* out = reinterpret_cast<float4*>(slots.partial + slot * (HAS_GDIST ? 20 : 16));
            out[0] = a0; out[1] = a1; out[2] = a2; out[3] = a3;
            if (HAS_GDIST) {
                float ex = 0.f, ey = 0.f, ez = 0.f;
#if GRUT_BWD_FULL_REDUCE
                ex = s_acc2[lane * 16]; ey = s_acc2[lane * 16 + 1]; ez = s_acc2[lane * 16 + 2];
#else
                for (int r = 0; r < 4; ++r) { ex += s_acc2[lane * 64 + 16 * r]; ey += s_acc2[lane * 64 + 16 * r + 1]; ez += s_acc2[lane * 64 + 16 * r + 2]; }
#endif
                out[4] = make_float4(ex, ey, ez, 0.f);
            }
            slots.flag[slot] = 1;
        }
        __syncthreads();
        b = bend;
    }
    if (COUNT && P.work && lane == 0) { atomicAdd(&P.work[2], (unsigned long long)n_eval); atomicAdd(&P.work[3], (unsigned long long)n_acc); }
}

template <int DEG, bool HAS_GDIST, bool COUNT = false>
#if GRUT_BWD_WAVES
__global__ __launch_bounds__(64) __attribute__((amdgpu_waves_per_eu(HAS_GDIST ? 3 : GRUT_BWD_WAVES, HAS_GDIST ? 3 : GRUT_BWD_WAVES))) void gut_render_bwd_kernel(
#else
__global__ __launch_bounds__(64) void gut_render_bwd_kernel(
#endif
                                                            GutParams P, const uint2* __restrict__ ranges, EntryLists lists,
                                                            const float4* __restrict__ density12, const float* __restrict__ rgb,
                                                            const float* __restrict__ ray_o, const float* __restrict__ ray_d,
                                                            const float4* __restrict__ fd, GutGradIn g_in,
                                                            const float* __restrict__ dist, const float* __restrict__ g_dist,
                                                            GutGradSlots slots, GutCheckpoints ck) {
    constexpr uint32_t kBatch = kBwdBatch;
    __shared__ float4 s_rec[kBatch * kRecQuads];
#if GRUT_BWD_FULL_REDUCE == 2
    __shared__ float s_tr[16 * 65];
#else
    float* s_tr = nullptr;
#endif
#if GRUT_BWD_FULL_REDUCE
    __shared__ float s_acc[kBatch * 16];
    __shared__ float s_acc2[HAS_GDIST ? kBatch * 16 : 1];
#else
    __shared__ float s_acc[kBatch * 64];
    __shared__ float s_acc2[HAS_GDIST ? kBatch * 64 : 1];
#endif
    const uint32_t num_tiles = (uint32_t)(P.gx * P.gy), bnd_pad = (ck.num_boundaries + 7u) & ~7u;
    uint32_t vtile, half;
    half_mapping(blockIdx.x, vtile, half);
    uint32_t tile, seg_begin;
    bool from_checkpoint = false;
    uint32_t boundary = 0, reached_bits = 3u;
#ifndef GRUT_BWD_TASK_STRIDE
#define GRUT_BWD_TASK_STRIDE 0
#endif
    if (vtile >= bnd_pad) {
        tile = vtile - bnd_pad;
        if (tile >= num_tiles) return;
        seg_begin = ranges[tile].x;
    } else {
        boundary = GRUT_BWD_TASK_STRIDE > 1 ? stride_permute(vtile, bnd_pad, GRUT_BWD_TASK_STRIDE) : vtile;
        if (boundary == 0 || boundary >= ck.num_boundaries) return;
        reached_bits = ck.reached[(size_t)boundary * 2 + half];
        if (!reached_bits) return;
        tile = ck.boundary_tile[boundary];
        if (tile >= num_tiles) return;
        seg_begin = boundary * kGutSegment;
        if (seg_begin <= ranges[tile].x) return;
        from_checkpoint = true;
    }
    const int lane = threadIdx.x;
    const uint32_t seg_end = min(ranges[tile].y, (seg_begin / kGutSegment + 1u) * kGutSegment);
    const unsigned long long t_begin = COUNT ? wall_clock64() : 0ull;
    const RayPair rp = init_ray_pair(P, ray_o, ray_d, tile, half, lane);
    bool alive0 = rp.valid0, alive1 = rp.valid1;

    v2f T = splat(1.f), D = splat(0.f), Cr = splat(0.f), Cg = splat(0.f), Cb = splat(0.f);
    v2f T_fin = splat(0.f), D_fin = splat(0.f), gT = splat(0.f), gD = splat(0.f);
    p3 C_fin = p3{splat(0.f), splat(0.f), splat(0.f)}, gC = C_fin;
    if (alive0) {
        const size_t pix = (size_t)rp.py0 * P.W + rp.px;
        const float4 f = load_fd(P, fd, pix), g = load_grad_in(g_in, pix);
        C_fin.x.x = f.x; C_fin.y.x = f.y; C_fin.z.x = f.z; gC.x.x = g.x; gC.y.x = g.y; gC.z.x = g.z;
        T_fin.x = 1.f - f.w; gT.x = -g.w;
        if (HAS_GDIST) { D_fin.x = dist[pix]; gD.x = g_dist[pix]; }
    }
    if (alive1) {
        const size_t pix = (size_t)rp.py1 * P.W + rp.px;
        const float4 f = load_fd(P, fd, pix), g = load_grad_in(g_in, pix);
        C_fin.x.y = f.x; C_fin.y.y = f.y; C_fin.z.y = f.z; gC.x.y = g.x; gC.y.y = g.y; gC.z.y = g.z;
        T_fin.y = 1.f - f.w; gT.y = -g.w;
        if (HAS_GDIST) { D_fin.y = dist[pix]; gD.y = g_dist[pix]; }
    }
    if (from_checkpoint) {
        const size_t slot = (((size_t)boundary * 2 + half) * 64 + lane) * 2;
        const float4 zero4 = make_float4(0.f, 0.f, 0.f, 0.f);
        const float4 c0 = (reached_bits & 1u) ? ck.tc[slot] : zero4, c1 = (reached_bits & 2u) ? ck.tc[slot + 1] : zero4;
        T = v2f{c0.x, c1.x}; Cr = v2f{c0.y, c1.y}; Cg = v2f{c0.z, c1.z}; Cb = v2f{c0.w, c1.w};
        if (HAS_GDIST) D = v2f{(reached_bits & 1u) ? ck.d[slot] : 0.f, (reached_bits & 2u) ? ck.d[slot + 1] : 0.f};
        alive0 = alive0 && !(T.x < P.min_transmittance);
        alive1 = alive1 && !(T.y < P.min_transmittance);
    }

    BwdPixels px{T, D, Cr, Cg, Cb, T_fin, D_fin, gT, gD, C_fin, gC, alive0, alive1};
    if (rp.uniform_origin)
        render_bwd_sweep<DEG, HAS_GDIST, true, COUNT>(P, rp, seg_begin, seg_end, lane, half, lists, density12, rgb, slots, s_rec, s_acc, s_acc2, s_tr, px);
    else
        render_bwd_sweep<DEG, HAS_GDIST, false, COUNT>(P, rp, seg_begin, seg_end, lane, half, lists, density12, rgb, slots, s_rec, s_acc, s_acc2, s_tr, px);
    if (COUNT && P.work && lane == 0) {
        const size_t gid = (size_t)atomicAdd(&P.work[8], 1ull);
        const size_t base = 16 + 4 * (size_t)(((num_tiles + 7u) & ~7u) * 2u) + 2 * gid;
        if (gid < P.work_task_capacity) {
            P.work[base] = wall_clock64() - t_begin;
            P.work[base + 1] = t_begin;
        }
    }
}

__device__ __forceinline__ float gray_limit_rt(int deg, float x) {
    switch (deg) {
    case 8: return response_gray_limit<8>(x);
    case 5: return response_gray_limit<5>(x);
    case 4: return response_gray_limit<4>(x);
    case 3: return response_gray_limit<3>(x);
    case 1: return response_gray_limit<1>(x);
    case 0: return response_gray_limit<0>(x);
    default: return response_gray_limit<2>(x);
    }
}
__device__ __forceinline__ float response_rt(int deg, float g) {
    switch (deg) {
    case 8: return particle_response<8>(g);
    case 5: return particle_response<5>(g);
    case 4: return particle_response<4>(g);
    case 3: return particle_response<3>(g);
    case 1: return particle_response<1>(g);
    case 0: return particle_response<0>(g);
    default: return particle_response<2>(g);
    }
}
__device__ __forceinline__ float response_grd_rt(int deg, float g, float gres, float gresGrd) {
    switch (deg) {
    case 8: return particle_response_grd<8>(g, gres, gresGrd);
    case 5: return particle_response_grd<5>(g, gres, gresGrd);
    case 4: return particle_response_grd<4>(g, gres, gresGrd);
    case 3: return particle_response_grd<3>(g, gres, gresGrd);
    case 1: return particle_response_grd<1>(g, gres, gresGrd);
    case 0: return particle_response_grd<0>(g, gres, gresGrd);
    default: return particle_response_grd<2>(g, gres, gresGrd);
    }
}

__device__ __forceinline__ float sub_rn(float a, float b) { float r; asm("v_sub_f32 %0, %1, %2" : "=v"(r) : "v"(a), "v"(b)); return r; }
__device__ __forceinline__ void rn_rotT(float r, float x, float y, float z, f3& r0, f3& r1, f3& r2) {
    const float xx = mul_rn(x, x), yy = mul_rn(y, y), zz = mul_rn(z, z), xy = mul_rn(x, y), xz = mul_rn(x, z), yz = mul_rn(y, z);
    const float rx = mul_rn(r, x), ry = mul_rn(r, y), rz = mul_rn(r, z);
    r0 = mk3(sub_rn(1.f, mul_rn(2.f, add_rn(yy, zz))), mul_rn(2.f, add_rn(xy, rz)), mul_rn(2.f, sub_rn(xz, ry)));
    r1 = mk3(mul_rn(2.f, sub_rn(xy, rz)), sub_rn(1.f, mul_rn(2.f, add_rn(xx, zz))), mul_rn(2.f, add_rn(yz, rx)));
    r2 = mk3(mul_rn(2.f, add_rn(xz, ry)), mul_rn(2.f, sub_rn(yz, rx)), sub_rn(1.f, mul_rn(2.f, add_rn(xx, yy))));
}
__device__ __forceinline__ float oracle_order_hit_t(const Ray& ray, f3 pos, f3 scl, f3 rt0, f3 rt1, f3 rt2, f3 gis) {
    const f3 gposc = mk3(sub_rn(ray.o.x, pos.x), sub_rn(ray.o.y, pos.y), sub_rn(ray.o.z, pos.z));
    const f3 gro = mk3(mul_rn(gis.x, rn_dot3(rt0, gposc)), mul_rn(gis.y, rn_dot3(rt1, gposc)), mul_rn(gis.z, rn_dot3(rt2, gposc)));
    const f3 grdu = mk3(mul_rn(gis.x, rn_dot3(rt0, ray.d)), mul_rn(gis.y, rn_dot3(rt1, ray.d)), mul_rn(gis.z, rn_dot3(rt2, ray.d)));
    const float inv = 1.f / sqrtf(rn_dot3(grdu, grdu));
    const f3 grd = mk3(mul_rn(grdu.x, inv), mul_rn(grdu.y, inv), mul_rn(grdu.z, inv));
// ... 1341 lines not shown
```

3dgrut_amd/csrc/scan_sort.hip:

```cpp
#include "common.hpp"

namespace grut {

namespace {

constexpr int kScanThreads = 256;
constexpr int kScanItems   = 8;
constexpr int kScanTile    = kScanThreads * kScanItems;

__device__ __forceinline__ uint32_t wave_incl_scan_u32(uint32_t v, int lane) {
#pragma unroll
    for (int off = 1; off < 64; off <<= 1) {
        const uint32_t n = __shfl_up(v, off, 64);
        if (lane >= off) v += n;
    }
    return v;
}

__device__ __forceinline__ uint32_t block_excl_scan_256(uint32_t v, uint32_t* total, uint32_t* s_wave ) {
    const int lane = threadIdx.x & 63, wave = threadIdx.x >> 6;
    const uint32_t incl = wave_incl_scan_u32(v, lane);
    if (lane == 63) s_wave[wave] = incl;
    __syncthreads();
    uint32_t base = 0, tot = 0;
#pragma unroll
    for (int w = 0; w < 4; ++w) {
        const uint32_t s = s_wave[w];
        if (w < wave) base += s;
        tot += s;
    }
    *total = tot;
    __syncthreads();
    return base + incl - v;
}

__device__ __forceinline__ void load_items(const uint32_t* __restrict__ in, const uint32_t* __restrict__ gather,
                                           uint32_t base, uint32_t n, uint32_t (&x)[kScanItems]) {
    const uint32_t i0 = base + threadIdx.x * kScanItems;
    if (!gather && i0 + kScanItems <= n) {
        const uint4 a = *reinterpret_cast<const uint4*>(in + i0);
        const uint4 b = *reinterpret_cast<const uint4*>(in + i0 + 4);
        x[0] = a.x; x[1] = a.y; x[2] = a.z; x[3] = a.w; x[4] = b.x; x[5] = b.y; x[6] = b.z; x[7] = b.w;
    } else {
#pragma unroll
        for (int k = 0; k < kScanItems; ++k) {
            const uint32_t i = i0 + k;
            x[k] = i < n ? (gather ? in[gather[i]] : in[i]) : 0u;
        }
    }
}

__global__ __launch_bounds__(kScanThreads) void scan_reduce_kernel(const uint32_t* __restrict__ in,
                                                                   const uint32_t* __restrict__ gather, uint32_t n,
                                                                   uint32_t* __restrict__ block_sums) {
    __shared__ uint32_t s_wave[4];
    uint32_t x[kScanItems];
    load_items(in, gather, blockIdx.x * kScanTile, n, x);
    uint32_t s = 0;
#pragma unroll
    for (int k = 0; k < kScanItems; ++k) s += x[k];
    uint32_t total;
    (void)block_excl_scan_256(s, &total, s_wave);
    if (threadIdx.x == 0) block_sums[blockIdx.x] = total;
}

__global__ __launch_bounds__(kScanThreads) void scan_block_sums_kernel(uint32_t* __restrict__ block_sums, uint32_t nb) {
    __shared__ uint32_t s_wave[4];
    const uint32_t per = (nb + kScanThreads - 1) / kScanThreads;
    const uint32_t b0 = threadIdx.x * per;
    uint32_t s = 0;
    for (uint32_t k = 0; k < per; ++k) {
        const uint32_t i = b0 + k;
        if (i < nb) s += block_sums[i];
    }
    uint32_t total;
    uint32_t run = block_excl_scan_256(s, &total, s_wave);
    for (uint32_t k = 0; k < per; ++k) {
        const uint32_t i = b0 + k;
        if (i < nb) {
            const uint32_t v = block_sums[i];
            block_sums[i] = run;
            run += v;
        }
    }
}

template <bool EXCLUSIVE, bool FUSED>
__global__ __launch_bounds__(kScanThreads) void scan_apply_kernel(const uint32_t* __restrict__ in,
                                                                  const uint32_t* __restrict__ gather, uint32_t n,
                                                                  const uint32_t* __restrict__ block_sums,
                                                                  uint32_t* __restrict__ out) {
    __shared__ uint32_t s_wave[4];
    uint32_t x[kScanItems];
    const uint32_t base = blockIdx.x * kScanTile;
    load_items(in, gather, base, n, x);
    uint32_t s = 0;
#pragma unroll
    for (int k = 0; k < kScanItems; ++k) s += x[k];
    uint32_t total;
    uint32_t block_base;
    if (FUSED) {
        uint32_t pre = 0;
        for (uint32_t i = threadIdx.x; i < blockIdx.x; i += kScanThreads) pre += block_sums[i];
        (void)block_excl_scan_256(pre, &block_base, s_wave);
    } else {
        block_base = block_sums[blockIdx.x];
    }
    uint32_t run = block_excl_scan_256(s, &total, s_wave) + block_base;
    const uint32_t i0 = base + threadIdx.x * kScanItems;
    uint32_t y[kScanItems];
#pragma unroll
    for (int k = 0; k < kScanItems; ++k) {
        if (EXCLUSIVE) { y[k] = run; run += x[k]; }
        else { run += x[k]; y[k] = run; }
    }
    if (i0 + kScanItems <= n) {
        *reinterpret_cast<uint4*>(out + i0)     = make_uint4(y[0], y[1], y[2], y[3]);
        *reinterpret_cast<uint4*>(out + i0 + 4) = make_uint4(y[4], y[5], y[6], y[7]);
    } else {
#pragma unroll
        for (int k = 0; k < kScanItems; ++k)
            if (i0 + k < n) out[i0 + k] = y[k];
    }
}

int scan_impl(hipStream_t s, uint32_t n, const uint32_t* in, const uint32_t* gather, uint32_t* out, bool exclusive,
              void* scratch, size_t scratch_bytes) {
    if (n == 0) return GRUT_OK;
    const uint32_t nb = div_up(n, kScanTile);
    GRUT_REQUIRE(scratch_bytes >= (size_t)nb * sizeof(uint32_t), "scan scratch too small");
    uint32_t* sums = reinterpret_cast<uint32_t*>(scratch);
    hipLaunchKernelGGL(scan_reduce_kernel, dim3(nb), dim3(kScanThreads), 0, s, in, gather, n, sums);
    const bool fused = nb <= 8192u;
    if (!fused) hipLaunchKernelGGL(scan_block_sums_kernel, dim3(1), dim3(kScanThreads), 0, s, sums, nb);
    if (exclusive) {
        if (fused) hipLaunchKernelGGL((scan_apply_kernel<true, true>), dim3(nb), dim3(kScanThreads), 0, s, in, gather, n, sums, out);
        else hipLaunchKernelGGL((scan_apply_kernel<true, false>), dim3(nb), dim3(kScanThreads), 0, s, in, gather, n, sums, out);
    } else {
        if (fused) hipLaunchKernelGGL((scan_apply_kernel<false, true>), dim3(nb), dim3(kScanThreads), 0, s, in, gather, n, sums, out);
        else hipLaunchKernelGGL((scan_apply_kernel<false, false>), dim3(nb), dim3(kScanThreads), 0, s, in, gather, n, sums, out);
    }
    GRUT_HIP(hipGetLastError());
    return GRUT_OK;
}

constexpr int kSortThreads = 256;
#ifndef GRUT_SORT_SMALL
#define GRUT_SORT_SMALL 8
#endif
constexpr int kSortRoundsLarge = 16, kSortRoundsSmall = GRUT_SORT_SMALL;
constexpr uint32_t kSortSmallLimit = 2u << 20;
constexpr int kRadix       = 256;

__device__ __forceinline__ uint32_t eff_count(uint32_t n, const uint32_t* n_dev) {
    if (!n_dev) return n;
    const uint32_t m = *n_dev;
    return m < n ? m : n;
}

template <int kSortRounds>
__global__ __launch_bounds__(kSortThreads) void radix_hist_kernel(const uint32_t* __restrict__ keys, uint32_t n,
                                                                  const uint32_t* __restrict__ n_dev, int shift, uint32_t mask,
                                                                  uint32_t nb, uint32_t* __restrict__ hist) {
    __shared__ uint32_t s_hist[4][kRadix];
    const int wave = threadIdx.x >> 6;
    const uint32_t ne = eff_count(n, n_dev);
#pragma unroll
    for (int w = 0; w < 4; ++w) s_hist[w][threadIdx.x] = 0;
    __syncthreads();
    constexpr int kSortTile = kSortThreads * kSortRounds;
    const uint32_t base = blockIdx.x * kSortTile;
    if (base < ne) {
#pragma unroll
        for (int k = 0; k < kSortRounds / 4; ++k) {
            const uint32_t i = base + (k * kSortThreads + threadIdx.x) * 4;
            if (i + 4 <= ne) {
                const uint4 v = *reinterpret_cast<const uint4*>(keys + i);
                atomicAdd(&s_hist[wave][(v.x >> shift) & mask], 1u);
                atomicAdd(&s_hist[wave][(v.y >> shift) & mask], 1u);
                atomicAdd(&s_hist[wave][(v.z >> shift) & mask], 1u);
                atomicAdd(&s_hist[wave][(v.w >> shift) & mask], 1u);
            } else {
                for (uint32_t j = i; j < ne && j < i + 4; ++j) atomicAdd(&s_hist[wave][(keys[j] >> shift) & mask], 1u);
            }
        }
    }
    __syncthreads();
    const uint32_t d = threadIdx.x;
    hist[(size_t)d * nb + blockIdx.x] = s_hist[0][d] + s_hist[1][d] + s_hist[2][d] + s_hist[3][d];
}

__global__ __launch_bounds__(kSortThreads) void radix_rowscan_kernel(uint32_t* __restrict__ hist, uint32_t nb, uint32_t* __restrict__ totals) {
    __shared__ uint32_t s_wave[4];
    if (blockIdx.x == 0 && threadIdx.x >= gridDim.x) totals[threadIdx.x] = 0u;
    uint32_t* row = hist + (size_t)blockIdx.x * nb;
    uint32_t carry = 0;
    for (uint32_t base = 0; base < nb; base += kSortThreads) {
        const uint32_t i = base + threadIdx.x;
        const uint32_t v = i < nb ? row[i] : 0u;
        uint32_t total;
        const uint32_t excl = block_excl_scan_256(v, &total, s_wave);
        if (i < nb) row[i] = carry + excl;
        carry += total;
    }
    if (threadIdx.x == 0) totals[blockIdx.x] = carry;
}

template <int kSortRounds>
__global__ __launch_bounds__(kSortThreads) void radix_scatter_kernel(const uint32_t* __restrict__ keys_in,
                                                                     const uint32_t* __restrict__ vals_in, uint32_t n,
                                                                     const uint32_t* __restrict__ n_dev, int shift, uint32_t mask,
                                                                     uint32_t nb, const uint32_t* __restrict__ hist_scanned,
                                                                     const uint32_t* __restrict__ digit_totals,
                                                                     uint32_t* __restrict__ keys_out, uint32_t* __restrict__ vals_out) {
    constexpr int kSortTile = kSortThreads * kSortRounds, kSortWaveKeys = 64 * kSortRounds;
    __shared__ uint32_t s_cnt[4][kRadix];
    const int lane = threadIdx.x & 63, wave = threadIdx.x >> 6;
    const uint32_t ne = eff_count(n, n_dev);
    const uint32_t base = blockIdx.x * kSortTile;
    if (base >= ne) return;
#pragma unroll
    for (int w = 0; w < 4; ++w) s_cnt[w][threadIdx.x] = 0;
    __syncthreads();

    uint32_t key[kSortRounds], val[kSortRounds], rank[kSortRounds];
    const uint32_t wbase = base + wave * kSortWaveKeys;
    volatile uint32_t* cnt = s_cnt[wave];
#pragma unroll
    for (int r = 0; r < kSortRounds; ++r) {
        const uint32_t i = wbase + r * 64 + lane;
        const bool valid = i < ne;
        key[r] = valid ? keys_in[i] : 0xFFFFFFFFu;
        val[r] = valid ? (vals_in ? vals_in[i] : i) : 0u;
    }
#pragma unroll
    for (int r = 0; r < kSortRounds; ++r) {
        const uint32_t i = wbase + r * 64 + lane;
        const bool valid = i < ne;
        const uint32_t d = (key[r] >> shift) & mask;
        unsigned long long m = __ballot(valid);
#pragma unroll
        for (int b = 0; b < 8; ++b) {
            const unsigned long long bb = __ballot((d >> b) & 1u);
            m &= ((d >> b) & 1u) ? bb : ~bb;
        }
        const uint32_t before = __builtin_amdgcn_mbcnt_hi((uint32_t)(m >> 32), __builtin_amdgcn_mbcnt_lo((uint32_t)m, 0u));
        const uint32_t count  = (uint32_t)__popcll(m);
        uint32_t old = 0;
        if (valid) old = cnt[d];
        __builtin_amdgcn_wave_barrier();
        if (valid && before == 0) cnt[d] = old + count;
        __builtin_amdgcn_wave_barrier();
        rank[r] = old + before;
    }
    __syncthreads();
    __shared__ uint32_t s_keys[kSortTile], s_vals[kSortTile];
    __shared__ uint32_t s_dstart[kRadix];
    __shared__ uint32_t s_gdelta[kRadix];
    __shared__ uint32_t s_wave_tot[4];
    {
        const uint32_t d = threadIdx.x;
        uint32_t run = 0;
#pragma unroll
        for (int w = 0; w < 4; ++w) {
            const uint32_t c = s_cnt[w][d];
            s_cnt[w][d] = run;
            run += c;
        }
        uint32_t total;
        const uint32_t excl = block_excl_scan_256(run, &total, s_wave_tot);
        const uint32_t digit_base = block_excl_scan_256(digit_totals[d], &total, s_wave_tot);
        s_dstart[d] = excl;
        s_gdelta[d] = digit_base + hist_scanned[(size_t)d * nb + blockIdx.x] - excl;
    }
    __syncthreads();
#pragma unroll
    for (int r = 0; r < kSortRounds; ++r) {
        const uint32_t i = wbase + r * 64 + lane;
        if (i < ne) {
            const uint32_t d = (key[r] >> shift) & mask;
            const uint32_t pos = s_dstart[d] + s_cnt[wave][d] + rank[r];
            s_keys[pos] = key[r];
            s_vals[pos] = val[r];
        }
    }
    __syncthreads();
    const uint32_t nvalid = min((uint32_t)kSortTile, ne - base);
#pragma unroll
    for (int r = 0; r < kSortRounds; ++r) {
        const uint32_t idx = r * kSortThreads + threadIdx.x;
        if (idx < nvalid) {
            const uint32_t k = s_keys[idx];
            const uint32_t dst = s_gdelta[(k >> shift) & mask] + idx;
            keys_out[dst] = k;
            vals_out[dst] = s_vals[idx];
        }
    }
}


constexpr uint32_t kFlagAgg = 1u << 30, kFlagPrefix = 2u << 30, kCountMask = (1u << 30) - 1u;
constexpr int kMaxPasses = 4;
#ifndef GRUT_SORT_LOOKBACK
#define GRUT_SORT_LOOKBACK 8
#endif
constexpr int kLookback = GRUT_SORT_LOOKBACK;

__global__ __launch_bounds__(kSortThreads) void radix_global_hist_kernel(const uint32_t* __restrict__ keys, uint32_t n, const uint32_t* __restrict__ n_dev,
                                                                         int begin_bit, int width, int passes, int end_bit,
                                                                         uint32_t* __restrict__ hist ) {
    __shared__ uint32_t s_hist[kMaxPasses][kRadix];
    const uint32_t ne = eff_count(n, n_dev);
    for (int p = 0; p < kMaxPasses; ++p) s_hist[p][threadIdx.x] = 0;
    __syncthreads();
    const uint32_t stride = gridDim.x * kSortThreads * 4;
    for (uint32_t i = (blockIdx.x * kSortThreads + threadIdx.x) * 4; i < ne; i += stride) {
        uint32_t k[4];
        if (i + 4 <= ne) {
            const uint4 v = *reinterpret_cast<const uint4*>(keys + i);
            k[0] = v.x; k[1] = v.y; k[2] = v.z; k[3] = v.w;
        } else {
            for (int j = 0; j < 4; ++j) k[j] = i + j < ne ? keys[i + j] : 0xFFFFFFFFu;
        }
        const int cnt = (int)min(4u, ne - i);
        for (int j = 0; j < cnt; ++j)
            for (int p = 0; p < passes; ++p) {
                const int bit = begin_bit + p * width;
                const int nbits = (end_bit - bit) < width ? (end_bit - bit) : width;
                atomicAdd(&s_hist[p][(k[j] >> bit) & ((1u << nbits) - 1u)], 1u);
            }
    }
    __syncthreads();
    for (int p = 0; p < passes; ++p) {
        const uint32_t c = s_hist[p][threadIdx.x];
        if (c) atomicAdd(&hist[p * kRadix + threadIdx.x], c);
    }
}

template <int kSortRounds>
__global__ __launch_bounds__(kSortThreads) void radix_onesweep_kernel(const uint32_t* __restrict__ keys_in, const uint32_t* __restrict__ vals_in, uint32_t n,
                                                                      const uint32_t* __restrict__ n_dev, int shift, uint32_t mask,
                                                                      const uint32_t* __restrict__ digit_totals ,
                                                                      uint32_t* __restrict__ status , uint32_t* __restrict__ ticket,
                                                                      uint32_t* __restrict__ keys_out, uint32_t* __restrict__ vals_out) {
    constexpr int kSortTile = kSortThreads * kSortRounds, kSortWaveKeys = 64 * kSortRounds;
    __shared__ uint32_t s_cnt[4][kRadix];
    __shared__ uint32_t s_tile;
    const int lane = threadIdx.x & 63, wave = threadIdx.x >> 6;
    const uint32_t ne = eff_count(n, n_dev);
    if (threadIdx.x == 0) s_tile = atomicAdd(ticket, 1u);
#pragma unroll
    for (int w = 0; w < 4; ++w) s_cnt[w][threadIdx.x] = 0;
    __syncthreads();
    const uint32_t tile = s_tile;
    const uint32_t base = tile * kSortTile;
    if (base >= ne) return;

    uint32_t key[kSortRounds], val[kSortRounds], rank[kSortRounds];
    const uint32_t wbase = base + wave * kSortWaveKeys;
    volatile uint32_t* cnt = s_cnt[wave];
#pragma unroll
    for (int r = 0; r < kSortRounds; ++r) {
        const uint32_t i = wbase + r * 64 + lane;
        const bool valid = i < ne;
        key[r] = valid ? keys_in[i] : 0xFFFFFFFFu;
        val[r] = valid ? (vals_in ? vals_in[i] : i) : 0u;
    }
#pragma unroll
    for (int r = 0; r < kSortRounds; ++r) {
        const uint32_t i = wbase + r * 64 + lane;
        const bool valid = i < ne;
        const uint32_t d = (key[r] >> shift) & mask;
        unsigned long long m = __ballot(valid);
#pragma unroll
        for (int b = 0; b < 8; ++b) {
            const unsigned long long bb = __ballot((d >> b) & 1u);
            m &= ((d >> b) & 1u) ? bb : ~bb;
        }
        const uint32_t before = __builtin_amdgcn_mbcnt_hi((uint32_t)(m >> 32), __builtin_amdgcn_mbcnt_lo((uint32_t)m, 0u));
        const uint32_t count  = (uint32_t)__popcll(m);
        uint32_t old = 0;
        if (valid) old = cnt[d];
        __builtin_amdgcn_wave_barrier();
        if (valid && before == 0) cnt[d] = old + count;
        __builtin_amdgcn_wave_barrier();
        rank[r] = old + before;
    }
    __syncthreads();
    __shared__ uint32_t s_keys[kSortTile], s_vals[kSortTile];
    __shared__ uint32_t s_dstart[kRadix];
    __shared__ uint32_t s_gdelta[kRadix];
    __shared__ uint32_t s_wave_tot[4];
    {
        const uint32_t d = threadIdx.x;
        uint32_t run = 0;
#pragma unroll
        for (int w = 0; w < 4; ++w) {
            const uint32_t c = s_cnt[w][d];
            s_cnt[w][d] = run;
            run += c;
        }
        uint32_t before_tiles = 0;
        if (d <= mask) {
            uint32_t* mine = status + (size_t)tile * kRadix + d;
            __hip_atomic_store(mine, (tile == 0 ? kFlagPrefix : kFlagAgg) | run, __ATOMIC_RELAXED, __HIP_MEMORY_SCOPE_AGENT);
            if (tile > 0) {
                int t = (int)tile - 1;
                bool done = false;
                while (!done) {
                    uint32_t w[kLookback];
#pragma unroll
                    for (int k = 0; k < kLookback; ++k)
                        w[k] = t - k >= 0 ? __hip_atomic_load(status + (size_t)(t - k) * kRadix + d, __ATOMIC_RELAXED, __HIP_MEMORY_SCOPE_AGENT) : kFlagPrefix;
                    int used = 0;
#pragma unroll
                    for (int k = 0; k < kLookback; ++k) {
                        if (!done && used == k) {
                            if ((w[k] >> 30) != 0u) {
                                before_tiles += w[k] & kCountMask;
                                ++used;
                                done = (w[k] & kFlagPrefix) != 0u;
                            }
                        }
                    }
                    t -= used;
                    if (!done && used == 0) __builtin_amdgcn_s_sleep(1);
                }
                __hip_atomic_store(mine, kFlagPrefix | (before_tiles + run), __ATOMIC_RELAXED, __HIP_MEMORY_SCOPE_AGENT);
            }
        }
        uint32_t total;
        const uint32_t excl = block_excl_scan_256(run, &total, s_wave_tot);
        const uint32_t digit_base = block_excl_scan_256(digit_totals[d], &total, s_wave_tot);
        s_dstart[d] = excl;
        s_gdelta[d] = digit_base + before_tiles - excl;
    }
    __syncthreads();
#pragma unroll
    for (int r = 0; r < kSortRounds; ++r) {
        const uint32_t i = wbase + r * 64 + lane;
        if (i < ne) {
            const uint32_t d = (key[r] >> shift) & mask;
            const uint32_t pos = s_dstart[d] + s_cnt[wave][d] + rank[r];
            s_keys[pos] = key[r];
            s_vals[pos] = val[r];
        }
    }
    __syncthreads();
    const uint32_t nvalid = min((uint32_t)kSortTile, ne - base);
#pragma unroll
    for (int r = 0; r < kSortRounds; ++r) {
        const uint32_t idx = r * kSortThreads + threadIdx.x;
        if (idx < nvalid) {
            const uint32_t k = s_keys[idx];
            const uint32_t dst = s_gdelta[(k >> shift) & mask] + idx;
            keys_out[dst] = k;
            vals_out[dst] = s_vals[idx];
        }
    }
}

}

size_t scan_scratch_bytes(uint32_t n) { return (size_t)(div_up(n, kScanTile) + 1) * sizeof(uint32_t); }

int inclusive_scan_u32(hipStream_t s, uint32_t n, const uint32_t* in, const uint32_t* gather, uint32_t* out,
                       void* scratch, size_t scratch_bytes) {
    return scan_impl(s, n, in, gather, out, false, scratch, scratch_bytes);
}

constexpr size_t kOnesweepHead = (size_t)kMaxPasses * kRadix + 64;
static bool sort_legacy();
size_t sort_scratch_bytes(uint32_t n) {
    const uint32_t nb = div_up(n, (uint32_t)(kSortThreads * kSortRoundsSmall));
    const size_t hist = (size_t)kRadix * nb * sizeof(uint32_t);
    const size_t legacy = hist + kRadix * sizeof(uint32_t) + 256;
    const size_t onesweep = (kOnesweepHead + (size_t)kMaxPasses * nb * kRadix) * sizeof(uint32_t);
    return (sort_legacy() || legacy > onesweep) ? legacy : onesweep;
}

static bool sort_legacy() {
    static const bool v = [] { const char* e = getenv("GRUT_SORT_ONESWEEP"); return !(e && e[0] == '1'); }();
    return v;
}

int sort_pairs_u32(hipStream_t s, uint32_t n, const uint32_t* n_dev, int begin_bit, int end_bit,
                   uint32_t* keys, uint32_t* vals, uint32_t* keys_tmp, uint32_t* vals_tmp,
                   void* scratch, size_t scratch_bytes, uint32_t** out_keys, uint32_t** out_vals, bool vals_iota) {
    *out_keys = keys;
    *out_vals = vals;
    if (n == 0 || end_bit <= begin_bit) return GRUT_OK;
    GRUT_REQUIRE(scratch_bytes >= sort_scratch_bytes(n), "sort scratch too small");
    const bool small = n <= kSortSmallLimit;
    const uint32_t nb = div_up(n, (uint32_t)(kSortThreads * (small ? kSortRoundsSmall : kSortRoundsLarge)));
    uint32_t* hist = reinterpret_cast<uint32_t*>(scratch);
    uint32_t* totals = hist + (size_t)kRadix * nb;
    uint32_t *ki = keys, *vi = vals, *ko = keys_tmp, *vo = vals_tmp;
    {
        const int total_bits = end_bit - begin_bit, passes = (total_bits + 7) / 8, width = (total_bits + passes - 1) / passes;
        if (!sort_legacy() && passes <= kMaxPasses) {
            uint32_t* head = reinterpret_cast<uint32_t*>(scratch);
            uint32_t* tickets = head + (size_t)kMaxPasses * kRadix;
            uint32_t* status = head + kOnesweepHead;
            GRUT_HIP(hipMemsetAsync(head, 0, (kOnesweepHead + (size_t)passes * nb * kRadix) * sizeof(uint32_t), s));
            const uint32_t hist_blocks = nb < 1024u ? nb : 1024u;
            hipLaunchKernelGGL(radix_global_hist_kernel, dim3(hist_blocks), dim3(kSortThreads), 0, s, ki, n, n_dev, begin_bit, width, passes, end_bit, head);
            int p = 0;
            for (int bit = begin_bit; bit < end_bit; bit += width, ++p) {
                const int nbits = (end_bit - bit) < width ? (end_bit - bit) : width;
                const uint32_t mask = (1u << nbits) - 1u;
                const uint32_t* vin = (vals_iota && bit == begin_bit) ? nullptr : vi;
                uint32_t* st = status + (size_t)p * nb * kRadix;
                if (small) hipLaunchKernelGGL(radix_onesweep_kernel<kSortRoundsSmall>, dim3(nb), dim3(kSortThreads), 0, s, ki, vin, n, n_dev, bit, mask, head + p * kRadix, st, tickets + p, ko, vo);
                else hipLaunchKernelGGL(radix_onesweep_kernel<kSortRoundsLarge>, dim3(nb), dim3(kSortThreads), 0, s, ki, vin, n, n_dev, bit, mask, head + p * kRadix, st, tickets + p, ko, vo);
                uint32_t* t;
                t = ki; ki = ko; ko = t;
                t = vi; vi = vo; vo = t;
            }
            GRUT_HIP(hipGetLastError());
            *out_keys = ki;
            *out_vals = vi;
            return GRUT_OK;
        }
    }
    const int total_bits = end_bit - begin_bit, passes = (total_bits + 7) / 8, width = (total_bits + passes - 1) / passes;
    for (int bit = begin_bit; bit < end_bit; bit += width) {
        const int nbits = (end_bit - bit) < width ? (end_bit - bit) : width;
        const uint32_t mask = (1u << nbits) - 1u;
        if (small) hipLaunchKernelGGL(radix_hist_kernel<kSortRoundsSmall>, dim3(nb), dim3(kSortThreads), 0, s, ki, n, n_dev, bit, mask, nb, hist);
        else hipLaunchKernelGGL(radix_hist_kernel<kSortRoundsLarge>, dim3(nb), dim3(kSortThreads), 0, s, ki, n, n_dev, bit, mask, nb, hist);
        hipLaunchKernelGGL(radix_rowscan_kernel, dim3(1u << nbits), dim3(kSortThreads), 0, s, hist, nb, totals);
        const uint32_t* vin = (vals_iota && bit == begin_bit) ? nullptr : vi;
        if (small) hipLaunchKernelGGL(radix_scatter_kernel<kSortRoundsSmall>, dim3(nb), dim3(kSortThreads), 0, s, ki, vin, n, n_dev, bit, mask, nb, hist, totals, ko, vo);
        else hipLaunchKernelGGL(radix_scatter_kernel<kSortRoundsLarge>, dim3(nb), dim3(kSortThreads), 0, s, ki, vin, n, n_dev, bit, mask, nb, hist, totals, ko, vo);
        uint32_t* t;
        t = ki; ki = ko; ko = t;
        t = vi; vi = vo; vo = t;
    }
    GRUT_HIP(hipGetLastError());
    *out_keys = ki;
    *out_vals = vi;
    return GRUT_OK;
}

}

extern "C" {

uint64_t grut_sort_scratch_bytes(uint32_t n) { return grut::sort_scratch_bytes(n); }
uint64_t grut_scan_scratch_bytes(uint32_t n) { return grut::scan_scratch_bytes(n); }

int grut_sort_pairs_u32(void* stream, uint32_t n, int begin_bit, int end_bit, uint32_t* keys, uint32_t* values,
                        uint32_t* keys_tmp, uint32_t* values_tmp, void* scratch, uint64_t scratch_bytes,
                        uint32_t** sorted_keys, uint32_t** sorted_values) {
    return grut::sort_pairs_u32(reinterpret_cast<hipStream_t>(stream), n, nullptr, begin_bit, end_bit, keys, values,
                                keys_tmp, values_tmp, scratch, scratch_bytes, sorted_keys, sorted_values);
}

int grut_inclusive_scan_u32(void* stream, uint32_t n, const uint32_t* in, uint32_t* out, void* scratch, uint64_t scratch_bytes) {
    return grut::inclusive_scan_u32(reinterpret_cast<hipStream_t>(stream), n, in, nullptr, out, scratch, scratch_bytes);
}

}
```

Baseline: 1.067 billion rays/s.

## Fuse radix row-scan into histogram kernel and epoch-tag backward gradient flags

```diff
diff --git a/3dgrut_amd/csrc/common.hpp b/3dgrut_amd/csrc/common.hpp
--- a/3dgrut_amd/csrc/common.hpp
+++ b/3dgrut_amd/csrc/common.hpp
@@ -159,6 +159,16 @@
 int sort_pairs_u32(hipStream_t s, uint32_t n, const uint32_t* n_dev, int begin_bit, int end_bit,
                    uint32_t* keys, uint32_t* vals, uint32_t* keys_tmp, uint32_t* vals_tmp,
                    void* scratch, size_t scratch_bytes, uint32_t** out_keys, uint32_t** out_vals, bool vals_iota = false);
+constexpr size_t kSortTicketBytes = 256;
+inline int ensure_sort_scratch(DeviceBuffer& b, size_t need, float growth = 1.0f) {
+    const size_t before = b.bytes;
+    GRUT_CHECK(b.ensure(need, growth));
+    if (b.bytes != before) {
+        if (b.external) GRUT_HIP(hipMemsetAsync(b.ptr, 0, kSortTicketBytes, scratch_stream()));
+        else GRUT_HIP(hipMemset(b.ptr, 0, kSortTicketBytes));
+    }
+    return GRUT_OK;
+}
 
 }
 
diff --git a/3dgrut_amd/csrc/grt_api.hip b/3dgrut_amd/csrc/grt_api.hip
--- a/3dgrut_amd/csrc/grt_api.hip
+++ b/3dgrut_amd/csrc/grt_api.hip
@@ -249,7 +249,7 @@
     GRUT_CHECK(h->ids.ensure(n * 4, 1.25f));
     GRUT_CHECK(h->codes_tmp.ensure(n * 4, 1.25f));
     GRUT_CHECK(h->ids_tmp.ensure(n * 4, 1.25f));
-    GRUT_CHECK(h->sort_scratch.ensure(sort_scratch_bytes((uint32_t)(n * 1.25f) + 4096)));
+    GRUT_CHECK(ensure_sort_scratch(h->sort_scratch, sort_scratch_bytes((uint32_t)(n * 1.25f) + 4096)));
     GRUT_CHECK(h->nodes.ensure(n * sizeof(GrtNode), 1.25f));
     GRUT_CHECK(h->counters.ensure(n * 4, 1.25f));
 
@@ -324,7 +324,7 @@
         grt_launch_list_cones(s, P, ray_origin, ray_direction, flag, dir_len, h->l_block_cones.as<GrtCone>(), h->l_super_cones.as<GrtCone>());
         grt_launch_list_count(s, P, bvh, ray_origin, flag, dir_len, h->l_block_cones.as<GrtCone>(), h->l_super_cones.as<GrtCone>(),
                               h->l_inst_rel.as<float>(), h->l_key_bits.as<uint32_t>(), h->l_counts.as<uint32_t>(), h->l_pidx.as<uint32_t>(), h->l_pair_cache.ptr);
-        GRUT_CHECK(h->l_sort_scratch.ensure(sort_scratch_bytes((uint32_t)(N * 1.25f) + 4096)));
+        GRUT_CHECK(ensure_sort_scratch(h->l_sort_scratch, sort_scratch_bytes((uint32_t)(N * 1.25f) + 4096)));
         uint32_t *sorted_key = nullptr, *rank_to_particle = nullptr;
         GRUT_CHECK(sort_pairs_u32(s, N, nullptr, 16, 32, h->l_key_bits.as<uint32_t>(), h->l_pidx.as<uint32_t>(), h->l_key_tmp.as<uint32_t>(),
                                   h->l_pidx_tmp.as<uint32_t>(), h->l_sort_scratch.ptr, h->l_sort_scratch.bytes, &sorted_key, &rank_to_particle, true));
@@ -353,7 +353,7 @@
             for (DeviceBuffer* b4 : {&h->l_block_keys, &h->l_vals, &h->l_block_keys_tmp, &h->l_vals_tmp}) ok = ok && b4->ensure((size_t)n * 4, 1.3f) == GRUT_OK;
             ok = ok && h->l_ranges.ensure((size_t)nb * 8, 1.25f) == GRUT_OK;
             ok = ok && h->l_bounds.ensure((size_t)n * 8, 1.3f) == GRUT_OK;
-            ok = ok && h->l_sort_scratch.ensure(sort_scratch_bytes((uint32_t)(n * 1.3f) + 4096)) == GRUT_OK;
+            ok = ok && ensure_sort_scratch(h->l_sort_scratch, sort_scratch_bytes((uint32_t)(n * 1.3f) + 4096)) == GRUT_OK;
             if (!ok) (void)hipGetLastError();
             return ok;
         };
@@ -621,7 +621,7 @@
     GRUT_CHECK(h->m_ids.ensure(n * 4, 1.25f));
     GRUT_CHECK(h->m_codes_tmp.ensure(n * 4, 1.25f));
     GRUT_CHECK(h->m_ids_tmp.ensure(n * 4, 1.25f));
-    GRUT_CHECK(h->m_sort_scratch.ensure(sort_scratch_bytes((uint32_t)(n * 1.25f) + 4096)));
+    GRUT_CHECK(ensure_sort_scratch(h->m_sort_scratch, sort_scratch_bytes((uint32_t)(n * 1.25f) + 4096)));
     GRUT_CHECK(h->m_nodes.ensure(n * sizeof(GrtNode), 1.25f));
     GRUT_CHECK(h->m_done.ensure(n * 4, 1.25f));
     grt_launch_mesh_aabb(s, num_faces, vertices, triangles, h->m_aabb.as<float>(), h->m_slack.as<float>(), h->m_scene_enc.as<uint32_t>());
diff --git a/3dgrut_amd/csrc/gut_api.hip b/3dgrut_amd/csrc/gut_api.hip
--- a/3dgrut_amd/csrc/gut_api.hip
+++ b/3dgrut_amd/csrc/gut_api.hip
@@ -63,6 +63,19 @@
     bool prof_used[kProfRing][GUT_NUM_STAGES];
     int prof_slot = 0, prof_created = 0;
     int prof_fwd_slot = 0;
+
+    uint32_t flag_epoch = 0;
+    int next_flag_epoch(size_t I, hipStream_t s, GutGradSlots* slots) {
+        const size_t before = grad_flag.bytes;
+        GRUT_CHECK(grad_flag.ensure(2 * I + 96, 1.3f));
+        if (grad_flag.bytes != before || flag_epoch >= 255u) {
+            GRUT_HIP(hipMemsetAsync(grad_flag.ptr, 0, grad_flag.bytes, s));
+            flag_epoch = 0;
+        }
+        slots->flag = grad_flag.as<uint8_t>();
+        slots->epoch = ++flag_epoch;
+        return GRUT_OK;
+    }
 
     uint32_t profile_mask = 0xFFFFFFFFu;
     int stage_begin(int stage, hipStream_t s, int slot) {
@@ -165,7 +178,7 @@
     GRUT_CHECK(h->part_offset.ensure(n * 4, 1.25f));
     GRUT_CHECK(h->rec64.ensure(n * 64, 1.25f));
     GRUT_CHECK(h->walk8.ensure(n * 8, 1.25f));
-    GRUT_CHECK(h->sort_scratch.ensure(sort_scratch_bytes((uint32_t)(n * 1.25f) + 4096)));
+    GRUT_CHECK(ensure_sort_scratch(h->sort_scratch, sort_scratch_bytes((uint32_t)(n * 1.25f) + 4096)));
     GRUT_CHECK(h->scan_scratch.ensure(scan_scratch_bytes((uint32_t)(n * 1.25f) + 4096)));
     if (!h->counters.ptr) {
         GRUT_CHECK(h->counters.ensure(kGutCounterWords * 4));
@@ -182,7 +195,7 @@
     GRUT_CHECK(h->tile_keys_tmp.ensure(n * 4, 1.3f));
     GRUT_CHECK(h->tile_vals_tmp.ensure(n * 4, 1.3f));
     GRUT_CHECK(h->pos_particle.ensure(n * 4, 1.3f));
-    GRUT_CHECK(h->tile_sort_scratch.ensure(sort_scratch_bytes((uint32_t)n), 1.3f));
+    GRUT_CHECK(ensure_sort_scratch(h->tile_sort_scratch, sort_scratch_bytes((uint32_t)n), 1.3f));
     GRUT_CHECK(h->ranges.ensure((size_t)tiles * 8 + 8));
     const size_t nb = (size_t)I / kGutSegment + 1;
     if (!h->params.nht && h->params.k_buffer == 0) {
@@ -497,13 +510,12 @@
             slots.stride = 16;
             slots.partial = nullptr;
             slots.flag = nullptr;
+            slots.epoch = 0;
             slots.pos_particle = h->pos_particle.as<uint32_t>();
             if (I > 0) {
                 GRUT_CHECK(h->grad_partial.ensure(2 * I * (size_t)slots.stride * 4, 1.3f));
-                GRUT_CHECK(h->grad_flag.ensure(2 * I + 96, 1.3f));
                 slots.partial = h->grad_partial.as<float>();
-                slots.flag = h->grad_flag.as<uint8_t>();
-                GRUT_HIP(hipMemsetAsync(slots.flag, 0, 2 * I, s));
+                GRUT_CHECK(h->next_flag_epoch(I, s, &slots));
                 GRUT_CHECK(h->stage_begin(GUT_STAGE_RENDER_BWD, s, slot));
                 launch_render_nhtp_bwd(s, P, h->ranges.as<uint32_t>(), h->sorted_pos, particle_density, particle_sph, ray_origin, ray_direction, feat_density,
                                        io ? nullptr : grad_feat_density, io ? io->grad_features : nullptr, io ? io->grad_opacity : nullptr, hit_distance,
@@ -544,6 +556,7 @@
     slots.stride = has_gdist ? 20 : 16;
     slots.partial = nullptr;
     slots.flag = nullptr;
+    slots.epoch = 0;
     slots.pos_particle = h->pos_particle.as<uint32_t>();
     const size_t I = h->num_intersections;
     if (P.k_buffer > 0) {
@@ -566,10 +579,8 @@
     }
     if (I > 0) {
         GRUT_CHECK(h->grad_partial.ensure(2 * I * (size_t)slots.stride * 4, 1.3f));
-        GRUT_CHECK(h->grad_flag.ensure(2 * I + 96, 1.3f));
         slots.partial = h->grad_partial.as<float>();
-        slots.flag = h->grad_flag.as<uint8_t>();
-        GRUT_HIP(hipMemsetAsync(slots.flag, 0, 2 * I, s));
+        GRUT_CHECK(h->next_flag_epoch(I, s, &slots));
         GRUT_CHECK(h->stage_begin(GUT_STAGE_RENDER_BWD, s, slot));
         launch_render_bwd(s, P, h->ranges.as<uint32_t>(), h->sorted_pos, particle_density, proj.rgb, ray_origin, ray_direction, feat_density,
                           g_in, hit_distance, grad_hit_distance, slots, h->checkpoints);
diff --git a/3dgrut_amd/csrc/gut_internal.hpp b/3dgrut_amd/csrc/gut_internal.hpp
--- a/3dgrut_amd/csrc/gut_internal.hpp
+++ b/3dgrut_amd/csrc/gut_internal.hpp
@@ -52,6 +52,7 @@
     uint8_t* flag;
     const uint32_t* pos_particle;
     int stride;
+    uint32_t epoch;
 };
 
 struct GutGradOut {
diff --git a/3dgrut_amd/csrc/gut_kernels.hip b/3dgrut_amd/csrc/gut_kernels.hip
--- a/3dgrut_amd/csrc/gut_kernels.hip
+++ b/3dgrut_amd/csrc/gut_kernels.hip
@@ -736,8 +736,13 @@
             for (uint32_t base = 0; base < nb; base += 64) {
                 const FlagChunk* fc = reinterpret_cast<const FlagChunk*>(slots.flag + s0 + base);
                 const FlagChunk w0 = fc[0], w1 = fc[1], w2 = fc[2], w3 = fc[3];
-                constexpr unsigned long long kPack = 0x0102040810204080ull, kLsb = 0x0101010101010101ull;
-                auto pack8 = [](unsigned long long w) { return ((w & kLsb) * kPack) >> 56; };
+                constexpr unsigned long long kPack = 0x0102040810204080ull, kLsb = 0x0101010101010101ull, kLow7 = 0x7F7F7F7F7F7F7F7Full;
+                const unsigned long long splat = (unsigned long long)slots.epoch * kLsb;
+                auto pack8 = [splat](unsigned long long w) {
+                    const unsigned long long x = w ^ splat;
+                    const unsigned long long zero = ~(((x & kLow7) + kLow7) | x | kLow7);
+                    return (((zero >> 7) & kLsb) * kPack) >> 56;
+                };
                 unsigned long long m = pack8(w0.lo) | (pack8(w0.hi) << 8) | (pack8(w1.lo) << 16) | (pack8(w1.hi) << 24) |
                                        (pack8(w2.lo) << 32) | (pack8(w2.hi) << 40) | (pack8(w3.lo) << 48) | (pack8(w3.hi) << 56);
                 const uint32_t rem = nb - base;
@@ -766,7 +771,7 @@
             part.clear();
             const int g = lane >> 2;
             for (uint32_t base = 0; base < n2; base += 64) {
-                const bool set = (base + (uint32_t)lane < n2) && slots.flag[s0 + base + lane] != 0;
+                const bool set = (base + (uint32_t)lane < n2) && slots.flag[s0 + base + lane] == (uint8_t)slots.epoch;
                 const unsigned long long m = __ballot(set);
                 if (m == 0) continue;
                 int b[4], nb = 0;
diff --git a/3dgrut_amd/csrc/gut_render.hip b/3dgrut_amd/csrc/gut_render.hip
--- a/3dgrut_amd/csrc/gut_render.hip
+++ b/3dgrut_amd/csrc/gut_render.hip
@@ -903,7 +903,7 @@
 #endif
                 out[4] = make_float4(ex, ey, ez, 0.f);
             }
-            slots.flag[slot] = 1;
+            slots.flag[slot] = (uint8_t)slots.epoch;
         }
         __syncthreads();
         b = bend;
diff --git a/3dgrut_amd/csrc/scan_sort.hip b/3dgrut_amd/csrc/scan_sort.hip
--- a/3dgrut_amd/csrc/scan_sort.hip
+++ b/3dgrut_amd/csrc/scan_sort.hip
@@ -158,11 +158,20 @@
     return m < n ? m : n;
 }
 
+constexpr int kSortChunks = 32;
+#ifndef GRUT_SORT_SCAN_BATCH
+#define GRUT_SORT_SCAN_BATCH 8
+#endif
+constexpr int kSortTicketWords = (int)(kSortTicketBytes / sizeof(uint32_t));
+static_assert(kSortChunks <= kSortTicketWords, "one ticket per chunk");
+
 template <int kSortRounds>
 __global__ __launch_bounds__(kSortThreads) void radix_hist_kernel(const uint32_t* __restrict__ keys, uint32_t n,
                                                                   const uint32_t* __restrict__ n_dev, int shift, uint32_t mask,
-                                                                  uint32_t nb, uint32_t* __restrict__ hist) {
+                                                                  uint32_t nb, int log2c, uint32_t* hist, uint32_t* __restrict__ ctot,
+                                                                  uint32_t* __restrict__ tickets) {
     __shared__ uint32_t s_hist[4][kRadix];
+    __shared__ uint32_t s_last;
     const int wave = threadIdx.x >> 6;
     const uint32_t ne = eff_count(n, n_dev);
 #pragma unroll
@@ -187,31 +196,61 @@
     }
     __syncthreads();
     const uint32_t d = threadIdx.x;
-    hist[(size_t)d * nb + blockIdx.x] = s_hist[0][d] + s_hist[1][d] + s_hist[2][d] + s_hist[3][d];
-}
-
-__global__ __launch_bounds__(kSortThreads) void radix_rowscan_kernel(uint32_t* __restrict__ hist, uint32_t nb, uint32_t* __restrict__ totals) {
-    __shared__ uint32_t s_wave[4];
-    if (blockIdx.x == 0 && threadIdx.x >= gridDim.x) totals[threadIdx.x] = 0u;
-    uint32_t* row = hist + (size_t)blockIdx.x * nb;
-    uint32_t carry = 0;
-    for (uint32_t base = 0; base < nb; base += kSortThreads) {
-        const uint32_t i = base + threadIdx.x;
-        const uint32_t v = i < nb ? row[i] : 0u;
-        uint32_t total;
-        const uint32_t excl = block_excl_scan_256(v, &total, s_wave);
-        if (i < nb) row[i] = carry + excl;
-        carry += total;
-    }
-    if (threadIdx.x == 0) totals[blockIdx.x] = carry;
+    if (d <= mask) __hip_atomic_store(&hist[(size_t)d * nb + blockIdx.x], s_hist[0][d] + s_hist[1][d] + s_hist[2][d] + s_hist[3][d], __ATOMIC_RELAXED, __HIP_MEMORY_SCOPE_AGENT);
+    asm volatile("s_waitcnt vmcnt(0)" ::: "memory");
+    __syncthreads();
+    const uint32_t chunk = blockIdx.x >> log2c, col0 = chunk << log2c;
+    const uint32_t ncols = min(1u << log2c, nb - col0);
+    if (threadIdx.x == 0) {
+        const uint32_t t = __hip_atomic_fetch_add(&tickets[chunk], 1u, __ATOMIC_RELAXED, __HIP_MEMORY_SCOPE_AGENT);
+        s_last = t == ncols - 1u;
+        if (t == ncols - 1u) __hip_atomic_store(&tickets[chunk], 0u, __ATOMIC_RELAXED, __HIP_MEMORY_SCOPE_AGENT);
+    }
+    __syncthreads();
+    if (!s_last) return;
+    __builtin_amdgcn_fence(__ATOMIC_ACQUIRE, "agent");
+
+    constexpr int kBatch = GRUT_SORT_SCAN_BATCH;
+    const uint32_t hl = threadIdx.x & 31u, hw = threadIdx.x >> 5;
+    for (uint32_t row0 = hw; row0 <= mask; row0 += 8u * kBatch) {
+        uint32_t carry[kBatch];
+#pragma unroll
+        for (int r = 0; r < kBatch; ++r) carry[r] = 0u;
+        for (uint32_t c = 0; c < ncols; c += 32u) {
+            const bool in = c + hl < ncols;
+            uint32_t v[kBatch];
+#pragma unroll
+            for (int r = 0; r < kBatch; ++r) {
+                const uint32_t row = row0 + 8u * r;
+                v[r] = (in && row <= mask) ? hist[(size_t)row * nb + col0 + c + hl] : 0u;
+            }
+#pragma unroll
+            for (int r = 0; r < kBatch; ++r) {
+                const uint32_t row = row0 + 8u * r;
+                uint32_t incl = v[r];
+#pragma unroll
+                for (int o = 1; o < 32; o <<= 1) {
+                    const uint32_t up = __shfl_up(incl, o, 32);
+                    if (hl >= (uint32_t)o) incl += up;
+                }
+                if (in && row <= mask) hist[(size_t)row * nb + col0 + c + hl] = carry[r] + incl - v[r];
+                carry[r] += __shfl(incl, 31, 32);
+            }
+        }
+#pragma unroll
+        for (int r = 0; r < kBatch; ++r) {
+            const uint32_t row = row0 + 8u * r;
+            if (hl == 0 && row <= mask) ctot[row * kSortChunks + chunk] = carry[r];
+        }
+    }
 }
 
 template <int kSortRounds>
 __global__ __launch_bounds__(kSortThreads) void radix_scatter_kernel(const uint32_t* __restrict__ keys_in,
                                                                      const uint32_t* __restrict__ vals_in, uint32_t n,
                                                                      const uint32_t* __restrict__ n_dev, int shift, uint32_t mask,
-                                                                     uint32_t nb, const uint32_t* __restrict__ hist_scanned,
-                                                                     const uint32_t* __restrict__ digit_totals,
+                                                                     uint32_t nb, int log2c, const uint32_t* __restrict__ hist_scanned,
+                                                                     const uint32_t* __restrict__ ctot,
                                                                      uint32_t* __restrict__ keys_out, uint32_t* __restrict__ vals_out) {
     constexpr int kSortTile = kSortThreads * kSortRounds, kSortWaveKeys = 64 * kSortRounds;
     __shared__ uint32_t s_cnt[4][kRadix];
@@ -267,11 +306,22 @@
             s_cnt[w][d] = run;
             run += c;
         }
+        uint32_t dtot = 0, before = 0;
+        if (d <= mask) {
+            const uint32_t nch = (nb + (1u << log2c) - 1u) >> log2c, mine = blockIdx.x >> log2c;
+#pragma unroll
+            for (uint32_t c = 0; c < (uint32_t)kSortChunks; ++c) {
+                const uint32_t v = c < nch ? ctot[d * kSortChunks + c] : 0u;
+                dtot += v;
+                before += c < mine ? v : 0u;
+            }
+            before += hist_scanned[(size_t)d * nb + blockIdx.x];
+        }
         uint32_t total;
         const uint32_t excl = block_excl_scan_256(run, &total, s_wave_tot);
-        const uint32_t digit_base = block_excl_scan_256(digit_totals[d], &total, s_wave_tot);
+        const uint32_t digit_base = block_excl_scan_256(dtot, &total, s_wave_tot);
         s_dstart[d] = excl;
-        s_gdelta[d] = digit_base + hist_scanned[(size_t)d * nb + blockIdx.x] - excl;
+        s_gdelta[d] = digit_base + before - excl;
     }
     __syncthreads();
 #pragma unroll
@@ -474,8 +524,8 @@
 size_t sort_scratch_bytes(uint32_t n) {
     const uint32_t nb = div_up(n, (uint32_t)(kSortThreads * kSortRoundsSmall));
     const size_t hist = (size_t)kRadix * nb * sizeof(uint32_t);
-    const size_t legacy = hist + kRadix * sizeof(uint32_t) + 256;
-    const size_t onesweep = (kOnesweepHead + (size_t)kMaxPasses * nb * kRadix) * sizeof(uint32_t);
+    const size_t legacy = (kSortTicketWords + (size_t)kRadix * kSortChunks) * sizeof(uint32_t) + hist;
+    const size_t onesweep = (kSortTicketWords + kOnesweepHead + (size_t)kMaxPasses * nb * kRadix) * sizeof(uint32_t);
     return (sort_legacy() || legacy > onesweep) ? legacy : onesweep;
 }
 
@@ -493,13 +543,16 @@
     GRUT_REQUIRE(scratch_bytes >= sort_scratch_bytes(n), "sort scratch too small");
     const bool small = n <= kSortSmallLimit;
     const uint32_t nb = div_up(n, (uint32_t)(kSortThreads * (small ? kSortRoundsSmall : kSortRoundsLarge)));
-    uint32_t* hist = reinterpret_cast<uint32_t*>(scratch);
-    uint32_t* totals = hist + (size_t)kRadix * nb;
+    uint32_t* tickets = reinterpret_cast<uint32_t*>(scratch);
+    uint32_t* hist = tickets + kSortTicketWords;
+    uint32_t* ctot = hist + (size_t)kRadix * nb;
+    int log2c = 5;
+    while (div_up(nb, 1u << log2c) > (uint32_t)kSortChunks) ++log2c;
     uint32_t *ki = keys, *vi = vals, *ko = keys_tmp, *vo = vals_tmp;
     {
         const int total_bits = end_bit - begin_bit, passes = (total_bits + 7) / 8, width = (total_bits + passes - 1) / passes;
         if (!sort_legacy() && passes <= kMaxPasses) {
-            uint32_t* head = reinterpret_cast<uint32_t*>(scratch);
+            uint32_t* head = reinterpret_cast<uint32_t*>(scratch) + kSortTicketWords;
             uint32_t* tickets = head + (size_t)kMaxPasses * kRadix;
             uint32_t* status = head + kOnesweepHead;
             GRUT_HIP(hipMemsetAsync(head, 0, (kOnesweepHead + (size_t)passes * nb * kRadix) * sizeof(uint32_t), s));
@@ -527,12 +580,11 @@
     for (int bit = begin_bit; bit < end_bit; bit += width) {
         const int nbits = (end_bit - bit) < width ? (end_bit - bit) : width;
         const uint32_t mask = (1u << nbits) - 1u;
-        if (small) hipLaunchKernelGGL(radix_hist_kernel<kSortRoundsSmall>, dim3(nb), dim3(kSortThreads), 0, s, ki, n, n_dev, bit, mask, nb, hist);
-        else hipLaunchKernelGGL(radix_hist_kernel<kSortRoundsLarge>, dim3(nb), dim3(kSortThreads), 0, s, ki, n, n_dev, bit, mask, nb, hist);
-        hipLaunchKernelGGL(radix_rowscan_kernel, dim3(1u << nbits), dim3(kSortThreads), 0, s, hist, nb, totals);
+        if (small) hipLaunchKernelGGL(radix_hist_kernel<kSortRoundsSmall>, dim3(nb), dim3(kSortThreads), 0, s, ki, n, n_dev, bit, mask, nb, log2c, hist, ctot, tickets);
+        else hipLaunchKernelGGL(radix_hist_kernel<kSortRoundsLarge>, dim3(nb), dim3(kSortThreads), 0, s, ki, n, n_dev, bit, mask, nb, log2c, hist, ctot, tickets);
         const uint32_t* vin = (vals_iota && bit == begin_bit) ? nullptr : vi;
-        if (small) hipLaunchKernelGGL(radix_scatter_kernel<kSortRoundsSmall>, dim3(nb), dim3(kSortThreads), 0, s, ki, vin, n, n_dev, bit, mask, nb, hist, totals, ko, vo);
-        else hipLaunchKernelGGL(radix_scatter_kernel<kSortRoundsLarge>, dim3(nb), dim3(kSortThreads), 0, s, ki, vin, n, n_dev, bit, mask, nb, hist, totals, ko, vo);
+        if (small) hipLaunchKernelGGL(radix_scatter_kernel<kSortRoundsSmall>, dim3(nb), dim3(kSortThreads), 0, s, ki, vin, n, n_dev, bit, mask, nb, log2c, hist, ctot, ko, vo);
+        else hipLaunchKernelGGL(radix_scatter_kernel<kSortRoundsLarge>, dim3(nb), dim3(kSortThreads), 0, s, ki, vin, n, n_dev, bit, mask, nb, log2c, hist, ctot, ko, vo);
         uint32_t* t;
         t = ki; ki = ko; ko = t;
         t = vi; vi = vo; vo = t;
@@ -553,6 +605,8 @@
 int grut_sort_pairs_u32(void* stream, uint32_t n, int begin_bit, int end_bit, uint32_t* keys, uint32_t* values,
                         uint32_t* keys_tmp, uint32_t* values_tmp, void* scratch, uint64_t scratch_bytes,
                         uint32_t** sorted_keys, uint32_t** sorted_values) {
+    if (n > 0 && end_bit > begin_bit && scratch && scratch_bytes >= grut::kSortTicketBytes)
+        GRUT_HIP(hipMemsetAsync(scratch, 0, grut::kSortTicketBytes, reinterpret_cast<hipStream_t>(stream)));
     return grut::sort_pairs_u32(reinterpret_cast<hipStream_t>(stream), n, nullptr, begin_bit, end_bit, keys, values,
                                 keys_tmp, values_tmp, scratch, scratch_bytes, sorted_keys, sorted_values);
 }
```

Measured after the change: 974.5 million rays/s. 8.7% lower.
